# malaire/reed-solomon-16

Hardware: AMD Instinct MI355X
Metric: encode+decode GiB/s (device-resident, 1024B shards); % of HBM roofline (higher is better)
Workload: dtype u16; 1 GPU; 32768:32768 x 1024 B encode + 100%-loss decode per GPU (BASELINE configs[3]); original_count=32768, recovery_count=32768, parallelism=independent stripes x 1 (weak, no collective), column_slices=1, decode_issue=serial: rs16_decode_device after the encode

## Files before the change

include/rs16.h:

```cpp
#ifndef RS16_H
#define RS16_H

#include <stddef.h>
#include <stdint.h>

#ifdef __cplusplus
extern "C" {
#endif

typedef enum rs16_error_code {
    RS16_OK = 0,
    RS16_DIFFERENT_SHARD_SIZE = 1,
    RS16_DUPLICATE_ORIGINAL_SHARD_INDEX = 2,
    RS16_DUPLICATE_RECOVERY_SHARD_INDEX = 3,
    RS16_INVALID_ORIGINAL_SHARD_INDEX = 4,
    RS16_INVALID_RECOVERY_SHARD_INDEX = 5,
    RS16_INVALID_SHARD_SIZE = 6,
    RS16_NOT_ENOUGH_SHARDS = 7,
    RS16_TOO_FEW_ORIGINAL_SHARDS = 8,
    RS16_TOO_MANY_ORIGINAL_SHARDS = 9,
    RS16_UNSUPPORTED_SHARD_COUNT = 10,
    RS16_DEVICE_ERROR = 100,
    RS16_INVALID_ARGUMENT = 101
} rs16_error_code;
// ... 71 lines not shown
const void* rs16_decoder_restored_original_device(rs16_decoder* dec, size_t index);
int rs16_decoder_restored_original_copy(rs16_decoder* dec, size_t index, void* dst, size_t len, rs16_error* err);
void rs16_decoder_result_drop(rs16_decoder* dec);
int rs16_decoder_is_high_rate(const rs16_decoder* dec);

int rs16_encode_device(rs16_engine* eng, size_t original_count, size_t recovery_count, size_t shard_bytes,
                       const void* d_original, void* d_recovery, void* stream, rs16_error* err);
int rs16_encode_device_batch(rs16_engine* eng, size_t original_count, size_t recovery_count, size_t shard_bytes,
                             size_t nstripes, const void* d_original, size_t original_stride, void* d_recovery,
                             size_t recovery_stride, void* stream, rs16_error* err);
int rs16_decode_device(rs16_engine* eng, size_t original_count, size_t recovery_count, size_t shard_bytes,
                       void* d_original, const uint8_t* d_original_received, const void* d_recovery,
                       const uint8_t* d_recovery_received, size_t original_received_count,
                       size_t recovery_received_count, void* stream, rs16_error* err);
int rs16_decode_device_batch(rs16_engine* eng, size_t original_count, size_t recovery_count, size_t shard_bytes,
                             size_t nstripes, void* d_original, size_t original_stride,
                             const uint8_t* d_original_received, const void* d_recovery, size_t recovery_stride,
                             const uint8_t* d_recovery_received, size_t original_received_count,
                             size_t recovery_received_count, void* stream, rs16_error* err);
int rs16_decode_device_batch_varied(rs16_engine* eng, size_t original_count, size_t recovery_count,
                                    size_t shard_bytes, size_t nstripes, void* d_original, size_t original_stride,
                                    const uint8_t* d_original_received, size_t original_received_stride,
                                    const void* d_recovery, size_t recovery_stride,
                                    const uint8_t* d_recovery_received, size_t recovery_received_stride,
                                    const size_t* original_received_counts, const size_t* recovery_received_counts,
                                    void* stream, rs16_error* err);
int rs16_decode_check(rs16_engine* eng, void* stream, rs16_error* err);
int rs16_engine_set_slices(rs16_engine* eng, int slices, rs16_error* err);

int rs16_encode_host(rs16_engine* eng, size_t original_count, size_t recovery_count, size_t shard_bytes,
                     const void* h_original, void* h_recovery, size_t slice_bytes, rs16_error* err);
int rs16_decode_host(rs16_engine* eng, size_t original_count, size_t recovery_count, size_t shard_bytes,
                     void* h_original, const uint8_t* original_received, const void* h_recovery,
                     const uint8_t* recovery_received, size_t slice_bytes, rs16_error* err);

int rs16_decode_prepare(rs16_engine* eng, size_t original_count, size_t recovery_count, size_t shard_bytes,
                        const uint8_t* d_original_received, const uint8_t* d_recovery_received,
                        size_t original_received_count, size_t recovery_received_count, void* stream,
                        rs16_error* err);
int rs16_decode_device_prepared(rs16_engine* eng, size_t original_count, size_t recovery_count,
                                size_t shard_bytes, void* d_original, const void* d_recovery, void* stream,
                                rs16_error* err);

enum { RS16_UPDATE_MAX_SHARDS = 32 };
typedef struct rs16_update_plan rs16_update_plan;
rs16_update_plan* rs16_update_plan_new(rs16_engine* eng, int rate, size_t original_count, size_t recovery_count,
                                       const size_t* indices, size_t n, rs16_error* err);
void rs16_update_plan_free(rs16_update_plan* plan);
size_t rs16_update_plan_count(const rs16_update_plan* plan);
int rs16_update_plan_coefficients(rs16_update_plan* plan, uint16_t* out, rs16_error* err);
int rs16_update_device(rs16_update_plan* plan, size_t shard_bytes, const void* d_delta, void* d_recovery,
                       size_t recovery_pos, size_t recovery_n, void* stream, rs16_error* err);

int rs16_encode_host_batch(rs16_engine* eng, size_t original_count, size_t recovery_count, size_t shard_bytes,
                           size_t nstripes, const void* h_original, size_t original_stride, void* h_recovery,
                           size_t recovery_stride, rs16_error* err);
int rs16_decode_host_batch(rs16_engine* eng, size_t original_count, size_t recovery_count, size_t shard_bytes,
                           size_t nstripes, void* h_original, size_t original_stride,
                           const uint8_t* original_received, size_t original_received_stride,
                           const void* h_recovery, size_t recovery_stride, const uint8_t* recovery_received,
                           size_t recovery_received_stride, rs16_error* err);

int rs16_encode_host_multi(rs16_engine* const* engines, int n, size_t original_count, size_t recovery_count,
                           size_t shard_bytes, const void* h_original, void* h_recovery, rs16_error* err);
int rs16_decode_host_multi(rs16_engine* const* engines, int n, size_t original_count, size_t recovery_count,
                           size_t shard_bytes, void* h_original, const uint8_t* original_received,
                           const void* h_recovery, const uint8_t* recovery_received, rs16_error* err);

typedef struct rs16_comm rs16_comm;
int rs16_comm_unique_id(void* id128, rs16_error* err);
rs16_comm* rs16_comm_new(rs16_engine* eng, int nranks, int rank, const void* id128, rs16_error* err);
int rs16_comm_init_all(rs16_engine* const* engines, int n, rs16_comm** comms, rs16_error* err);
void rs16_comm_free(rs16_comm* comm);
int rs16_comm_rank(const rs16_comm* comm);
int rs16_comm_size(const rs16_comm* comm);
int rs16_column_slice(size_t shard_bytes, int nranks, int rank, size_t* offset, size_t* width);
int rs16_scatter_columns(rs16_comm* const* comms, int n, int root, size_t rows, size_t shard_bytes,
                         const void* const* d_full, void* const* d_slice, void* stream, rs16_error* err);
int rs16_gather_columns(rs16_comm* const* comms, int n, int root, size_t rows, size_t shard_bytes,
                        const void* const* d_slice, void* const* d_full, void* stream, rs16_error* err);
int rs16_scatter_columns_virtual(rs16_comm* comm, int vslices, size_t rows, size_t shard_bytes, const void* d_full,
                                 void* const* d_slices, void* stream, rs16_error* err);
int rs16_gather_columns_virtual(rs16_comm* comm, int vslices, size_t rows, size_t shard_bytes,
                                const void* const* d_slices, void* d_full, void* stream, rs16_error* err);

void* rs16_device_alloc(rs16_engine* eng, size_t bytes, rs16_error* err);
void rs16_device_free(rs16_engine* eng, void* d_ptr);
int rs16_memcpy_htod(rs16_engine* eng, void* d_dst, const void* src, size_t bytes, void* stream, rs16_error* err);
int rs16_memcpy_dtoh(rs16_engine* eng, void* dst, const void* d_src, size_t bytes, void* stream, rs16_error* err);
int rs16_memset_device(rs16_engine* eng, void* d_dst, int value, size_t bytes, void* stream, rs16_error* err);
int rs16_memcpy2d_htod(rs16_engine* eng, void* d_dst, size_t d_pitch, const void* src, size_t h_pitch, size_t width,
                       size_t rows, void* stream, rs16_error* err);
int rs16_memcpy2d_dtoh(rs16_engine* eng, void* dst, size_t h_pitch, const void* d_src, size_t d_pitch, size_t width,
                       size_t rows, void* stream, rs16_error* err);
void* rs16_stream_create(rs16_engine* eng, rs16_error* err);
void rs16_stream_destroy(rs16_engine* eng, void* stream);
void* rs16_host_alloc(rs16_engine* eng, size_t bytes, rs16_error* err);
void rs16_host_free(rs16_engine* eng, void* h_ptr);

int rs16_engine_set_profiling(rs16_engine* eng, int enable, rs16_error* err);
int rs16_engine_profile_read(rs16_engine* eng, int prog, double* total_ms, uint64_t* launches, rs16_error* err);
void rs16_engine_profile_reset(rs16_engine* eng);
int rs16_prog_count(void);
int rs16_engine_set_stamps(rs16_engine* eng, void* d_buf, int prog, rs16_error* err);
const char* rs16_prog_name(int prog);

enum {
    RS16_DIAG_FORCE_VOFF64 = 1,
    RS16_DIAG_EVAL_TWO_KERNEL = 2,
    RS16_DIAG_EVAL_FULL = 4,
    RS16_DIAG_NO_COLUMN = 8,
    RS16_DIAG_FORCE_COLUMN = 16,
    RS16_DIAG_TILE_LAST = 32,
    RS16_DIAG_NO_TILE_LAST = 64,
    RS16_DIAG_FD_LDS = 128,
    RS16_DIAG_COL_RADIX4 = 256,
    RS16_DIAG_NO_IDENTITY = 512,
    RS16_DIAG_NO_MID_DIRECT = 1024,
    RS16_DIAG_WIDE_TWIDDLES = 2048,
    RS16_DIAG_NO_LATE_ROWS = 4096,
    RS16_DIAG_NO_PAIRED_ROWS = 8192,
    RS16_DIAG_NO_TOWER_ROWS = 16384
};
int rs16_engine_set_diagnostics(rs16_engine* eng, int flags);
int rs16_set_diagnostics(int flags);

void rs16_host_mul(const void* in, void* out, size_t bytes, uint16_t log_m);
void rs16_host_mul_narrow(const void* in, void* out, size_t bytes, uint16_t log_m);
uint32_t rs16_host_twiddle(uint32_t index, uint32_t* log_m, uint32_t* table20);
int rs16_host_twiddle_narrow(uint32_t index);
uint64_t rs16_host_fast_div_check(uint32_t divisor, uint32_t n0, uint32_t count, uint32_t step);
typedef struct rs16_pass_consts {
    uint32_t voff32, full_lanes, nslab;
    uint32_t quads, threads, load_shb, store_shb, reg_bits, row_sets;
    uint64_t rs_in, rs_seg, rs_out;
    uint32_t late_rows;
} rs16_pass_consts;
int rs16_host_pass_consts(int prog, int T, uint32_t lo, uint64_t s_in, uint64_t s_out, uint64_t s_seg, uint64_t s_rest,
                          uint32_t qrow, uint32_t chunk, uint32_t row_base_in, uint32_t in_rows_mask, int diag,
                          rs16_pass_consts* out);
int rs16_host_pass_consts_many(int prog, int T, uint32_t lo, size_t n, const uint64_t* s_in, const uint64_t* s_out,
                               const uint64_t* s_seg, const uint64_t* s_rest, const uint32_t* qrow, uint32_t chunk,
                               uint32_t row_base_in, uint32_t in_rows_mask, int diag, rs16_pass_consts* out);
int rs16_host_pass_consts_rows(int prog, int T, uint32_t lo, uint64_t s_in, uint64_t s_out, uint64_t s_seg,
                               uint64_t s_rest, uint32_t qrow, uint32_t chunk, uint32_t row_base_in,
                               uint32_t in_rows_mask, uint32_t a_count, int diag, rs16_pass_consts* out);
int rs16_host_paired_rows(uint32_t chunk_rows, uint64_t S, uint64_t S_user, uint32_t a_count, uint32_t seg_chunk,
                          uint32_t row_base_in, int diag);
int rs16_host_tower_rows(uint32_t chunk_rows, uint64_t S, uint64_t S_user, uint32_t a_count, uint32_t seg_chunk,
                         uint32_t row_base_in, int diag);
uint32_t rs16_host_tower_basis(uint32_t i);
void rs16_host_tower_conv(const void* in, void* out, size_t bytes);
int rs16_host_tower_twiddle(uint32_t index, uint32_t* table20);
void rs16_host_mul_tower(const void* in, void* out, size_t bytes, uint32_t index, int narrow);
int rs16_host_update_consts(uint32_t rows, uint64_t shard_bytes, uint32_t n, uint32_t* quads_per_lane,
                            uint32_t* nslab, uint32_t* rows_per_wave, uint64_t* blocks);

const char* rs16_version(void);

#ifdef __cplusplus
}
#endif
#endif
```

reed-solomon-16_amd/csrc/rs16_api.cpp:

```cpp
#include <atomic>
#include <rccl/rccl.h>

#include <cstdio>

#include "rs16_api.hpp"
#include "rs16_pass_common.hpp"

using namespace rs16;

extern "C" size_t rs16_error_message(const rs16_error* e, char* buf, size_t len) {
    char tmp[256];
    unsigned long long a = e->v0, b = e->v1, c = e->v2;
    switch (e->code) {
    case RS16_OK: snprintf(tmp, sizeof tmp, "ok"); break;
    case RS16_DIFFERENT_SHARD_SIZE:
        snprintf(tmp, sizeof tmp, "different shard size: expected %llu bytes, got %llu bytes", a, b);
        break;
    case RS16_DUPLICATE_ORIGINAL_SHARD_INDEX: snprintf(tmp, sizeof tmp, "duplicate original shard index: %llu", a); break;
    case RS16_DUPLICATE_RECOVERY_SHARD_INDEX: snprintf(tmp, sizeof tmp, "duplicate recovery shard index: %llu", a); break;
    case RS16_INVALID_ORIGINAL_SHARD_INDEX:
        snprintf(tmp, sizeof tmp, "invalid original shard index: %llu >= original_count %llu", b, a);
        break;
    case RS16_INVALID_RECOVERY_SHARD_INDEX:
        snprintf(tmp, sizeof tmp, "invalid recovery shard index: %llu >= recovery_count %llu", b, a);
        break;
    case RS16_INVALID_SHARD_SIZE:
        snprintf(tmp, sizeof tmp, "invalid shard size: %llu bytes (must non-zero and multiple of 64)", a);
        break;
    case RS16_NOT_ENOUGH_SHARDS:
        snprintf(tmp, sizeof tmp, "not enough shards: %llu original + %llu recovery < %llu original_count", b, c, a);
        break;
    case RS16_TOO_FEW_ORIGINAL_SHARDS:
        snprintf(tmp, sizeof tmp, "too few original shards: got %llu shards while original_count is %llu", b, a);
        break;
    case RS16_TOO_MANY_ORIGINAL_SHARDS:
        snprintf(tmp, sizeof tmp, "too many original shards: got more than original_count (%llu) shards", a);
        break;
    case RS16_UNSUPPORTED_SHARD_COUNT:
        snprintf(tmp, sizeof tmp, "unsupported shard count: %llu original shards with %llu recovery shards", a, b);
        break;
    case RS16_DEVICE_ERROR:
        if (a >= 1000)
            snprintf(tmp, sizeof tmp, "device error: RCCL: %s", ncclGetErrorString((ncclResult_t)(a - 1000)));
        else
            snprintf(tmp, sizeof tmp, "device error: %s", hipGetErrorString((hipError_t)a));
        break;
    case RS16_INVALID_ARGUMENT: snprintf(tmp, sizeof tmp, "invalid argument"); break;
    default: snprintf(tmp, sizeof tmp, "unknown error %d", e->code); break;
    }
    size_t n = strlen(tmp);
    if (buf && len) {
        size_t c2 = std::min(n, len - 1);
        memcpy(buf, tmp, c2);
        buf[c2] = 0;
    }
    return n;
}

template <class F> static void host_mul_table(const void* in, void* out, size_t bytes, const uint32_t* t, F mul) {
    const uint8_t* src = (const uint8_t*)in;
    uint8_t* dst = (uint8_t*)out;
    for (size_t q = 0; q < bytes / 8; q++) {
        const size_t off = (q >> 3) * 64 + (q & 7) * 4;
        uint32_t yl, yh, ol = 0, oh = 0;
        memcpy(&yl, src + off, 4);
        memcpy(&yh, src + off + 32, 4);
        mul(ol, oh, yl, yh, t);
        memcpy(dst + off, &ol, 4);
        memcpy(dst + off + 32, &oh, 4);
    }
}
template <class Mul> static void host_mul(const void* in, void* out, size_t bytes, uint16_t log_m, Mul mul) {
    host_mul_table(in, out, bytes, &host_tables().mul_tab[(size_t)log_m * TAB_DWORDS], mul);
}
extern "C" void rs16_host_mul(const void* in, void* out, size_t bytes, uint16_t log_m) {
    host_mul(in, out, bytes, log_m, mul_xor);
}
extern "C" void rs16_host_mul_narrow(const void* in, void* out, size_t bytes, uint16_t log_m) {
    host_mul(in, out, bytes, log_m, mul_xor_narrow);
}
extern "C" uint32_t rs16_host_twiddle(uint32_t index, uint32_t* log_m, uint32_t* table20) {
    const HostTables& t = host_tables();
    if (index >= GF_MODULUS) return ~0u;
    if (log_m) *log_m = t.skew[index];
    if (table20) memcpy(table20, &t.skew_tab[(size_t)index * TAB_DWORDS], 20 * sizeof(uint32_t));
    return t.skew[index] == GF_MODULUS ? 0u : t.exp[t.skew[index]];
}
extern "C" int rs16_host_twiddle_narrow(uint32_t index) { return twiddle_narrow(index) ? 1 : 0; }
extern "C" uint64_t rs16_host_fast_div_check(uint32_t divisor, uint32_t n0, uint32_t count, uint32_t step) {
    const FastDiv f = fast_div_of(divisor);
    uint64_t bad = 0;
    for (uint64_t i = 0, n = n0; i < count && n < ((uint64_t)1 << 32); i++, n += step)
        bad += fast_div((uint32_t)n, f.mul, f.one) != (uint32_t)n / divisor;
    return bad;
}

static int host_pass_consts(int prog, int T, uint32_t lo, size_t n, const uint64_t* s_in, const uint64_t* s_out,
                            const uint64_t* s_seg, const uint64_t* s_rest, const uint32_t* qrow, uint32_t chunk,
                            uint32_t row_base_in, uint32_t in_rows_mask, uint32_t a_count, int diag,
                            rs16_pass_consts* out) {
    if (prog < 0 || prog >= NUM_PROGS || T < 0 || T > 8 || !out) return 0;
    const PassKernel& k = pass_kernel_of(prog, T);
    if (!k.fn) return 0;
    PassArgs a{};
    a.lo = lo, a.chunk = chunk, a.row_base_in = row_base_in, a.in_rows_mask = in_rows_mask;
    a.diag = (uint32_t)diag;
    a.a_count = a_count;
    for (size_t i = 0; i < n; i++) {
        a.S_in = s_in[i], a.S_out = s_out[i], a.S_seg = s_seg[i], a.S_rest = s_rest[i], a.qrow = qrow[i];
        const PassConsts c = pass_launch_consts(k, T, a);
        rs16_pass_consts& o = out[i];
        o.voff32 = c.voff32, o.full_lanes = c.full_lanes, o.nslab = c.nslab;
        o.quads = (uint32_t)k.quads, o.threads = (uint32_t)k.threads;
        o.load_shb = (uint32_t)k.load_shb, o.store_shb = (uint32_t)k.store_shb;
        o.reg_bits = (uint32_t)k.reg_bits, o.row_sets = k.quads >= 64 ? 1u : 64u / (uint32_t)k.quads;
        o.rs_in = c.rs_in, o.rs_seg = c.rs_seg, o.rs_out = c.rs_out;
        o.late_rows = c.late_rows;
    }
    return 1;
}
extern "C" int rs16_host_pass_consts_many(int prog, int T, uint32_t lo, size_t n, const uint64_t* s_in,
                                          const uint64_t* s_out, const uint64_t* s_seg, const uint64_t* s_rest,
                                          const uint32_t* qrow, uint32_t chunk, uint32_t row_base_in,
                                          uint32_t in_rows_mask, int diag, rs16_pass_consts* out) {
    return host_pass_consts(prog, T, lo, n, s_in, s_out, s_seg, s_rest, qrow, chunk, row_base_in, in_rows_mask, 0, diag,
                            out);
}
extern "C" int rs16_host_pass_consts_rows(int prog, int T, uint32_t lo, uint64_t s_in, uint64_t s_out, uint64_t s_seg,
                                          uint64_t s_rest, uint32_t qrow, uint32_t chunk, uint32_t row_base_in,
                                          uint32_t in_rows_mask, uint32_t a_count, int diag, rs16_pass_consts* out) {
    return host_pass_consts(prog, T, lo, 1, &s_in, &s_out, &s_seg, &s_rest, &qrow, chunk, row_base_in, in_rows_mask,
                            a_count, diag, out);
}
extern "C" int rs16_host_pass_consts(int prog, int T, uint32_t lo, uint64_t s_in, uint64_t s_out, uint64_t s_seg,
                                     uint64_t s_rest, uint32_t qrow, uint32_t chunk, uint32_t row_base_in,
                                     uint32_t in_rows_mask, int diag, rs16_pass_consts* out) {
    return rs16_host_pass_consts_many(prog, T, lo, 1, &s_in, &s_out, &s_seg, &s_rest, &qrow, chunk, row_base_in,
                                      in_rows_mask, diag, out);
}
extern "C" int rs16_host_paired_rows(uint32_t chunk_rows, uint64_t S, uint64_t S_user, uint32_t a_count,
                                     uint32_t seg_chunk, uint32_t row_base_in, int diag) {
    return z_form_sequence(chunk_rows, S, S_user, a_count, seg_chunk, row_base_in, diag) >= Z_PAIRED ? 1 : 0;
}
extern "C" int rs16_host_tower_rows(uint32_t chunk_rows, uint64_t S, uint64_t S_user, uint32_t a_count,
                                    uint32_t seg_chunk, uint32_t row_base_in, int diag) {
    return z_form_sequence(chunk_rows, S, S_user, a_count, seg_chunk, row_base_in, diag) == Z_TOWER ? 1 : 0;
}
extern "C" uint32_t rs16_host_tower_basis(uint32_t i) { return i < 8 ? host_tables().tower_a[i] : ~0u; }
extern "C" void rs16_host_tower_conv(const void* in, void* out, size_t bytes) {
    TowerB tb;
    memcpy(tb.p, host_tables().tower_b, sizeof tb.p);
    const uint8_t* src = (const uint8_t*)in;
    uint8_t* dst = (uint8_t*)out;
    for (size_t q = 0; q < bytes / 8; q++) {
        const size_t off = (q >> 3) * 64 + (q & 7) * 4;
        uint32_t l, h;
        memcpy(&l, src + off, 4);
        memcpy(&h, src + off + 32, 4);
        tower_conv(l, h, tb);
        memcpy(dst + off, &l, 4);
        memcpy(dst + off + 32, &h, 4);
    }
}
extern "C" int rs16_host_tower_twiddle(uint32_t index, uint32_t* table20) {
    if (index >= GF_MODULUS) return 0;
    if (table20) memcpy(table20, &host_tables().skew_tab_tower[(size_t)index * TAB_DWORDS], 20 * sizeof(uint32_t));
    return 1;
}
extern "C" void rs16_host_mul_tower(const void* in, void* out, size_t bytes, uint32_t index, int narrow) {
    const uint32_t* t = &host_tables().skew_tab_tower[(size_t)(index < GF_MODULUS ? index : GF_MODULUS) * TAB_DWORDS];
    host_mul_table(in, out, bytes, t, narrow ? mul_xor_tower_narrow : mul_xor);
}
extern "C" int rs16_host_update_consts(uint32_t rows, uint64_t shard_bytes, uint32_t n, uint32_t* quads_per_lane,
                                       uint32_t* nslab, uint32_t* rows_per_wave, uint64_t* blocks) {
    if (shard_bytes == 0 || (shard_bytes & 63) != 0 || shard_bytes / 8 > 0xFFFFFFFFu) return 0;
    UpdateArgs a{};
    a.S = shard_bytes, a.qrow = (uint32_t)(shard_bytes / 8), a.rows = rows;
    uint64_t nb;
    if (!update_launch_consts(a, n, &nb)) return 0;
    if (quads_per_lane) *quads_per_lane = a.quads_per_lane;
    if (nslab) *nslab = a.nslab;
    if (rows_per_wave) *rows_per_wave = a.rows_per_wave;
    if (blocks) *blocks = nb;
    return 1;
}

extern "C" int rs16_engine_set_profiling(rs16_engine* e, int enable, rs16_error* err) {
    if (int rc = e->activate(err)) return rc;
    if (int rc = e->prof_collect(err)) return rc;
    e->profiling = enable != 0;
    return set_error(err, RS16_OK);
}
extern "C" int rs16_engine_profile_read(rs16_engine* e, int prog, double* total_ms, uint64_t* launches,
                                        rs16_error* err) {
    if (prog < 0 || prog >= NUM_PROF) return set_error(err, RS16_INVALID_ARGUMENT);
    if (int rc = e->activate(err)) return rc;
    if (int rc = e->prof_collect(err)) return rc;
    if (total_ms) *total_ms = e->prof_ms[prog];
    if (launches) *launches = e->prof_n[prog];
    return set_error(err, RS16_OK);
}
extern "C" void rs16_engine_profile_reset(rs16_engine* e) {
    rs16_error err;
    (void)e->activate(&err);
    (void)e->prof_collect(&err);
    for (int i = 0; i < NUM_PROF; i++) e->prof_ms[i] = 0, e->prof_n[i] = 0;
}
extern "C" int rs16_engine_set_stamps(rs16_engine* e, void* d_buf, int prog, rs16_error* err) {
    if (prog < -1 || prog >= NUM_PROF) return set_error(err, RS16_INVALID_ARGUMENT);
    e->stamp_buf = d_buf;
    e->stamp_prof = prog;
    return set_error(err, RS16_OK);
}
extern "C" int rs16_engine_set_slices(rs16_engine* e, int n, rs16_error* err) {
    if (n < 1 || n > rs16_engine::MAX_SLICES) return set_error(err, RS16_INVALID_ARGUMENT);
    e->slices = n;
    return set_error(err, RS16_OK);
}
extern "C" int rs16_decode_check(rs16_engine* e, void* stream, rs16_error* err) {
    if (!e->last_dec_valid && !e->last_dec_flags_only) return set_error(err, RS16_OK);
    if (int rc = e->activate(err)) return rc;
    RS16_HIP(hipStreamSynchronize(e->pick(stream)));
    const DecodeGeom& g = e->last_dec;
    uint64_t a = 0, b = 0;
    if (e->last_dec_flags_only) {
        std::vector<uint8_t> f(2 * (size_t)GF_ORDER);
        RS16_HIP(hipMemcpy(f.data(), e->ws_flags.p, f.size(), hipMemcpyDeviceToHost));
        for (uint32_t i = 0; i < g.a_count; i++) a += f[i] != 0;
        for (uint32_t i = 0; i < g.b_count; i++) b += f[GF_ORDER + i] != 0;
    } else {
        const size_t chunks = ((size_t)g.n + 63) / 64;
        std::vector<uint32_t> c(2 * chunks);
        RS16_HIP(hipMemcpy(c.data(), e->ev_main.rcount.p, c.size() * 4, hipMemcpyDeviceToHost));
        for (size_t i = 0; i < chunks; i++) a += c[2 * i], b += c[2 * i + 1];
    }
    const auto want = DecodeSides::by_segment<uint64_t>(g.high, g.a_recv, g.b_recv);
    const auto got = DecodeSides::by_segment<uint64_t>(g.high, a, b);
    if (got != want) return set_error(err, RS16_INVALID_ARGUMENT, got.first, got.second);
    return set_error(err, RS16_OK);
}
static constexpr int DIAG_ALL = DIAG_FORCE_VOFF64 | DIAG_EVAL_TWO_KERNEL | DIAG_EVAL_FULL | DIAG_NO_COLUMN |
                                DIAG_FORCE_COLUMN | DIAG_TILE_LAST | DIAG_NO_TILE_LAST | DIAG_FD_LDS |
                                DIAG_COL_RADIX4 | DIAG_NO_IDENTITY | DIAG_NO_MID_DIRECT | DIAG_WIDE_TWIDDLES |
                                DIAG_NO_LATE_ROWS | DIAG_NO_PAIRED_ROWS | DIAG_NO_TOWER_ROWS;
extern "C" int rs16_engine_set_diagnostics(rs16_engine* e, int flags) {
    const int old = e->diag;
    e->diag = flags & DIAG_ALL;
    return old;
}
static std::atomic<int> g_default_diag{0};
extern "C" int rs16_set_diagnostics(int flags) { return g_default_diag.exchange(flags & DIAG_ALL); }
extern "C" int rs16_prog_count(void) { return NUM_PROF; }
extern "C" const char* rs16_prog_name(int prog) {
    static const char* names[] = {"GEN_FFT",   "GEN_IFFT",   "ENC_FIRST",     "ENC_MID",
                                  "ENC_LAST",  "ENC_SINGLE", "DEC_FIRST",     "DEC_MID",
                                  "DEC_LAST",  "DEC_SINGLE", "DEC_HALF_LAST", "DEC_HALF_SINGLE",
                                  "DEC_HALF_FIRST", "DEC_HALF_MID", "EVAL_POLY", "COL_ENC", "COL_DEC",
                                  "DEC_MID_DIRECT", "DEC_TILE_LAST"};
    static_assert(sizeof names / sizeof names[0] == NUM_PROF, "profiling names");
    return (prog >= 0 && prog < NUM_PROF) ? names[prog] : "?";
}

extern "C" const char* rs16_version(void) { return "rs16-mi355x 0.1 gfx950 (v_perm GF(2^16) engine)"; }

static bool high_supports(size_t k, size_t m) {
    return k > 0 && m > 0 && k < GF_ORDER && m < GF_ORDER && next_pow2(m) + k <= GF_ORDER;
}
static bool low_supports(size_t k, size_t m) {
    return k > 0 && m > 0 && k < GF_ORDER && m < GF_ORDER && next_pow2(k) + m <= GF_ORDER;
}

extern "C" int rs16_use_high_rate(size_t k, size_t m, rs16_error* err) {
    if (k > GF_ORDER || m > GF_ORDER) return set_error(err, RS16_UNSUPPORTED_SHARD_COUNT, k, m), -1;
    const size_t kp = next_pow2(k), mp = next_pow2(m);
    const size_t smaller = std::min(kp, mp), larger = std::max(k, m);
    if (k == 0 || m == 0 || smaller + larger > GF_ORDER) return set_error(err, RS16_UNSUPPORTED_SHARD_COUNT, k, m), -1;
    set_error(err, RS16_OK);
    if (kp < mp) return 0;
    if (kp > mp) return 1;
    return k <= m ? 1 : 0;
}

extern "C" int rs16_supports(int rate, size_t k, size_t m) {
    if (rate == RS16_RATE_HIGH) return high_supports(k, m);
    if (rate == RS16_RATE_LOW) return low_supports(k, m);
    return rs16_use_high_rate(k, m, nullptr) >= 0;
}

extern "C" int rs16_validate(int rate, size_t k, size_t m, size_t S, rs16_error* err) {
    if (!rs16_supports(rate, k, m)) return set_error(err, RS16_UNSUPPORTED_SHARD_COUNT, k, m);
    if (S == 0 || (S & 63) != 0 || (uint64_t)S >> 32) return set_error(err, RS16_INVALID_SHARD_SIZE, S);
    return set_error(err, RS16_OK);
}

extern "C" size_t rs16_encoder_work_count(int high, size_t k, size_t m) {
    const size_t chunk = high ? next_pow2(m) : next_pow2(k);
    const size_t n = high ? k : m;
    return (n + chunk - 1) / chunk * chunk;
}
extern "C" size_t rs16_decoder_work_count(int high, size_t k, size_t m) {
    return decode_geom(high != 0, k, m).n;
}

int rs16::resolve_rate(int rate, size_t k, size_t m, size_t S, bool* high, rs16_error* err) {
    if (rate == RS16_RATE_DEFAULT) {
        int h = rs16_use_high_rate(k, m, err);
        if (h < 0) return err ? err->code : RS16_UNSUPPORTED_SHARD_COUNT;
        *high = h == 1;
    } else if (rate == RS16_RATE_HIGH || rate == RS16_RATE_LOW) {
        *high = rate == RS16_RATE_HIGH;
    } else {
        return set_error(err, RS16_INVALID_ARGUMENT);
    }
    return rs16_validate(*high ? RS16_RATE_HIGH : RS16_RATE_LOW, k, m, S, err);
}
int rs16::check_received(size_t k, size_t orig_recv, size_t rec_recv, rs16_error* err) {
    if (orig_recv + rec_recv < k) return set_error(err, RS16_NOT_ENOUGH_SHARDS, k, orig_recv, rec_recv);
    return RS16_OK;
}

extern "C" rs16_engine* rs16_engine_new(int device, rs16_error* err) { return rs16_engine_new_ex(device, 0, err); }

extern "C" rs16_engine* rs16_engine_new_ex(int device, int flags, rs16_error* err) {
    if (flags & ~RS16_ENGINE_OWN_QUEUE) return set_error(err, RS16_INVALID_ARGUMENT), nullptr;
// ... 249 lines not shown
```

reed-solomon-16_amd/csrc/rs16_engine.cpp:

```cpp
#include <cstdlib>
#include "rs16_engine.hpp"

#include <algorithm>
#include <cstring>

namespace rs16 {

hipError_t DevBuf::reserve(size_t bytes) {
    if (bytes <= cap) return hipSuccess;
    if (p) (void)hipFree(p);
    p = nullptr;
    cap = 0;
    hipError_t e = hipMalloc(&p, bytes);
    if (e == hipSuccess) cap = bytes;
    return e;
}
void DevBuf::release() {
    if (p) (void)hipFree(p);
    p = nullptr;
    cap = 0;
}

hipError_t HostBuf::reserve(size_t bytes) {
    if (bytes <= cap) return hipSuccess;
// ... 114 lines not shown
        RS16_HIP(hipStreamWaitEvent(s, order_ev, 0));
    }
    return RS16_OK;
}

int rs16_engine::scratch_done(hipStream_t s, rs16_error* err) {
    if (s == stream) {
        last = LAST_ENGINE;
        return RS16_OK;
    }
    if (!order_ev) RS16_HIP(hipEventCreateWithFlags(&order_ev, hipEventDisableTiming));
    RS16_HIP(hipEventRecord(order_ev, s));
    last = LAST_CALLER;
    return RS16_OK;
}

int rs16_engine::prof_begin(hipStream_t s, hipEvent_t* ev, rs16_error* err) {
    *ev = nullptr;
    if (!profiling) return RS16_OK;
    if (ev_pool.empty()) {
        hipEvent_t e;
        RS16_HIP(hipEventCreate(&e));
        ev_pool.push_back(e);
    }
    *ev = ev_pool.back();
    ev_pool.pop_back();
    RS16_HIP(hipEventRecord(*ev, s));
    return RS16_OK;
}

int rs16_engine::prof_end(int id, hipStream_t s, hipEvent_t ev, rs16_error* err) {
    if (!ev) return RS16_OK;
    if (ev_pool.empty()) {
        hipEvent_t e;
        RS16_HIP(hipEventCreate(&e));
        ev_pool.push_back(e);
    }
    hipEvent_t b = ev_pool.back();
    ev_pool.pop_back();
    RS16_HIP(hipEventRecord(b, s));
    prof_pending.push_back({id, ev, b});
    if (prof_pending.size() > 4096) return prof_collect(err);
    return RS16_OK;
}

int rs16_engine::prof_collect(rs16_error* err) {
    for (const ProfRec& r : prof_pending) {
        RS16_HIP(hipEventSynchronize(r.b));
        float ms = 0.f;
        RS16_HIP(hipEventElapsedTime(&ms, r.a, r.b));
        prof_ms[r.id] += ms;
        prof_n[r.id] += 1;
        ev_pool.push_back(r.a);
        ev_pool.push_back(r.b);
    }
    prof_pending.clear();
    return RS16_OK;
}

template <class F> int rs16_engine::profiled(int prof, hipStream_t s, rs16_error* err, F launch) {
    hipEvent_t ev;
    if (int rc = prof_begin(s, &ev, err)) return rc;
    RS16_HIP(launch(stamp_buf && prof == stamp_prof ? (uint64_t*)stamp_buf : nullptr));
    return prof_end(prof, s, ev, err);
}

int rs16_engine::pass(int prog, int T, const PassArgs& a, uint32_t tiles, hipStream_t s, rs16_error* err, int prof) {
    return profiled(prof < 0 ? prog : prof, s, err, [&](uint64_t* stamps) {
        if (!stamps) return launch_pass(prog, T, a, tiles, s);
        PassArgs b = a;
        b.stamps = stamps;
        return launch_pass(prog, T, b, tiles, s);
    });
}

bool rs16_engine::col_ok(int L, size_t S, size_t nstripes, bool gen) const {
    const bool rows = col_rows_ok((uint32_t)L) || (gen && L == (int)COL_LGEN);
    if (!rows || (diag & DIAG_NO_COLUMN)) return false;
    return (S / 8) * nstripes <= col_max_quads || (diag & DIAG_FORCE_COLUMN);
}

bool rs16_engine::col_chunks_ok(int L, uint32_t nch, size_t S, bool high) const {
    const size_t rows_max = high && L <= 9 ? std::max<size_t>(col_max_chunk_rows, 8192) : col_max_chunk_rows;
    return L >= (int)COL_LCHUNK && L <= (int)COL_LMAX && nch > 1 && nch <= COL_MAX_CHUNKS &&
           (((size_t)nch << L) <= rows_max || (diag & DIAG_FORCE_COLUMN)) &&
           nch < col_img_count((uint32_t)L) && col_ok(L, S, 1);
}

ColArgs rs16_engine::col_args() const {
    ColArgs a;
    std::memset(&a, 0, sizeof a);
    a.skew_tab = d_skew_tab;
    a.mul_tab = d_mul_tab;
    a.zero = d_zero_sink;
    a.elog = (const uint32_t*)evset->elog.p;
    a.nstripes = 1;
    a.diag = (uint32_t)diag;
    return a;
}

int rs16_engine::col_tables(hipStream_t s, rs16_error* err) {
    if (d_col_img) return RS16_OK;
    const HostTables& t = host_tables();
    uint32_t *img = nullptr, *v = nullptr;
    RS16_HIP(hipMalloc(&img, COL_IMG_DWORDS * 4));
    if (hipError_t e = hipMalloc(&v, t.col_v.size() * 4)) {
        (void)hipFree(img);
        return hip_fail(err, e);
    }
    hipError_t e = hipMemcpyAsync(img, t.col_img.data(), COL_IMG_DWORDS * 4, hipMemcpyHostToDevice, s);
    if (e == hipSuccess) e = hipMemcpyAsync(v, t.col_v.data(), t.col_v.size() * 4, hipMemcpyHostToDevice, s);
    if (e == hipSuccess) e = hipStreamSynchronize(s);
    if (e != hipSuccess) {
        (void)hipFree(img);
        (void)hipFree(v);
        return hip_fail(err, e);
    }
    d_col_img = img;
    d_col_v = v;
    return RS16_OK;
}

int rs16_engine::col(const ColArgs& args, int L, int mode, hipStream_t s, rs16_error* err) {
    const bool dec = mode == COL_DEC_EWORK || mode == COL_DEC_EVAL || mode == COL_DEC_GEN;
    if (int rc = col_tables(s, err)) return rc;
    ColArgs a = args;
    const uint32_t N = 1u << L;
    if ((a.skew_ifft != 0 && a.skew_ifft != N) || (a.skew_fft != 0 && a.skew_fft != N) ||
        (a.nch > 1 && a.nch >= col_img_count((uint32_t)L)))
        return hip_fail(err, hipErrorInvalidValue);
    a.img_ifft = (const uint8_t*)(d_col_img + col_img_offset((uint32_t)L, a.skew_ifft ? 1 : 0));
    a.img_fft = (const uint8_t*)(d_col_img + col_img_offset((uint32_t)L, a.skew_fft ? 1 : 0));
    if (mode == COL_DEC_EVAL) a.vtab = d_col_v + col_v_offset(2u << L);
    if (mode == COL_DEC_GEN) a.vtab = d_col_v + col_v_offset(1u << L);
    return profiled(dec ? PROF_COL_DEC : PROF_COL_ENC, s, err, [&](uint64_t* stamps) {
        if (stamps) a.stamps = stamps;
        return launch_col(a, (uint32_t)L, mode, s);
    });
}

int rs16_engine::col_multi(size_t k, size_t m, size_t S, size_t S_user, const uint8_t* d_orig, uint8_t* d_rec,
                           uint32_t nch, bool high, hipStream_t s, rs16_error* err) {
    ColArgs c = col_args();
    c.in = d_orig;
    c.out = d_rec;
    c.S_in = c.S_out = S_user;
    c.qrow = (uint32_t)(S / 8);
    c.in_rows = (uint32_t)k;
    c.out_rows = (uint32_t)m;
    c.nch = nch;
    return profiled(PROF_COL_ENC, s, err, [&](uint64_t*) { return launch_col_multi(c, high, s); });
}

void rs16_engine::z_form_args(PassArgs& a, int prog, ZForm f) const {
    a.z_form = f;
    a.skew_tab = prog == ENC_MID && f == Z_TOWER ? d_skew_tab_tower : d_skew_tab;
}

int rs16_engine::fft(uint8_t* data, size_t S, size_t pos, size_t size, size_t skew_delta, hipStream_t s,
                     rs16_error* err) {
    const int L = ilog2(size);
    if (L == 0) return RS16_OK;
    PassArgs a = base_args(this, S);
    a.in = a.out = data + pos * S;
    a.skew_fft = (uint32_t)skew_delta;
    if (L <= 8) {
        RS16_PASS(GEN_FFT, L, a, 1, s);
        return RS16_OK;
    }
    const int lo = row_split(L).lo, hi = row_split(L).hi;
    a.lo = lo;
    RS16_PASS(GEN_FFT, hi, a, 1u << lo, s);
    a.lo = 0;
    RS16_PASS(GEN_FFT, lo, a, 1u << hi, s);
    return RS16_OK;
}

int rs16_engine::ifft(uint8_t* data, size_t S, size_t pos, size_t size, size_t skew_delta, hipStream_t s,
                      rs16_error* err) {
    const int L = ilog2(size);
    if (L == 0) return RS16_OK;
    PassArgs a = base_args(this, S);
    a.in = a.out = data + pos * S;
    a.skew_ifft = (uint32_t)skew_delta;
    if (L <= 8) {
        RS16_PASS(GEN_IFFT, L, a, 1, s);
        return RS16_OK;
    }
    const int lo = row_split(L).lo, hi = row_split(L).hi;
    a.lo = 0;
    RS16_PASS(GEN_IFFT, lo, a, 1u << hi, s);
    a.lo = lo;
    RS16_PASS(GEN_IFFT, hi, a, 1u << lo, s);
    return RS16_OK;
}

int rs16_engine::encode_high_fused(size_t k, size_t m, size_t S, size_t S_user, const uint8_t* d_orig, uint8_t* d_rec, uint8_t* Z,
                                   hipStream_t s, rs16_error* err, size_t nst, size_t bs_orig, size_t bs_rec) {
    const size_t chunk = next_pow2(m);
    const int L = ilog2(chunk);
    PassArgs a = base_args(this, S);
    a.seg_a = d_orig;
    a.S_seg = S_user;
    a.a_count = (uint32_t)k;
    a.skew_ifft = (uint32_t)chunk;
    a.skew_fft = 0;
    a.out_rows = (uint32_t)m;
    const uint32_t ns = (uint32_t)nst;
    auto batch = [&](uint32_t tiles, size_t bs_in, size_t bs_out, size_t bs_seg) {
        a.stripe_tiles = ns > 1 ? tiles : 0;
        a.bs_in = bs_in;
        a.bs_out = bs_out;
        a.bs_seg = bs_seg;
        return tiles * ns;
    };
    if (col_ok(L, S, nst)) {
        ColArgs c = col_args();
        c.in = d_orig;
        c.out = d_rec;
        c.S_in = c.S_out = S_user;
        c.qrow = (uint32_t)(S / 8);
        c.nstripes = ns;
        c.bs_in = bs_orig;
        c.bs_out = bs_rec;
        c.in_rows = (uint32_t)k;
        c.out_rows = (uint32_t)m;
        c.skew_ifft = (uint32_t)chunk;
        c.skew_fft = 0;
        return col(c, L, COL_ENC, s, err);
    }
    if (L <= 8) {
        a.out = d_rec;
        a.S_out = S_user;
        RS16_PASS(ENC_SINGLE, L, a, batch(1, 0, bs_rec, bs_orig), s);
        return RS16_OK;
    }
    const int lo = row_split(L).lo, hi = row_split(L).hi;
    const size_t zs = chunk * S;
    const ZForm zf = z_form_sequence((uint32_t)chunk, S, S_user, a.a_count, a.chunk, a.row_base_in, diag);
    a.out = Z;
    a.lo = 0;
    z_form_args(a, ENC_FIRST, zf);
    RS16_PASS(ENC_FIRST, lo, a, batch(1u << hi, 0, zs, bs_orig), s);
    a.in = Z;
    a.lo = lo;
    z_form_args(a, ENC_MID, zf);
    RS16_PASS(ENC_MID, hi, a, batch(1u << lo, zs, zs, 0), s);
    a.in = Z;
    a.out = d_rec;
    a.S_out = S_user;
    a.lo = 0;
    z_form_args(a, ENC_LAST, zf);
    const uint32_t tiles = (uint32_t)((m + ((size_t)1 << lo) - 1) >> lo);
    RS16_PASS(ENC_LAST, lo, a, batch(tiles, zs, bs_rec, 0), s);
    return RS16_OK;
}

int rs16_engine::decode_fused(const DecodeGeom& g, size_t S, size_t S_user, const uint8_t* seg_a, const uint8_t* flags_a,
                              const uint8_t* seg_b, const uint8_t* flags_b, uint8_t* rest, uint8_t* Z, uint8_t* U,
                              hipStream_t s, rs16_error* err) {
    if (int rc = decode_eval(g, flags_a, flags_b, s, err, S)) return rc;
    return decode_passes(g, S, S_user, seg_a, flags_a, seg_b, flags_b, rest, Z, U, (uint32_t*)evset->rcount.p, s, err);
}

int rs16_engine::guard_eval(hipStream_t s, bool consume, rs16_error* err) {
    if (!prep_pending) return RS16_OK;
    RS16_HIP(hipStreamWaitEvent(s, prep_ev, 0));
    prep_pending = false;
    if (!consume) prep.valid = false;
    return RS16_OK;
}

int rs16_engine::decode_eval(const DecodeGeom& g, const uint8_t* flags_a, const uint8_t* flags_b, hipStream_t s,
                             rs16_error* err, size_t S, size_t nstripes, uint32_t vary, size_t bs_fa, size_t bs_fb) {
    if (evset == &ev_main && !preparing)
        if (int rc = guard_eval(s, false, err)) return rc;
    if (!preparing) prep.valid = false;
    const size_t nv = vary > 1 ? vary : 1;
    RS16_HIP(evset->work32.reserve(nv * VARY_WORK * 4));
    RS16_HIP(evset->elog.reserve(nv * VARY_WORK * 4));
    RS16_HIP(evset->zflag.reserve(nv * VARY_ZFLAGS));
    RS16_HIP(evset->rbits.reserve(nv * VARY_RBITS * 4));
    RS16_HIP(evset->lost.reserve(nv * VARY_LOST * 4));
    RS16_HIP(evset->rcount.reserve(GF_ORDER / 64 * 8));
    var_ns = vary > 1 ? vary : 0;
    var_bs_fa = vary > 1 ? bs_fa : 0;
    var_bs_fb = vary > 1 ? bs_fb : 0;
    ErasureSpec es{};
    es.flags_a = flags_a;
    es.flags_b = flags_b;
    es.a_count = g.a_count;
    es.chunk = g.chunk;
    es.b_count = g.b_count;
    es.pad_fill = g.high ? 1 : 0;
    es.tail_fill = g.high ? 0 : 1;
    const int L = ilog2(g.n);
    es.rbits = (uint32_t*)evset->rbits.p;
    es.zflags = L > 8 ? (uint8_t*)evset->zflag.p : nullptr;
    es.n = g.n;
    es.zlo = (uint32_t)(L / 2);
    const bool prune = !half_decode(g) && L > 8;
    es.lostpart = prune ? (uint32_t*)evset->lost.p : nullptr;
    es.lostrange = prune ? (uint32_t*)evset->lost.p + 512 : nullptr;
    es.orig_b = g.high ? 1 : 0;
    es.rcount = (uint32_t*)evset->rcount.p;
    es.diag = (uint32_t)diag;
    last_dec = g;
    last_dec_valid = true;
    if (var_ns) {
        es.nstripes = var_ns;
        es.bs_fa = var_bs_fa;
        es.bs_fb = var_bs_fb;
        es.bs_work = es.bs_elog = VARY_WORK;
        es.bs_rbits = VARY_RBITS;
        es.bs_zflags = VARY_ZFLAGS;
        es.bs_lost = VARY_LOST;
        es.rcount = nullptr;
        last_dec_valid = false;
    }
    e_ident = identity_logs(g, vary);
    if (e_ident) {
        eval_in_col = elog_fused = false;
        return RS16_OK;
    }
    eval_in_col = S && (half_decode(g) ? g.high && col_ok(ilog2(g.n) - 1, S, nstripes)
                                       : col_ok(ilog2(g.n), S, nstripes, true));
    if (eval_in_col) return RS16_OK;
    es.stamps = stamp_prof == PROF_EVAL_POLY ? (uint64_t*)stamp_buf : nullptr;
    hipEvent_t pev;
    if (int rc = prof_begin(s, &pev, err)) return rc;
    const bool small = g.high && g.n <= 2048 && !(diag & DIAG_EVAL_FULL);
    elog_fused = !(half_decode(g) && ilog2(g.n) - 1 <= 8);
    if (small) {
        RS16_HIP(launch_eval_poly_small(es, (uint32_t)g.n, (uint32_t*)evset->work32.p, (uint32_t*)evset->elog.p, d_log_walsh,
                                        s, !elog_fused));
    } else {
        RS16_HIP(launch_eval_poly_from_flags(es, (uint32_t*)evset->work32.p, (uint32_t*)evset->elog.p, d_log_walsh, s,
                                             !elog_fused));
    }
    return prof_end(PROF_EVAL_POLY, s, pev, err);
}

bool rs16_engine::half_decode(const DecodeGeom& g) {
    const bool orig_lost = g.high ? g.b_recv == 0 : g.a_recv == 0;
    return orig_lost && g.n >= 2 && g.n == 2 * (size_t)g.chunk;
}

bool rs16_engine::identity_logs(const DecodeGeom& g, uint32_t vary) const {
    if ((diag & DIAG_NO_IDENTITY) || vary > 1 || !half_decode(g) || ilog2(g.n) - 1 < 11) return false;
    if (g.a_count != g.chunk || g.b_count != g.chunk) return false;
    return g.high ? g.a_recv == g.a_count : g.b_recv == g.b_count;
}

int rs16_engine::mid_tables(int L, const uint32_t** out, rs16_error* err) {
    DevBuf& b = mid_tab[L];
    if (!b.p) {
        const HostTables& t = host_tables();
        const std::vector<uint32_t> ent = mid_matrix_entries(t, L);
        std::vector<uint32_t> tabs(ent.size() * 20);
        for (size_t i = 0; i < ent.size(); i++)
            std::copy_n(&t.mul_tab[(size_t)ent[i] * TAB_DWORDS], 20, &tabs[i * 20]);
        hipError_t he = b.reserve(tabs.size() * 4);
        if (he == hipSuccess) he = hipMemcpy(b.p, tabs.data(), tabs.size() * 4, hipMemcpyHostToDevice);
        if (he != hipSuccess) {
            b.release();
            return hip_fail(err, he);
        }
    }
    *out = (const uint32_t*)b.p;
    return RS16_OK;
}

int rs16_engine::decode_passes(const DecodeGeom& g, size_t S, size_t S_user, const uint8_t* seg_a, const uint8_t* flags_a,
                               const uint8_t* seg_b, const uint8_t* flags_b, uint8_t* rest, uint8_t* Z, uint8_t* U,
                               uint32_t* rcount, hipStream_t s, rs16_error* err, size_t nst, size_t bs_a, size_t bs_b,
                               size_t bs_rest) {
    PassArgs a = base_args(this, S);
    a.S_seg = a.S_rest = S_user;
    a.seg_a = seg_a;
    a.seg_b = seg_b;
    a.flags_a = flags_a;
    a.flags_b = flags_b;
    a.a_count = g.a_count;
    a.chunk = g.chunk;
    a.b_count = g.b_count;
    a.elog = (const uint32_t*)evset->elog.p;
    a.ework = elog_fused ? (const uint32_t*)evset->work32.p : nullptr;
    a.rest = rest;
    a.rest_seg_b = g.high ? 1 : 0;
    a.rbits = (const uint32_t*)evset->rbits.p;
    a.skew_ifft = a.skew_fft = 0;
    if (var_ns) {
        a.bs_fa = var_bs_fa;
        a.bs_fb = var_bs_fb;
        a.bs_elog = VARY_WORK;
        a.bs_rbits = VARY_RBITS;
        a.bs_zflags = VARY_ZFLAGS;
        a.bs_lost = VARY_LOST;
        rcount = nullptr;
    }
    const uint32_t ns = (uint32_t)nst;
    const size_t zs = (size_t)g.n * S;
    a.bs_seg = bs_a;
    a.bs_seg_b = bs_b;
    a.bs_rest = bs_rest;
    auto batch = [&](uint32_t tiles, size_t bs_in, size_t bs_in2, size_t bs_out) {
        a.stripe_tiles = ns > 1 ? tiles : 0;
        a.bs_in = bs_in;
        a.bs_in2 = bs_in2;
        a.bs_out = bs_out;
        return tiles * ns;
    };
    const int L = ilog2(g.n);
    if (half_decode(g)) {
        const uint32_t half = g.n / 2, src = g.high ? 0 : half, dst = g.high ? half : 0;
        const uint32_t orig = g.high ? g.b_count : g.a_count;
        a.row_base_in = a.skew_ifft = src;
        a.row_base_out = a.skew_fft = dst;
        const int Lh = L - 1;
        if (e_ident) {
            const int lo = row_split(Lh).lo, hi = row_split(Lh).hi;
            a.seg_a = g.high ? seg_a : seg_b;
            a.bs_seg = g.high ? bs_a : bs_b;
            a.a_count = half;
            a.rcount = rcount;
            a.cnt_flags = g.high ? flags_a : flags_b;
            a.cnt_base = src;
            a.cnt_seg = g.high ? 0 : 1;
            const ZForm zf = z_form_sequence(half, S, S_user, a.a_count, a.chunk, a.row_base_in, diag);
            a.lo = 0;
            a.out = Z;
            z_form_args(a, ENC_FIRST, zf);
            RS16_PASS_AS(PROF_DEC_HALF_FIRST, ENC_FIRST, lo, a, batch(1u << hi, 0, 0, zs), s);
            a.rcount = nullptr;
            a.lo = lo;
            a.in = Z;
            z_form_args(a, ENC_MID, zf);
            RS16_PASS_AS(PROF_DEC_HALF_MID, ENC_MID, hi, a, batch(1u << lo, zs, 0, zs), s);
            a.lo = 0;
            a.out = rest;
            a.S_out = S_user;
            a.out_rows = orig;
            z_form_args(a, ENC_LAST, zf);
            a.rcount = rcount;
            a.cnt_flags = g.high ? flags_b : flags_a;
            a.cnt_base = dst;
            a.cnt_seg = g.high ? 1 : 0;
            RS16_PASS_AS(DEC_HALF_LAST, ENC_LAST, lo, a, batch((orig + (1u << lo) - 1) >> lo, zs, 0, bs_rest), s);
            return RS16_OK;
        }
        const bool col_eval = eval_in_col && g.high;
        if (!col_eval && Lh <= 8) {
            a.ework = nullptr;
            RS16_PASS(DEC_HALF_SINGLE, Lh, a, batch(1, 0, 0, 0), s);
            return RS16_OK;
        }
        if (col_eval || col_ok(Lh, S, ns)) {
            ColArgs c = col_args();
            c.in = g.high ? seg_a : seg_b;
            c.flags = g.high ? flags_a : flags_b;
            c.in_rows = g.high ? g.a_count : g.b_count;
            c.out = rest;
            c.S_in = c.S_out = S_user;
            c.qrow = (uint32_t)(S / 8);
            c.nstripes = ns;
            c.bs_in = g.high ? bs_a : bs_b;
            c.bs_out = bs_rest;
            c.out_rows = orig;
            c.base_in = c.skew_ifft = src;
            c.base_out = c.skew_fft = dst;
            c.chunk = g.chunk;
            c.e_pad = 1;
            c.bs_flags = g.high ? var_bs_fa : var_bs_fb;
            c.bs_flags_o = var_bs_fb;
            c.bs_elog = var_ns ? VARY_WORK : 0;
            if (col_eval) {
                c.flags_o = flags_b;
                c.o_rows = g.b_count;
                c.vtab = nullptr;
                c.rcount = rcount;
                return col(c, Lh, COL_DEC_EVAL, s, err);
            }
            c.elog = (const uint32_t*)evset->work32.p;
            return col(c, Lh, COL_DEC_EWORK, s, err);
        }
        const int lo = row_split(Lh).lo, hi = row_split(Lh).hi;
        a.lo = 0;
        a.out = Z;
        RS16_PASS_AS(PROF_DEC_HALF_FIRST, DEC_FIRST, lo, a, batch(1u << hi, 0, 0, zs), s);
        a.lo = lo;
        a.in = Z;
        RS16_PASS_AS(PROF_DEC_HALF_MID, ENC_MID, hi, a, batch(1u << lo, zs, 0, zs), s);
        a.lo = 0;
        a.out = nullptr;
        RS16_PASS(DEC_HALF_LAST, lo, a, batch((orig + (1u << lo) - 1) >> lo, zs, 0, 0), s);
        return RS16_OK;
    }
    if (eval_in_col) {
        ColArgs c = col_args();
        c.in = seg_a;
        c.flags = flags_a;
        c.in_rows = g.a_count;
        c.in_b = seg_b;
        c.bs_in_b = bs_b;
        c.flags_o = flags_b;
        c.o_rows = g.b_count;
        c.chunk = g.chunk;
        c.rev_a = g.high ? 0 : 1;
        c.e_pad = g.high ? 1 : 0;
        c.e_tail = g.high ? 0 : 1;
        c.e_k = g.high ? 0 : host_tables().col_k[L];
        c.out = rest;
        c.S_in = c.S_out = S_user;
        c.qrow = (uint32_t)(S / 8);
        c.nstripes = ns;
        c.bs_in = bs_a;
        c.bs_out = bs_rest;
        c.out_rows = g.high ? g.b_count : g.a_count;
        c.rcount = rcount;
        c.bs_flags = var_bs_fa;
        c.bs_flags_o = var_bs_fb;
        return col(c, L, COL_DEC_GEN, s, err);
    }
    if (L <= 8) {
        RS16_PASS(DEC_SINGLE, L, a, batch(1, 0, 0, 0), s);
        return RS16_OK;
    }
    const int lo = L / 2, hi = L - lo;
    a.zflags = (const uint8_t*)evset->zflag.p;
    a.lostrange = (const uint32_t*)evset->lost.p + 512;
    const uint32_t tile = 1u << lo, ntiles = 1u << hi;
    uint32_t t0z = ntiles, t1z = 0;
    if (g.a_recv) t0z = 0, t1z = (g.a_count + tile - 1) / tile;
    if (g.b_recv) {
        t0z = std::min(t0z, g.chunk / tile);
        t1z = std::max(t1z, std::min(ntiles, (uint32_t)(((size_t)g.chunk + g.b_count + tile - 1) / tile)));
    }
    if (t1z <= t0z) t0z = 0, t1z = 1;
    a.tile_base = t0z;
    a.lo = 0;
    a.out = Z;
    RS16_PASS(DEC_FIRST, lo, a, batch(t1z - t0z, 0, 0, zs), s);
    a.tile_base = 0;
    const uint32_t ob = g.high ? g.chunk : 0;
    const uint32_t oc = g.high ? g.b_count : g.a_count;
    const uint32_t t0 = ob >> lo, t1 = (uint32_t)(((size_t)ob + oc + ((size_t)1 << lo) - 1) >> lo);
    a.lo = lo;
    a.in = Z;
    a.out = U;
    a.need_lo = t0;
    a.need_hi = t1;
    const size_t lost = g.high ? (size_t)g.b_count - g.b_recv : (size_t)g.a_count - g.a_recv;
    if (!(diag & DIAG_NO_MID_DIRECT) && lost <= ((size_t)MID_DIRECT_MAX << lo) && ns <= 65535) {
        const uint32_t* mt = nullptr;
        if (int rc = mid_tables(L, &mt, err)) return rc;
        batch(1u << lo, zs, 0, zs);
        if (int rc = profiled(PROF_DEC_MID_DIRECT, s, err, [&](uint64_t* stamps) {
                a.stamps = stamps;
                const hipError_t e = launch_mid_direct(a, mt, (uint32_t)hi, ns, s);
                a.stamps = nullptr;
                return e;
            }))
            return rc;
        a.mid_direct = MID_DIRECT_MAX;
    }
    RS16_PASS(DEC_MID, hi, a, batch(1u << lo, zs, 0, zs), s);
    a.mid_direct = 0;
    a.need_lo = a.need_hi = 0;
    a.lo = 0;
    a.in = Z;
    a.in2 = U;
    a.out = nullptr;
    a.tile_base = t0;
    const bool tile_last = lo == 8 && !(diag & DIAG_NO_TILE_LAST) && (lost <= 2048 || (diag & DIAG_TILE_LAST));
    if (tile_last) {
        a.tl_max = (diag & DIAG_TILE_LAST) ? (1u << hi) : TILE_LAST_MAX;
        const uint32_t tiles = batch(std::min(t1 - t0, a.tl_max), zs, zs, 0);
        if (int rc = profiled(PROF_DEC_TILE_LAST, s, err, [&](uint64_t* stamps) {
                a.stamps = stamps;
                const hipError_t e = launch_tile_last(a, tiles, s);
                a.stamps = nullptr;
                return e;
            }))
            return rc;
        if (diag & DIAG_TILE_LAST) return RS16_OK;
    }
    RS16_PASS(DEC_LAST, lo, a, batch(t1 - t0, zs, zs, 0), s);
    return RS16_OK;
}

int rs16_engine::fft_to_recovery(size_t m, size_t S, size_t S_user, const uint8_t* src, uint8_t* Z, uint8_t* d_rec,
                                 size_t chunk, uint32_t nch, uint32_t skew, hipStream_t s, rs16_error* err) {
    const int L = ilog2(chunk), lo = L <= 8 ? L : L / 2, hi = L - lo;
    PassArgs a = base_args(this, S);
    a.skew_fft = skew;
    const uint32_t mask = src != Z ? (uint32_t)(chunk - 1) : 0u;
// ... 135 lines not shown
```

reed-solomon-16_amd/csrc/rs16_engine.hpp:

```cpp
#pragma once
#include <cstddef>
#include <cstdint>
#include <vector>

#include "../../include/rs16.h"
#include "rs16_internal.hpp"

namespace rs16 {

struct DevBuf {
    void* p = nullptr;
    size_t cap = 0;
    hipError_t reserve(size_t bytes);
    void release();
};
struct HostBuf {
    void* p = nullptr;
    size_t cap = 0;
    hipError_t reserve(size_t bytes);
    void release();
};
struct Pending {
    hipEvent_t ev = nullptr;
    bool busy = false;
    hipError_t record(hipStream_t s);
    hipError_t wait();
    void release();
};

int set_error(rs16_error* err, int code, uint64_t v0 = 0, uint64_t v1 = 0, uint64_t v2 = 0);
int hip_fail(rs16_error* err, hipError_t e);
#define RS16_HIP(call)                                 \
    do {                                               \
        hipError_t _e = (call);                        \
        if (_e != hipSuccess) return hip_fail(err, _e); \
    } while (0)
#define RS16_PASS(...)                                       \
    do {                                                     \
        if (int _rc = this->pass(__VA_ARGS__, err)) return _rc; \
    } while (0)
#define RS16_PASS_AS(PROF, ...)                                     \
    do {                                                            \
        if (int _rc = this->pass(__VA_ARGS__, err, PROF)) return _rc; \
    } while (0)

size_t next_pow2(size_t x);
inline int ilog2(size_t x) { int l = 0; while (((size_t)1 << l) < x) l++; return l; }

struct DecodeGeom {
    bool high;
    uint32_t a_count, chunk, b_count, n;
    size_t a_recv = 1, b_recv = 1;
};
DecodeGeom decode_geom(bool high, size_t k, size_t m);

}

struct rs16_encoder;
struct rs16_decoder;
struct rs16_update_plan;

struct rs16_engine {
    int device = 0;
    int flags = 0;
    hipStream_t stream = nullptr;
    int diag = 0;
    uint32_t* d_skew_tab = nullptr;
    uint32_t* d_skew_tab_tower = nullptr;
    uint32_t* d_mul_tab = nullptr;
    uint32_t* d_col_img = nullptr;
    uint32_t* d_col_v = nullptr;
    uint16_t* d_log_walsh = nullptr;
    uint8_t* d_zero_sink = nullptr;
    rs16::DevBuf ws_z, ws_u, ws_fd, ws_flags;
    rs16::DevBuf mid_tab[17];
    struct EvalBufs {
        rs16::DevBuf work32, elog;
        rs16::DevBuf zflag;
        rs16::DevBuf rbits;
        rs16::DevBuf lost;
        rs16::DevBuf rcount;
        void release() { work32.release(), elog.release(), zflag.release(), rbits.release(), lost.release(), rcount.release(); }
    };
    EvalBufs ev_main, ev_lane[2];
    EvalBufs* evset = &ev_main;
    struct Prepared {
        bool valid = false, nothing = false;
        size_t k = 0, m = 0, S = 0;
        rs16::DecodeGeom g{};
        const uint8_t* fl_a = nullptr;
        const uint8_t* fl_b = nullptr;
        int nslices = 1;
    } prep;
    hipEvent_t prep_ev = nullptr;
    bool prep_pending = false;
    bool preparing = false;
    int guard_eval(hipStream_t s, bool consume, rs16_error* err);
    rs16::DecodeGeom last_dec{};
    bool last_dec_valid = false;
    bool last_dec_flags_only = false;
    void forget_decode() { last_dec_valid = last_dec_flags_only = false; }
    struct HostSlot {
        hipStream_t s = nullptr;
        rs16::DevBuf orig, rec, z, u;
        rs16::DevBuf rcount;
    };
    HostSlot hslot[2];
    static constexpr int MAX_SLICES = 4;
    int slices = 1;
    hipStream_t sl_stream[MAX_SLICES] = {};
    hipStream_t sl_own[MAX_SLICES] = {};
    hipEvent_t sl_fork = nullptr, sl_join[MAX_SLICES] = {};
    int slice_count(size_t S) const;
    int fork(hipStream_t s, int n, rs16_error* err);
    int join(hipStream_t s, int n, rs16_error* err);
    rs16::DevBuf hflags;
    hipEvent_t hev = nullptr;
    hipEvent_t hp_ev[2] = {};
    hipEvent_t hp_off = nullptr;
    rs16::HostBuf hp_flags;
    int host_pipe_events(rs16_error* err);
    int host_slots(rs16_error* err);

    hipStream_t pick(void* s) const { return s ? (hipStream_t)s : stream; }
    int activate(rs16_error* err);

    enum { LAST_NONE, LAST_ENGINE, LAST_CALLER } last = LAST_NONE;
    hipEvent_t order_ev = nullptr;
    int order(hipStream_t s, rs16_error* err);
    int scratch_done(hipStream_t s, rs16_error* err);

    std::vector<rs16_encoder*> encoders;
    std::vector<rs16_decoder*> decoders;
    std::vector<rs16_update_plan*> update_plans;

    int pass(int prog, int T, const rs16::PassArgs& a, uint32_t tiles, hipStream_t s, rs16_error* err,
             int prof = -1);
    int prof_begin(hipStream_t s, hipEvent_t* ev, rs16_error* err);
    int prof_end(int id, hipStream_t s, hipEvent_t ev, rs16_error* err);
    template <class F> int profiled(int prof, hipStream_t s, rs16_error* err, F launch);
    bool profiling = false;
    void* stamp_buf = nullptr;
    int stamp_prof = -1;
    bool elog_fused = false;
    bool eval_in_col = false;
    bool e_ident = false;
    struct ProfRec {
        int id;
        hipEvent_t a, b;
    };
    std::vector<ProfRec> prof_pending;
    std::vector<hipEvent_t> ev_pool;
    double prof_ms[rs16::NUM_PROF] = {};
    uint64_t prof_n[rs16::NUM_PROF] = {};
    int prof_collect(rs16_error* err);

    void z_form_args(rs16::PassArgs& a, int prog, rs16::ZForm f) const;
    int fft(uint8_t* data, size_t S, size_t pos, size_t size, size_t skew_delta, hipStream_t s, rs16_error* err);
    int ifft(uint8_t* data, size_t S, size_t pos, size_t size, size_t skew_delta, hipStream_t s, rs16_error* err);

    int encode_high_fused(size_t k, size_t m, size_t S, size_t S_user, const uint8_t* d_orig, uint8_t* d_rec, uint8_t* Z,
                          hipStream_t s, rs16_error* err, size_t nstripes = 1, size_t bs_orig = 0, size_t bs_rec = 0);
    int decode_fused(const rs16::DecodeGeom& g, size_t S, size_t S_user, const uint8_t* seg_a, const uint8_t* flags_a,
                     const uint8_t* seg_b, const uint8_t* flags_b, uint8_t* rest, uint8_t* Z, uint8_t* U,
                     hipStream_t s, rs16_error* err);
    bool identity_logs(const rs16::DecodeGeom& g, uint32_t vary) const;
    int mid_tables(int L, const uint32_t** out, rs16_error* err);
    int decode_eval(const rs16::DecodeGeom& g, const uint8_t* flags_a, const uint8_t* flags_b, hipStream_t s,
                    rs16_error* err, size_t S = 0, size_t nstripes = 1, uint32_t vary = 0, size_t bs_fa = 0,
                    size_t bs_fb = 0);
    static constexpr uint32_t VARY_WORK = rs16::GF_ORDER, VARY_RBITS = rs16::GF_ORDER / 32, VARY_ZFLAGS = 256,
                              VARY_LOST = 520;
    uint32_t var_ns = 0;
    uint64_t var_bs_fa = 0, var_bs_fb = 0;
    int decode_passes(const rs16::DecodeGeom& g, size_t S, size_t S_user, const uint8_t* seg_a, const uint8_t* flags_a,
                      const uint8_t* seg_b, const uint8_t* flags_b, uint8_t* rest, uint8_t* Z, uint8_t* U,
                      uint32_t* rcount, hipStream_t s, rs16_error* err, size_t nstripes = 1, size_t bs_a = 0,
                      size_t bs_b = 0, size_t bs_rest = 0);
    static bool half_decode(const rs16::DecodeGeom& g);
    uint32_t col_max_quads = 256;
    bool col_ok(int L, size_t S, size_t nstripes, bool gen = false) const;
    uint32_t col_max_chunk_rows = 6144;
    bool col_chunks_ok(int L, uint32_t nch, size_t S, bool high) const;
    int col(const rs16::ColArgs& a, int L, int mode, hipStream_t s, rs16_error* err);
    int col_multi(size_t k, size_t m, size_t S, size_t S_user, const uint8_t* d_orig, uint8_t* d_rec, uint32_t nch,
                  bool high, hipStream_t s, rs16_error* err);
    int col_tables(hipStream_t s, rs16_error* err);
    rs16::ColArgs col_args() const;
    int encode_high_multi(size_t k, size_t m, size_t S, size_t S_user, const uint8_t* d_orig, uint8_t* d_rec,
                          uint8_t* Z, hipStream_t s, rs16_error* err);
    int encode_low_multi(size_t k, size_t m, size_t S, size_t S_user, const uint8_t* d_orig, uint8_t* d_rec,
                         uint8_t* Z, uint8_t* U, hipStream_t s, rs16_error* err);
    int fft_to_recovery(size_t m, size_t S, size_t S_user, const uint8_t* src, uint8_t* Z, uint8_t* d_rec,
                        size_t chunk, uint32_t nch, uint32_t skew, hipStream_t s, rs16_error* err);
};
```

reed-solomon-16_amd/csrc/rs16_gf.hpp:

```cpp
#pragma once
#include <stdint.h>

#if defined(__HIPCC__) || defined(__HIP__)
#include <hip/hip_runtime.h>
#define RS16_HD __host__ __device__ __forceinline__
#else
#define RS16_HD inline
#endif

namespace rs16 {

constexpr uint32_t GF_ORDER = 65536;
constexpr uint32_t GF_MODULUS = 65535;
constexpr uint32_t ZERO_ENTRY = 65536;
constexpr uint32_t TAB_ENTRIES = 65537;
constexpr uint32_t TAB_DWORDS = 32;

RS16_HD uint32_t perm_sw(uint32_t hi, uint32_t lo, uint32_t sel) {
    uint64_t pool = ((uint64_t)hi << 32) | lo;
    uint32_t r = 0;
    for (int i = 0; i < 4; i++) {
        uint32_t s = (sel >> (8 * i)) & 0xFF;
        r |= (uint32_t)((pool >> (8 * s)) & 0xFF) << (8 * i);
    }
    return r;
}

#if defined(__HIP_DEVICE_COMPILE__)
__device__ __forceinline__ uint32_t perm(uint32_t hi, uint32_t lo, uint32_t sel) {
    return __builtin_amdgcn_perm(hi, lo, sel);
}
__device__ __forceinline__ uint32_t xor3(uint32_t a, uint32_t b, uint32_t c) {
    return __builtin_amdgcn_bitop3_b32(a, b, c, 0x96);
}
#else
inline uint32_t perm(uint32_t hi, uint32_t lo, uint32_t sel) { return perm_sw(hi, lo, sel); }
inline uint32_t xor3(uint32_t a, uint32_t b, uint32_t c) { return a ^ b ^ c; }
#endif

struct MulSel {
    uint32_t s0, s1, s2, s3, s4, s5;
};
RS16_HD MulSel mul_selectors(uint32_t yL, uint32_t yH) {
#if defined(__HIP_DEVICE_COMPILE__)
    const uint64_t y = ((uint64_t)yH << 32) | yL;
    uint64_t a, b;
    asm("v_lshrrev_b64 %0, 3, %1" : "=v"(a) : "v"(y));
    asm("v_lshrrev_b64 %0, 6, %1" : "=v"(b) : "v"(y));
    const uint32_t s0 = yL & 0x07070707u;
    const uint32_t s1 = (uint32_t)a & 0x07070707u;
    const uint32_t s2 = (uint32_t)b & 0x03030303u;
    const uint32_t s3 = yH & 0x07070707u;
    const uint32_t s4 = (uint32_t)(a >> 32) & 0x07070707u;
    const uint32_t s5 = (uint32_t)(b >> 32) & 0x03030303u;
#else
    const uint32_t s0 = yL & 0x07070707u;
    const uint32_t a = yL >> 3;
    const uint32_t s1 = a & 0x07070707u;
    const uint32_t s2 = (a >> 3) & 0x03030303u;
    const uint32_t s3 = yH & 0x07070707u;
    const uint32_t b = yH >> 3;
    const uint32_t s4 = b & 0x07070707u;
    const uint32_t s5 = (b >> 3) & 0x03030303u;
#endif
    return MulSel{s0, s1, s2, s3, s4, s5};
}
template <bool NARROW>
RS16_HD void mul_xor_sel(uint32_t& xL, uint32_t& xH, const MulSel& y, const uint32_t* t) {
    const uint32_t s0 = y.s0, s1 = y.s1, s2 = y.s2, s3 = y.s3, s4 = y.s4, s5 = y.s5;
    if constexpr (NARROW) {
        const uint32_t l0 = perm(t[1], t[0], s0);
        const uint32_t l1 = perm(t[5], t[4], s1);
        const uint32_t l3 = perm(t[9], t[8], s3), h3 = perm(t[11], t[10], s3);
        const uint32_t l4 = perm(t[13], t[12], s4), h4 = perm(t[15], t[14], s4);
        const uint32_t l2 = perm(t[16], t[16], s2);
        const uint32_t l5 = perm(t[18], t[18], s5), h5 = perm(t[19], t[19], s5);
        xL = xor3(xor3(xL, l0, l1), xor3(l2, l3, l4), l5);
        xH = xor3(xH, h3, h4) ^ h5;
    } else {
        const uint32_t l0 = perm(t[1], t[0], s0), h0 = perm(t[3], t[2], s0);
        const uint32_t l1 = perm(t[5], t[4], s1), h1 = perm(t[7], t[6], s1);
        const uint32_t l3 = perm(t[9], t[8], s3), h3 = perm(t[11], t[10], s3);
        const uint32_t l4 = perm(t[13], t[12], s4), h4 = perm(t[15], t[14], s4);
        const uint32_t l2 = perm(t[16], t[16], s2), h2 = perm(t[17], t[17], s2);
        const uint32_t l5 = perm(t[18], t[18], s5), h5 = perm(t[19], t[19], s5);
        xL = xor3(xor3(xL, l0, l1), xor3(l2, l3, l4), l5);
        xH = xor3(xor3(xH, h0, h1), xor3(h2, h3, h4), h5);
    }
}
template <bool NARROW>
RS16_HD void mul_xor_t(uint32_t& xL, uint32_t& xH, uint32_t yL, uint32_t yH, const uint32_t* t) {
    mul_xor_sel<NARROW>(xL, xH, mul_selectors(yL, yH), t);
}
RS16_HD void mul_xor(uint32_t& xL, uint32_t& xH, uint32_t yL, uint32_t yH, const uint32_t* t) {
    mul_xor_t<false>(xL, xH, yL, yH, t);
}
RS16_HD void mul_xor_narrow(uint32_t& xL, uint32_t& xH, uint32_t yL, uint32_t yH, const uint32_t* t) {
    mul_xor_t<true>(xL, xH, yL, yH, t);
}

constexpr uint32_t TOWER_B_DWORD = 20;
struct TowerB {
    uint32_t p[5];
};
RS16_HD void tower_conv_sel(uint32_t& L, const MulSel& y, const TowerB& tb) {
    const uint32_t b0 = perm(tb.p[1], tb.p[0], y.s3);
    const uint32_t b1 = perm(tb.p[3], tb.p[2], y.s4);
    const uint32_t b2 = perm(tb.p[4], tb.p[4], y.s5);
    L = xor3(L, b0, b1) ^ b2;
}
RS16_HD MulSel high_selectors(uint32_t H) {
    const uint32_t a = H >> 3;
    return MulSel{0, 0, 0, H & 0x07070707u, a & 0x07070707u, (a >> 3) & 0x03030303u};
}
RS16_HD void tower_conv(uint32_t& L, uint32_t H, const TowerB& tb) { tower_conv_sel(L, high_selectors(H), tb); }
RS16_HD MulSel low_selectors(uint32_t L, const MulSel& y) {
    const uint32_t a = L >> 3;
    return MulSel{L & 0x07070707u, a & 0x07070707u, (a >> 3) & 0x03030303u, y.s3, y.s4, y.s5};
}
RS16_HD void mul_xor_tower_narrow_sel(uint32_t& xL, uint32_t& xH, const MulSel& y, const uint32_t* t) {
    const uint32_t l0 = perm(t[1], t[0], y.s0), h0 = perm(t[1], t[0], y.s3);
    const uint32_t l1 = perm(t[5], t[4], y.s1), h1 = perm(t[5], t[4], y.s4);
    const uint32_t l2 = perm(t[16], t[16], y.s2), h2 = perm(t[16], t[16], y.s5);
    xL = xor3(xL, l0, l1) ^ l2;
    xH = xor3(xH, h0, h1) ^ h2;
}
RS16_HD void mul_xor_tower_narrow(uint32_t& xL, uint32_t& xH, uint32_t yL, uint32_t yH, const uint32_t* t) {
    mul_xor_tower_narrow_sel(xL, xH, mul_selectors(yL, yH), t);
}

RS16_HD uint32_t add_mod(uint32_t x, uint32_t y) {
    uint32_t s = x + y;
    return (s + (s >> 16)) & 0xFFFFu;
}
RS16_HD uint32_t sub_mod(uint32_t x, uint32_t y) {
    uint32_t d = x - y;
    return (d + (d >> 16)) & 0xFFFFu;
}

}
```

reed-solomon-16_amd/csrc/rs16_internal.hpp:

```cpp
#pragma once
#include <hip/hip_runtime.h>
#include <stddef.h>
#include <stdint.h>

#include <vector>

#include "rs16_gf.hpp"

namespace rs16 {

struct HostTables {
    std::vector<uint16_t> exp, log, skew, log_walsh;
    std::vector<uint32_t> skew_entry;
    std::vector<uint32_t> mul_tab;
    std::vector<uint32_t> skew_tab;
    uint8_t tower_a[8] = {};
    uint32_t tower_b[5] = {};
    std::vector<uint32_t> skew_tab_tower;
    std::vector<uint32_t> col_img;
    std::vector<uint32_t> col_v;
    std::vector<uint32_t> col_k;
};
std::vector<uint32_t> mid_matrix_entries(const HostTables& t, int L);

constexpr uint32_t COL_LMIN = 6, COL_LMAX = 10;
constexpr uint32_t COL_LGEN = 11;
constexpr uint32_t COL_LCHUNK = 8;
constexpr uint32_t col_img_count(uint32_t L) {
    return L == COL_LGEN ? 1u : (L >= COL_LCHUNK ? (1u << (16 - L)) : 2u);
}
constexpr size_t col_img_offset(uint32_t L, uint32_t d) {
    size_t off = 0;
    for (uint32_t l = COL_LMIN; l < L; l++) off += (size_t)col_img_count(l) * ((1u << l) - 1) * 20;
    return off + (size_t)d * ((1u << L) - 1) * 20;
}
constexpr size_t COL_IMG_DWORDS = col_img_offset(COL_LGEN + 1, 0);
constexpr size_t col_v_offset(uint32_t n) { return n - (1u << COL_LMIN); }
constexpr size_t COL_V_DWORDS = col_v_offset(4u << COL_LMAX);
const HostTables& host_tables();

RS16_HD bool twiddle_narrow(uint32_t i) {
    const uint32_t x = i + 1;
    return x < ((x & (0u - x)) << 8);
}
inline int first_narrow_layer(uint32_t lo, int T, uint32_t skew, uint32_t bh_max) {
    int k = T;
    for (int kb = T - 1; kb >= 0; kb--) {
        const uint64_t d = (uint64_t)1 << (lo + kb);
        const uint64_t xmax = (((uint64_t)bh_max + 1) << (lo + T)) - d + skew;
        const uint64_t low = (d + skew) & (2 * d - 1);
        const uint64_t bit = low ? (low & (0 - low)) : 2 * d;
        if (xmax >= (bit << 8)) break;
        k = kb;
    }
    return k;
}

enum Prog : int {
    GEN_FFT = 0,
    GEN_IFFT,
    ENC_FIRST,
    ENC_MID,
    ENC_LAST,
    ENC_SINGLE,
    DEC_FIRST,
    DEC_MID,
    DEC_LAST,
    DEC_SINGLE,
    DEC_HALF_LAST,
    DEC_HALF_SINGLE,
    NUM_PROGS
};
enum ProfId : int {
    PROF_DEC_HALF_FIRST = NUM_PROGS,
    PROF_DEC_HALF_MID,
    PROF_EVAL_POLY,
    PROF_COL_ENC,
    PROF_COL_DEC,
    PROF_DEC_MID_DIRECT,
    PROF_DEC_TILE_LAST,
    NUM_PROF
};

struct PassArgs {
    uint8_t* out;
    const uint8_t* in;
    const uint8_t* in2;
    const uint8_t* seg_a;
    const uint8_t* seg_b;
    const uint8_t* flags_a;
    const uint8_t* flags_b;
    uint8_t* rest;
    const uint32_t* elog;
    const uint32_t* skew_tab;
    const uint32_t* mul_tab;
    uint64_t S_in, S_out, S_seg, S_rest;
    uint32_t qrow;
    uint32_t nslab;
    uint32_t ntiles;
    uint32_t lo;
    uint32_t a_count, chunk, b_count;
    uint32_t skew_ifft, skew_fft;
    uint32_t out_rows;
    uint32_t rest_seg_b;
    uint32_t row_base_in, row_base_out;
    uint32_t tile_base;
    uint32_t need_lo, need_hi;
    uint32_t voff32;
    uint32_t fd_lds;
    const uint8_t* zflags;
    const uint32_t* rbits;
    const uint8_t* zero;
    const uint32_t* ework;
    const uint32_t* lostrange;
    uint64_t* stamps;
    uint32_t stripe_tiles;
    uint64_t bs_in, bs_out, bs_seg, bs_in2, bs_seg_b, bs_rest;
    uint32_t in_rows_mask;
    uint64_t bs_fa, bs_fb;
    uint32_t bs_elog, bs_rbits, bs_zflags, bs_lost;
    uint32_t diag;
    uint32_t* rcount;
    const uint8_t* cnt_flags;
    uint32_t cnt_base, cnt_seg;
    uint32_t mid_direct;
    uint32_t tl_max;
    uint64_t rs_in, rs_seg, rs_out;
    uint32_t full_lanes;
    uint32_t nslab_one, stripe_one;
    uint32_t z_form;
    uint64_t nslab_mul, stripe_mul;
};

struct FastDiv {
    uint64_t mul;
    uint32_t one;
};
inline FastDiv fast_div_of(uint32_t d) {
    if (d <= 1) return {0, ~0u};
    return {~(uint64_t)0 / d + 1, 0};
}
RS16_HD uint32_t fast_div(uint32_t n, uint64_t mul, uint32_t one) {
    const uint64_t lo = ((uint64_t)n * (uint32_t)mul) >> 32;
    return (uint32_t)(((uint64_t)n * (uint32_t)(mul >> 32) + lo) >> 32) + (n & one);
}

struct ColArgs {
    const uint8_t* img_ifft;
    const uint8_t* img_fft;
    const uint8_t* flags_o;
    uint32_t o_rows;
    const uint32_t* vtab;
    uint32_t* rcount;
    uint32_t chunk;
    uint32_t e_pad, e_tail, e_k;
    uint32_t rev_a;
    const uint8_t* in_b;
    uint64_t bs_in_b;
    const uint8_t* in;
    const uint8_t* flags;
    uint8_t* out;
    const uint32_t* elog;
    const uint32_t* skew_tab;
    const uint32_t* mul_tab;
    const uint8_t* zero;
    uint64_t S_in, S_out;
    uint32_t qrow;
    uint32_t nstripes;
    uint32_t in_rows, out_rows;
    uint32_t skew_ifft, skew_fft;
    uint32_t base_in, base_out;
    uint64_t bs_in, bs_out;
    uint64_t bs_flags, bs_flags_o;
    uint32_t bs_elog;
    uint32_t nch;
    uint64_t* stamps;
    uint32_t diag;
};
int col_rows_ok(uint32_t L);
enum ColMode : int { COL_ENC = 0, COL_DEC_EWORK, COL_DEC_EVAL, COL_DEC_GEN, COL_ENC_IFFT, COL_ENC_FFTX };
constexpr uint32_t COL_MAX_CHUNKS = 64;
hipError_t launch_col(const ColArgs& a, uint32_t L, int mode, hipStream_t s);
constexpr uint32_t COLM_L = 7, COLM_MAX_CHUNKS = 16;
hipError_t launch_col_multi(const ColArgs& a, bool high, hipStream_t s);

enum DiagFlags : int {
    DIAG_FORCE_VOFF64 = 1,
    DIAG_EVAL_TWO_KERNEL = 2,
    DIAG_EVAL_FULL = 4,
    DIAG_NO_COLUMN = 8,
    DIAG_FORCE_COLUMN = 16,
    DIAG_TILE_LAST = 32,
    DIAG_NO_TILE_LAST = 64,
    DIAG_FD_LDS = 128,
    DIAG_COL_RADIX4 = 256,
    DIAG_NO_IDENTITY = 512,
    DIAG_NO_MID_DIRECT = 1024,
    DIAG_WIDE_TWIDDLES = 2048,
    DIAG_NO_LATE_ROWS = 4096,
    DIAG_NO_PAIRED_ROWS = 8192,
    DIAG_NO_TOWER_ROWS = 16384,
};

constexpr size_t RS16_ZERO_BYTES = 65536;

hipError_t launch_pass(int prog, int T, const PassArgs& a, uint32_t num_tiles, hipStream_t s);
struct RowSplit {
    int lo, hi;
// ... 58 lines not shown
```

reed-solomon-16_amd/csrc/rs16_pass.hpp:

```cpp
#pragma once
#include <type_traits>

#include "rs16_pass_common.hpp"
#include "rs16_fwht.hpp"
#include "rs16_diag.hpp"

namespace rs16 {

enum LoadMode { LD_PLAIN = 0, LD_GATHER_ENC, LD_GATHER_DEC, LD_DEC_LAST };
enum StoreMode { ST_PLAIN = 0, ST_RECOVERY, ST_RESTORE };

template <int P> struct ProgTraits;
#define RS16_PROG(P, LD, I, F, FF, ST)          \
    template <> struct ProgTraits<P> {         \
        static constexpr int LOAD = LD;        \
        static constexpr bool IFFT = I;        \
        static constexpr bool FD = F;          \
        static constexpr bool FFT = FF;        \
        static constexpr int STORE = ST;       \
        static constexpr bool ST_NT = !(I && FF);                                           \
    };
RS16_PROG(GEN_FFT, LD_PLAIN, false, false, true, ST_PLAIN)
RS16_PROG(GEN_IFFT, LD_PLAIN, true, false, false, ST_PLAIN)
RS16_PROG(ENC_FIRST, LD_GATHER_ENC, true, false, false, ST_PLAIN)
// ... 295 lines not shown
    u32x4 v[PER > 0 ? PER : 1];

    template <class F> __device__ __forceinline__ void issue(const uint32_t* tabs, F entry) {
        const u32x4* tab = (const u32x4*)tabs;
#pragma unroll
        for (int i = 0; i < PER; i++) {
            const int idx = (int)threadIdx.x + i * Geo<T>::THREADS;
            if (idx < N * 5) v[i] = tab[(size_t)entry(idx / 5) * (TAB_DWORDS / 4) + idx % 5];
        }
    }
    __device__ __forceinline__ void commit(uint4* dst) const {
        u32x4* d = (u32x4*)dst;
#pragma unroll
        for (int i = 0; i < PER; i++) {
            const int idx = (int)threadIdx.x + i * Geo<T>::THREADS;
            if (idx < N * 5) d[idx] = v[i];
        }
    }
};

template <int P, int T> struct WaveStaged {
    static constexpr bool value = (P == ENC_FIRST || P == ENC_MID || P == ENC_LAST) && T >= 7;
};
template <int N> struct WaveStager {
    static constexpr int PER = (N * 5 + 63) / 64;
    u32x4 v[PER > 0 ? PER : 1];
    template <class F> __device__ __forceinline__ void issue(const uint32_t* tabs, uint32_t lane, F entry) {
        const u32x4* tab = (const u32x4*)tabs;
#pragma unroll
        for (int i = 0; i < PER; i++) {
            const int idx = (int)lane + i * 64;
            if (idx < N * 5) v[i] = tab[(size_t)entry(idx / 5) * (TAB_DWORDS / 4) + idx % 5];
        }
    }
    template <class F> __device__ __forceinline__ void commit(uint4* dst, uint32_t lane, F slot) const {
        u32x4* d = (u32x4*)dst;
#pragma unroll
        for (int i = 0; i < PER; i++) {
            const int idx = (int)lane + i * 64;
            if (idx < N * 5) d[slot(idx / 5) * 5 + idx % 5] = v[i];
        }
    }
};
__device__ __forceinline__ void wave_lds_publish() {
    __builtin_amdgcn_fence(__ATOMIC_RELEASE, "wavefront");
    __builtin_amdgcn_s_waitcnt(0xC07F);
    __builtin_amdgcn_wave_barrier();
    __builtin_amdgcn_fence(__ATOMIC_ACQUIRE, "wavefront");
}

template <int T> struct TwiddleEntry {
    const PassArgs& a;
    const Thr& c;
    int t_begin;
    uint32_t skew;
    __device__ __forceinline__ uint32_t operator()(int i) const {
        const int t = t_begin + i;
        const int kb = T - 32 + __clz((uint32_t)((1 << T) - 1 - t));
        const uint32_t j = (uint32_t)(t - ((1 << T) - (1 << (T - kb))));
        const uint32_t d = 1u << (a.lo + kb);
        const uint32_t g = (c.b_high << (a.lo + T)) + (j << (kb + 1 + a.lo));
        return g + d + skew - 1;
    }
};

template <int T> struct RevealEntry {
    const PassArgs& a;
    const Thr& c;
    const uint32_t* el;
    __device__ __forceinline__ uint32_t operator()(int k) const {
        const uint32_t r = row_rel<T>(c, a, (uint32_t)k) + a.row_base_out;
        return row_lost_original(a, r) ? GF_MODULUS - (el ? el[k] : a.elog[r]) : ZERO_ENTRY;
    }
};

struct NoFin {
    template <class X> __device__ __forceinline__ void operator()(const X&, const X&, int) const {}
};
struct NoPre {
    template <class X> __device__ __forceinline__ void operator()(X&, X&, int) const {}
};

template <int T, bool LB, int KB0, int KB1, bool FFT> struct LayerSeq {
    static constexpr int SH = LB ? Geo<T>::SHB : 0;
    static constexpr int NR = Geo<T>::NR;
    static constexpr bool DF = FFT && !LB && KB0 == 0 && KB1 == Geo<T>::R && NR >= 8;
    static constexpr int df_at(int g) {
        int skb[16] = {}, sgi[16] = {};
        int sp = 0, n = 0;
        skb[sp] = KB1 - 1, sgi[sp] = 0, sp++;
        while (sp > 0) {
            sp--;
            const int kb = skb[sp], gi = sgi[sp];
            if (n++ == g) return kb * 16 + gi;
            if (kb > 0) {
                skb[sp] = kb - 1, sgi[sp] = 2 * gi + 1, sp++;
                skb[sp] = kb - 1, sgi[sp] = 2 * gi, sp++;
            }
        }
        return 0;
    }
    static constexpr int kb_of(int s) { return FFT ? KB1 - 1 - s : KB0 + s; }
    static constexpr int groups_of(int s) { return NR >> (kb_of(s) - SH + 1); }
    static constexpr int total() {
        int n = 0;
        for (int s = 0; s < KB1 - KB0; s++) n += groups_of(s);
        return n;
    }
    static constexpr int step_of(int g) {
        if (DF) return KB1 - 1 - df_at(g) / 16;
        int s = 0;
        while (g >= groups_of(s)) g -= groups_of(s), s++;
        return s;
    }
    static constexpr int index_of(int g) {
        if (DF) return df_at(g) % 16;
        int s = 0;
        while (g >= groups_of(s)) g -= groups_of(s), s++;
        return g;
    }
};

template <int T, bool LB, int KB0, int KB1, bool FFT, int G, bool IN_TAB2>
__device__ __forceinline__ const uint4* group_table(const Thr& c, const uint4* tab1, const uint4* tab2) {
    using S = LayerSeq<T, LB, KB0, KB1, FFT>;
    constexpr int s = S::step_of(G), gi = S::index_of(G);
    constexpr int kb = S::kb_of(s);
    constexpr int off = (1 << T) - (1 << (T - kb));
    const uint32_t j = LB ? (uint32_t)gi : (c.s << (Geo<T>::R - 1 - kb)) + gi;
    const uint32_t t = off + j;
    constexpr uint32_t base2 = T > 4 ? Geo<T>::TSPLIT : 0;
    return IN_TAB2 ? tab2 + (t - base2) * 5 : tab1 + t * 5;
}

template <int NR> __device__ __forceinline__ void pin_rows(uint32_t (&L)[NR], uint32_t (&H)[NR]) {
    if constexpr (NR >= 4) {
#pragma unroll
        for (int i = 0; i < NR; i += 4)
            asm volatile("" : "+v"(L[i]), "+v"(L[i + 1]), "+v"(L[i + 2]), "+v"(L[i + 3]), "+v"(H[i]), "+v"(H[i + 1]),
                         "+v"(H[i + 2]), "+v"(H[i + 3]));
    } else {
#pragma unroll
        for (int i = 0; i < NR; i++) asm volatile("" : "+v"(L[i]), "+v"(H[i]));
    }
}

enum { PR_NONE = 0, PR_OUT, PR_ZERO };
template <int NV> struct NarrowVar {
    static constexpr int NONE = 99;
    static constexpr int IFFT_FROM = NV == 0 ? NONE : (NV == 2 ? 1 : 0);
    static constexpr int FFT_FROM = NV == 0 ? NONE : (NV == 3 ? 1 : 0);
};

template <int P, int T, int NK, bool LB, int KB0, int KB1, bool FFT, bool IN_TAB2, int PRUNE, int G, class FIN = NoFin,
          class PRE = NoPre, bool TW = false>
struct GroupLoop {
    static __device__ __forceinline__ void run(uint32_t (&L)[Geo<T>::NR], uint32_t (&H)[Geo<T>::NR], const Thr& c,
                                               const PassArgs& a, const uint4* tab1, const uint4* tab2,
                                               const uint32_t (&cur)[20], uint32_t zmask, const FIN& fin = FIN(),
                                               const PRE& pre = PRE()) {
        using S = LayerSeq<T, LB, KB0, KB1, FFT>;
        constexpr int s = S::step_of(G), gi = S::index_of(G);
        constexpr int kb = S::kb_of(s);
        constexpr int rb = kb - S::SH;
        constexpr bool more = G + 1 < S::total();
        constexpr bool NARROW = kb >= NK;
        uint32_t nxt[20];
        if constexpr (more)
            load_table_lds(nxt, group_table<T, LB, KB0, KB1, FFT, G + 1, IN_TAB2>(c, tab1, tab2));
        __builtin_amdgcn_sched_barrier(0);
        bool need = true;
        if constexpr (PRUNE == PR_OUT)
            need = ((uint32_t)gi << (kb + 1)) < a.need_hi && ((uint32_t)(gi + 1) << (kb + 1)) > a.need_lo;
        if constexpr (PRUNE == PR_ZERO) {
            static_assert(LB && kb >= 4, "zero pruning works on 16-row blocks of layout B");
            constexpr int nb = 1 << (kb - 3);
            constexpr uint32_t all = (uint32_t)((1ull << nb) - 1);
            need = ((zmask >> (gi * nb)) & all) != all;
        }
        bool mul = true;
        if constexpr (LB && gi == 0 && ProgTraits<P>::IFFT && ProgTraits<P>::FFT) {
            const uint32_t idx = (c.b_high << (a.lo + T)) + (1u << (a.lo + kb)) + (FFT ? a.skew_fft : a.skew_ifft) - 1;
            mul = (idx & (idx + 1)) != 0;
        }
        if (need && mul) {
#pragma unroll
            for (int j = 0; j < (1 << rb); j++) {
                const int m = (gi << (rb + 1)) + j, m2 = m + (1 << rb);
                if constexpr (!std::is_same<PRE, NoPre>::value && s == 0) pre(L, H, (gi << rb) + j);
                if constexpr (TW && P == ENC_LAST && LB && FFT && s == 0) {
                    MulSel y = high_selectors(H[m2]);
                    tower_conv_sel(L[m2], y, pre.tb);
                    y = low_selectors(L[m2], y);
                    tower_conv(L[m], H[m], pre.tb);
                    mul_xor_sel<false>(L[m], H[m], y, cur);
                    L[m2] ^= L[m];
                    H[m2] ^= H[m];
                } else if constexpr (TW && P == ENC_MID && NARROW) {
                    if (FFT) {
                        mul_xor_tower_narrow(L[m], H[m], L[m2], H[m2], cur);
                        L[m2] ^= L[m];
                        H[m2] ^= H[m];
                    } else {
                        L[m2] ^= L[m];
                        H[m2] ^= H[m];
                        mul_xor_tower_narrow(L[m], H[m], L[m2], H[m2], cur);
                    }
                } else if (FFT) {
                    mul_xor_t<NARROW>(L[m], H[m], L[m2], H[m2], cur);
                    L[m2] ^= L[m];
                    H[m2] ^= H[m];
                } else {
                    L[m2] ^= L[m];
                    H[m2] ^= H[m];
                    mul_xor_t<NARROW>(L[m], H[m], L[m2], H[m2], cur);
                }
            }
        } else if (need) {
#pragma unroll
            for (int j = 0; j < (1 << rb); j++) {
                const int m = (gi << (rb + 1)) + j, m2 = m + (1 << rb);
                L[m2] ^= L[m];
                H[m2] ^= H[m];
            }
        }
#pragma unroll
        for (int j = 0; j < (1 << rb); j++) {
            const int m = (gi << (rb + 1)) + j, m2 = m + (1 << rb);
            asm volatile("" : "+v"(L[m]), "+v"(H[m]), "+v"(L[m2]), "+v"(H[m2]));
        }
        __builtin_amdgcn_sched_barrier(0);
        if constexpr (S::DF && kb == 0) fin(L, H, gi << 1);
        if constexpr (more)
            GroupLoop<P, T, NK, LB, KB0, KB1, FFT, IN_TAB2, PRUNE, G + 1, FIN, PRE, TW>::run(L, H, c, a, tab1, tab2,
                                                                                              nxt, zmask, fin, pre);
    }
};

__device__ __forceinline__ const uint4* lds_vgpr(const uint4* p) {
    uint32_t v = (uint32_t)(uintptr_t)(const __attribute__((address_space(3))) uint4*)p;
    asm volatile("" : "+v"(v));
    return (const uint4*)(const __attribute__((address_space(3))) uint4*)(uintptr_t)v;
}

template <int P, int T, int NK, bool LB, int KB0, int KB1, bool FFT, bool IN_TAB2, int PRUNE = PR_NONE,
          class FIN = NoFin, class PRE = NoPre, bool TW = false>
__device__ __forceinline__ void layers(uint32_t (&L)[Geo<T>::NR], uint32_t (&H)[Geo<T>::NR], const Thr& c,
                                       const PassArgs& a, const uint4* tab1, const uint4* tab2,
                                       uint32_t zmask = 0, const FIN& fin = FIN(), const PRE& pre = PRE()) {
    if constexpr (KB1 > KB0) {
        if constexpr (LB) {
            if constexpr (IN_TAB2) tab2 = lds_vgpr(tab2);
            else tab1 = lds_vgpr(tab1);
        }
        uint32_t t0[20];
        load_table_lds(t0, group_table<T, LB, KB0, KB1, FFT, 0, IN_TAB2>(c, tab1, tab2));
        GroupLoop<P, T, NK, LB, KB0, KB1, FFT, IN_TAB2, PRUNE, 0, FIN, PRE, TW>::run(L, H, c, a, tab1, tab2, t0, zmask,
                                                                                     fin, pre);
    }
}

template <int T, int QL> struct Img {
    static constexpr int PLANE = (1 << T) * QL;
    static __device__ __forceinline__ uint32_t* at(uint2* lds, const Thr& c, uint32_t k) {
        return (uint32_t*)lds + k * QL + c.ql;
    }
};

template <int NQR> __device__ __forceinline__ bool my_round(const Thr& c, int r) {
    return NQR == 1 || c.round == (uint32_t)r;
}

template <int T, int QL, bool LB>
__device__ __forceinline__ void put_rows(const uint32_t (&L)[Geo<T>::NR], const uint32_t (&H)[Geo<T>::NR],
                                         const Thr& c, uint2* lds) {
#pragma unroll
    for (int m = 0; m < Geo<T>::NR; m++) {
        uint32_t* p = Img<T, QL>::at(lds, c, kidx<T, LB>(c, m));
        p[0] = L[m];
        p[Img<T, QL>::PLANE] = H[m];
    }
}
template <int T, int QL, bool LB>
__device__ __forceinline__ void get_rows(uint32_t (&L)[Geo<T>::NR], uint32_t (&H)[Geo<T>::NR], const Thr& c,
                                         uint2* lds) {
#pragma unroll
    for (int m = 0; m < Geo<T>::NR; m++) {
        const uint32_t* p = Img<T, QL>::at(lds, c, kidx<T, LB>(c, m));
        L[m] = p[0];
        H[m] = p[Img<T, QL>::PLANE];
    }
}

template <int T, int QL, bool LB>
__device__ __forceinline__ void fd_rows(uint32_t (&L)[Geo<T>::NR], uint32_t (&H)[Geo<T>::NR],
                                        const uint32_t (&SL)[Geo<T>::NR], const uint32_t (&SH)[Geo<T>::NR],
                                        const Thr& c, uint2* lds) {
    constexpr int R = Geo<T>::R, SHB = Geo<T>::SHB;
#pragma unroll
    for (int m = 0; m < Geo<T>::NR; m++) {
        const uint32_t k = kidx<T, LB>(c, m);
        uint32_t xl = L[m], xh = H[m];
#pragma unroll
        for (int b = 0; b < T; b++) {
            const bool reg_bit = LB ? (b >= SHB) : (b < R);
            if (reg_bit) {
                const int mb = LB ? b - SHB : b;
                if (!((m >> mb) & 1)) {
                    xl ^= SL[m | (1 << mb)];
                    xh ^= SH[m | (1 << mb)];
                }
            } else {
                constexpr int LOG_HWS = Geo<T>::HWS == 4 ? 2 : (Geo<T>::HWS == 2 ? 1 : 0);
                const int sb = LB ? b : b - R;
                if (sb >= LOG_HWS) {
                    if (!((c.w >> (sb - LOG_HWS)) & 1)) {
                        const uint32_t* p = Img<T, QL>::at(lds, c, k | (1u << b));
                        xl ^= p[0];
                        xh ^= p[Img<T, QL>::PLANE];
                    }
                } else {
                    const uint32_t* p = Img<T, QL>::at(lds, c, k | (1u << b));
                    const uint32_t vl = p[0], vh = p[Img<T, QL>::PLANE];
                    const bool take = !((k >> b) & 1);
                    xl ^= take ? vl : 0u;
                    xh ^= take ? vh : 0u;
                }
            }
        }
        L[m] = xl;
        H[m] = xh;
    }
}

struct NoMid {
    __device__ __forceinline__ void operator()() const {}
};
template <int T, int NQR, bool FROM_B, class MID = NoMid, class POST = NoMid>
__device__ __forceinline__ void exchange(uint32_t (&L)[Geo<T>::NR], uint32_t (&H)[Geo<T>::NR], const Thr& c,
                                         uint2* lds, MID mid = MID(), POST post = POST()) {
    constexpr int QL = Geo<T>::Q / NQR;
#pragma unroll
    for (int r = 0; r < NQR; r++) {
        if (my_round<NQR>(c, r)) put_rows<T, QL, FROM_B>(L, H, c, lds);
        __syncthreads();
        if (r == 0) mid();
        if (my_round<NQR>(c, r)) {
            get_rows<T, QL, !FROM_B>(L, H, c, lds);
            post();
        }
        __syncthreads();
    }
}

template <int T, int ND>
__device__ __forceinline__ void few_switch(uint32_t (&L)[Geo<T>::NR], uint32_t (&H)[Geo<T>::NR], const Thr& c,
                                           uint2* lds, uint32_t m0) {
    constexpr int Q = Geo<T>::Q, SHB = Geo<T>::SHB, R = Geo<T>::R, NR = Geo<T>::NR;
    constexpr uint32_t ROWS = (uint32_t)ND << SHB, PLANE = ROWS * Q;
    uint32_t* img = (uint32_t*)lds;
    const uint32_t base = m0 << SHB;
#pragma unroll
    for (int m = 0; m < NR; m++) {
        const uint32_t i = (uint32_t)m - m0;
        if (i < (uint32_t)ND) {
            const uint32_t r = c.s + (i << SHB);
            img[r * Q + c.qt] = L[m];
            img[PLANE + r * Q + c.qt] = H[m];
        }
    }
    __syncthreads();
    const uint32_t k0 = c.s << R;
    if (k0 >= base && k0 < base + ROWS) {
#pragma unroll
        for (int m = 0; m < NR; m++) {
            const uint32_t r = k0 - base + (uint32_t)m;
            L[m] = img[r * Q + c.qt];
            H[m] = img[PLANE + r * Q + c.qt];
        }
    }
}

template <int T>
__device__ __forceinline__ void fd_regs(uint32_t (&L)[Geo<T>::NR], uint32_t (&H)[Geo<T>::NR]) {
    constexpr int R = Geo<T>::R, SHB = Geo<T>::SHB;
#pragma unroll
    for (int m = 0; m < Geo<T>::NR; m++) {
#pragma unroll
        for (int b = R; b < T; b++) {
            const int mb = b - SHB;
            if (!((m >> mb) & 1)) {
                L[m] ^= L[m | (1 << mb)];
                H[m] ^= H[m | (1 << mb)];
            }
        }
    }
}
template <int T, int QL>
__device__ __forceinline__ void fd_image(uint32_t& dl, uint32_t& dh, const Thr& c, const uint2* lds, uint32_t k) {
// ... 235 lines not shown
        if constexpr (WS) {
            const TwiddleEntry<T> tw{a, c, 0, PT::IFFT ? a.skew_ifft : a.skew_fft};
            sw.issue(a.skew_tab, c.lane, [&](int i) { return tw((int)wave_group(c, i)); });
        }
        s1.issue(a.skew_tab, TwiddleEntry<T>{a, c, 0, PT::IFFT ? a.skew_ifft : a.skew_fft});
        if constexpr (N1B > 0) s1b.issue(a.skew_tab, TwiddleEntry<T>{a, c, G::TSPLIT, a.skew_ifft});
        if constexpr (S2) s2.issue(a.skew_tab, TwiddleEntry<T>{a, c, G::NTAB - N2, a.skew_fft});
    }
    Stager<T, (PT::LOAD == LD_GATHER_DEC ? (1 << T) : 0)> se;
    const uint32_t* el = nullptr;
    __device__ __forceinline__ void gather(const PassArgs& a, const Thr& c, uint8_t* smem) {
        if constexpr (SM::ELOG_BYTES > 0) {
            if (a.ework) {
                uint32_t* elds = (uint32_t*)(smem + SM::ELOG_OFF);
                if (c.w == 0) {
                    fwht256_wave(ev);
#pragma unroll
                    for (int j = 0; j < 4; j++) elds[c.lane + 64 * j] = ev[j];
                }
                __syncthreads();
                el = elds + (elog_row0(a, c) & 255u);
            }
        }
        if constexpr (PT::LOAD == LD_GATHER_DEC) {
            static_assert(PER_E == Stager<T, (1 << T)>::PER, "one table chunk per (thread, i)");
            const u32x4* tab = (const u32x4*)a.mul_tab;
            auto gather_rows = [&](auto log_of) {
#pragma unroll
                for (int i = 0; i < PER_E; i++) {
                    const uint32_t idx = threadIdx.x + (uint32_t)i * G::THREADS;
                    const uint32_t k = min(idx / 5, (1u << T) - 1);
                    const uint32_t r = row_rel<T>(c, a, k) + a.row_base_in;
                    const bool rcv = (rw[i] >> (r & 31)) & 1u;
                    const uint32_t e = rcv ? log_of(k, r) : ZERO_ENTRY;
                    if (idx < (1u << T) * 5)
                        se.v[i] = tab[(size_t)e * (TAB_DWORDS / 4) + idx % 5];
                }
            };
            if (el) gather_rows([&](uint32_t k, uint32_t) { return el[k]; });
            else gather_rows([&](uint32_t, uint32_t r) { return a.elog[r]; });
        }
    }
    template <bool GATHERED = false>
    __device__ __forceinline__ void finish(const PassArgs& a, const Thr& c, uint8_t* smem) {
        if constexpr (!GATHERED) gather(a, c, smem);
        if constexpr (PT::LOAD == LD_GATHER_DEC) se.commit((uint4*)(smem + SM::ERT_OFF));
        if constexpr (PT::STORE == ST_RESTORE && !LateReveal<P, T>::value) {
            RevealStage<P, T> rs;
            rs.issue(a, c, el);
            rs.commit(smem);
        }
        if constexpr (WS) {
            sw.commit((uint4*)(smem + SM::TAB1_OFF), c.lane, [&](int i) { return wave_group(c, i); });
            if constexpr (S2) s2.commit((uint4*)(smem + SM::TAB2_OFF));
            s1.commit((uint4*)(smem + SM::TAB1_OFF));
            s1b.commit((uint4*)(smem + (SM::SHARED ? SM::TABB_OFF : SM::TAB1_OFF + G::TSPLIT * 80)));
            wave_lds_publish();
            return;
        }
        if constexpr (S2) s2.commit((uint4*)(smem + SM::TAB2_OFF));
        s1.commit((uint4*)(smem + SM::TAB1_OFF));
        if constexpr (N1B > 0) s1b.commit((uint4*)(smem + SM::TABB_OFF));
        __syncthreads();
    }
};

template <int P, int T> struct RcvCount {
    static constexpr bool ON = P == ENC_FIRST || P == ENC_LAST;
    static constexpr uint32_t NCH = (1u << T) >= 64 ? (1u << T) / 64 : 1;
    bool go;
    uint32_t r0, f, cnt;
    __device__ __forceinline__ void issue(const PassArgs& a, const Thr& c, bool first) {
        go = false;
        if constexpr (ON) {
            r0 = uni(row_rel<T>(c, a, 0) + 64u * c.w);
            go = first && a.rcount && c.w < NCH && (r0 & 63u) == 0;
            f = 1;
            asm("" : "+v"(f));
            if (go && a.cnt_flags) f = a.cnt_flags[r0 + c.lane];
        }
    }
    __device__ __forceinline__ void count() {
        if constexpr (ON)
            if (go) cnt = uni((uint32_t)__popcll(__ballot(f != 0)));
    }
    __device__ __forceinline__ void store(const PassArgs& a, const Thr& c) const {
        if constexpr (ON) {
            if (go && c.lane == 0) {
                const uint32_t ch = (r0 + a.cnt_base) >> 6;
                a.rcount[2 * ch + a.cnt_seg] = cnt;
                a.rcount[2 * ch + 1 - a.cnt_seg] = 0;
            }
        }
    }
};

template <int P, int T, bool V32>
__device__ __forceinline__ void store_row(const PassArgs& a, const Thr& cs, uint32_t L, uint32_t H, int m,
                                          const uint4* rvt, const uint32_t* lostf) {
    using PT = ProgTraits<P>;
    constexpr bool END_B = !PT::FFT && T > 4;
    constexpr bool NT = PT::ST_NT;
    const uint32_t lr = lane_rows<T, END_B>(cs, a);
    const WaveRows<T, END_B> wr(cs, a);
    const uint32_t ur = wr(m);
    if constexpr (PT::STORE == ST_PLAIN) {
        const LaneOff<V32> lo(lr, a.S_out, cs.offL);
        const uint32_t k = kidx<T, END_B>(cs, m);
        st_ptr<NT>(lo.at(sgpr_ptr(a.out + (uint64_t)ur * a.S_out)),
                   cs.active & (P != DEC_MID || (k >= a.need_lo && k < a.need_hi)), L, H);
    } else if constexpr (PT::STORE == ST_RECOVERY) {
        const LaneOff<V32> lo(lr, a.S_out, cs.offL);
        st_ptr<NT>(lo.at(sgpr_ptr(a.out + (uint64_t)ur * a.S_out)), cs.active & row_below(ur, lr, a.out_rows), L, H);
    } else {
        const LaneOff<V32> lo(lr, a.S_rest, cs.offL);
        const int64_t shift = (int64_t)a.row_base_out - (a.rest_seg_b ? (int64_t)a.chunk : 0);
        const uint32_t k = kidx<T, END_B>(cs, m);
        if (cs.active & (lostf[k] != 0)) {
            uint32_t tt[20];
            load_table_lds(tt, rvt + k * 5);
            uint32_t ol = 0, oh = 0;
            mul_xor(ol, oh, L, H, tt);
            st_ptr<NT>(lo.at(sgpr_ptr(a.rest + ((int64_t)ur + shift) * (int64_t)a.S_rest)), true, ol, oh);
        }
    }
}
template <int P, int T, bool V32>
__device__ __forceinline__ void store_rows(const PassArgs& a, const Thr& cs, const uint32_t (&L)[Geo<T>::NR],
                                           const uint32_t (&H)[Geo<T>::NR], const uint4* rvt, const uint32_t* lostf) {
#pragma unroll
    for (int m = 0; m < Geo<T>::NR; m++) store_row<P, T, V32>(a, cs, L[m], H[m], m, rvt, lostf);
}
template <int P, int T, bool PAIR = false> struct EarlyStore {
    const PassArgs& a;
    const Thr& cs;
    const uint4* rvt;
    const uint32_t* lostf;
    const FastStore<P, T, PAIR> fs;
    __device__ __forceinline__ void operator()(const uint32_t (&L)[Geo<T>::NR], const uint32_t (&H)[Geo<T>::NR],
                                               int m) const {
        if (PAIR || fs.on) {
            fs.row(m, L[m], H[m]);
            fs.row(m + 1, L[m + 1], H[m + 1]);
        } else if (a.voff32) {
            store_row<P, T, true>(a, cs, L[m], H[m], m, rvt, lostf);
            store_row<P, T, true>(a, cs, L[m + 1], H[m + 1], m + 1, rvt, lostf);
        } else {
            store_row<P, T, false>(a, cs, L[m], H[m], m, rvt, lostf);
            store_row<P, T, false>(a, cs, L[m + 1], H[m + 1], m + 1, rvt, lostf);
        }
    }
};

template <int T> struct HalfSeq {
    static constexpr int SH = Geo<T>::SHB, NR = Geo<T>::NR;
    static constexpr int at(int g) {
        int n = 0;
        for (int half = 0; half < 2; half++)
            for (int kb = Geo<T>::R; kb < T; kb++) {
                const int rb = kb - SH;
                if (rb == 0 && half == 1) continue;
                for (int gi = 0; gi < (NR >> (rb + 1)); gi++)
                    if (n++ == g) return half * 256 + kb * 16 + gi;
            }
        return -1;
    }
    static constexpr int total() {
        int g = 0;
        while (at(g) >= 0) g++;
        return g;
    }
};
struct NoTower {};
template <int T, int G, class FIN, class TB = NoTower> struct HalfLoop {
    static_assert(std::is_same<TB, NoTower>::value || HalfSeq<T>::SH < Geo<T>::R, "a row's last layer: kb = T - 1");
    static __device__ __forceinline__ void run(uint32_t (&L)[Geo<T>::NR], uint32_t (&H)[Geo<T>::NR],
                                               const uint4* tab1, const uint32_t (&cur)[20], const FIN& fin,
                                               const TB& tb = TB()) {
        using S = HalfSeq<T>;
        constexpr int e = S::at(G), half = e >> 8, kb = (e >> 4) & 15, gi = e & 15, rb = kb - S::SH;
        constexpr bool more = G + 1 < S::total();
        uint32_t nxt[20];
        if constexpr (more) {
            constexpr int kb2 = (S::at(G + 1) >> 4) & 15, gi2 = S::at(G + 1) & 15;
            load_table_lds(nxt, tab1 + ((1 << T) - (1 << (T - kb2)) + gi2) * 5);
        }
        __builtin_amdgcn_sched_barrier(0);
#pragma unroll
        for (int j = 0; j < (1 << rb); j++) {
            if (rb > 0 && (j & 1) != half) continue;
            const int m = (gi << (rb + 1)) + j, m2 = m + (1 << rb);
            L[m2] ^= L[m];
            H[m2] ^= H[m];
            if constexpr (!std::is_same<TB, NoTower>::value && kb == T - 1) {
                const MulSel y = mul_selectors(L[m2], H[m2]);
                mul_xor_sel<false>(L[m], H[m], y, cur);
                tower_conv_sel(L[m2], y, tb);
                tower_conv(L[m], H[m], tb);
            } else {
                mul_xor(L[m], H[m], L[m2], H[m2], cur);
            }
            asm volatile("" : "+v"(L[m]), "+v"(H[m]), "+v"(L[m2]), "+v"(H[m2]));
        }
        __builtin_amdgcn_sched_barrier(0);
        if constexpr (more) {
            if constexpr (half == 0 && (S::at(G + 1) >> 8) == 1) fin(L, H);
            HalfLoop<T, G + 1, FIN, TB>::run(L, H, tab1, nxt, fin, tb);
        }
    }
};
template <int T, class FIN, class TB = NoTower>
__device__ __forceinline__ void ifft_b_halves(uint32_t (&L)[Geo<T>::NR], uint32_t (&H)[Geo<T>::NR], const uint4* tab1,
                                              const FIN& fin, const TB& tb = TB()) {
    constexpr int e = HalfSeq<T>::at(0), kb = (e >> 4) & 15, gi = e & 15;
    tab1 = lds_vgpr(tab1);
    uint32_t t0[20];
    load_table_lds(t0, tab1 + ((1 << T) - (1 << (T - kb)) + gi) * 5);
    HalfLoop<T, 0, FIN, TB>::run(L, H, tab1, t0, fin, tb);
}
template <int P, int T, bool PAIR = false> struct EvenStore {
    const PassArgs& a;
    const Thr& cs;
    const FastStore<P, T, PAIR> fs;
    __device__ __forceinline__ void operator()(const uint32_t (&L)[Geo<T>::NR], const uint32_t (&H)[Geo<T>::NR]) const {
        if (PAIR || fs.on) {
#pragma unroll
            for (int m = 0; m < Geo<T>::NR; m += 2) fs.row(m, L[m], H[m]);
            return;
        }
#pragma unroll
        for (int m = 0; m < Geo<T>::NR; m += 2) {
            if (a.voff32) store_row<P, T, true>(a, cs, L[m], H[m], m, nullptr, nullptr);
            else store_row<P, T, false>(a, cs, L[m], H[m], m, nullptr, nullptr);
        }
    }
};

template <int P, int T, int NV, class PRE = NoPre, bool PAIR_OUT = false, bool TOWER = false>
__device__ __forceinline__ void process_item(const PassArgs& a, const Thr& c, uint32_t tile, ItemRegs<P, T>& d,
                                             uint8_t* smem, const PRE& pre = PRE()) {
    using PT = ProgTraits<P>;
    constexpr int NKI = NarrowVar<NV>::IFFT_FROM, NKF = NarrowVar<NV>::FFT_FROM;
    static_assert(NV == 0 || (PT::IFFT && PT::FFT && T > 4), "narrow variants: two-direction passes only");
    using SM = Smem<P, T>;
    using G = Geo<T>;
    constexpr int NR = G::NR;
    constexpr int R = G::R;
    constexpr int NQR = Rnd<P, T>::NQR;
    constexpr bool TWO = SM::TWO;
    constexpr bool ZERO_SKIP = P == DEC_MID && T > 4 && G::R == 4;
    constexpr bool EARLY = LayerSeq<T, false, 0, R, true>::DF && P != DEC_MID && PT::STORE != ST_RESTORE && PT::FFT &&
                           T > 4;
    constexpr bool EARLY_B = PT::IFFT && !PT::FFT && PT::STORE == ST_PLAIN && T > 4 && G::R == 4;
    uint2* lds = (uint2*)smem;
    const uint4* tab1 = (const uint4*)(smem + SM::TAB1_OFF);
    const uint4* tab2 = (const uint4*)(smem + SM::TAB2_OFF);
    const uint4* ert = (const uint4*)(smem + SM::ERT_OFF);
    const uint4* rvt = (const uint4*)(smem + SM::RVT_OFF);
    const uint32_t* lostf = (const uint32_t*)(smem + SM::LOST_OFF);
    uint32_t(&L)[NR] = d.L;
    uint32_t(&H)[NR] = d.H;
    constexpr bool START_B = !PT::IFFT;
    [[maybe_unused]] constexpr bool END_B = !PT::FFT && T > 4;
    constexpr bool SPLIT_FD = P == DEC_MID && T > 4;
    constexpr int FD_PB = 1 << (R - G::SHB);
    constexpr int FD_ND = FD_PB > 2 ? FD_PB : 2;
    [[maybe_unused]] bool fd_few = false;
    [[maybe_unused]] uint32_t fd_m0 = 0;
    [[maybe_unused]] uint32_t dl[FD_ND], dh[FD_ND];
    if constexpr (SPLIT_FD) {
        const uint32_t lo = uni(a.need_lo), hi = uni(min(a.need_hi, 1u << T));
        const uint32_t m0 = (lo >> R) * FD_PB, m1 = hi <= lo ? m0 : (((hi - 1) >> R) + 1) * FD_PB;
        fd_few = !a.fd_lds && m1 - m0 <= (uint32_t)FD_ND;
        fd_m0 = hi <= lo ? 0u : min(m0, (uint32_t)(NR - FD_ND));
    }

    if constexpr (P == DEC_FIRST) {
        if (a.zflags && tile_is_zero(a, tile)) {
            __builtin_amdgcn_s_waitcnt(vmcnt_wait(0));
            return;
        }
    }
    if constexpr (PT::LOAD == LD_GATHER_DEC) {
#pragma unroll
        for (int m = 0; m < NR; m++) {
            uint32_t tt[20];
            load_table_lds(tt, ert + kidx<T, START_B>(c, m) * 5);
            const uint32_t yl = L[m], yh = H[m];
            L[m] = H[m] = 0;
            mul_xor(L[m], H[m], yl, yh, tt);
        }
    }
    if constexpr (PT::LOAD == LD_DEC_LAST) {
        if (!d.ztile) tile_fd<T, NQR, START_B>(L, H, d.zl, d.zh, c, lds);
    }

    [[maybe_unused]] Stager<T, (SM::SHARED ? G::TSPLIT : 0)> s3s;
    bool in_b = START_B;
    if constexpr (PT::IFFT) {
        bool skip_a = false;
        if constexpr (ZERO_SKIP) skip_a = __all(d.zrow == (1u << NR) - 1);
        if constexpr (WaveStaged<P, T>::value) RS16_STAMP_ROWS(a, 6, L, H, 0, 1);
        if constexpr (!std::is_same<PRE, NoPre>::value)
            layers<P, T, NKI, false, 0, R, false, false, PR_NONE, NoFin, PRE, TOWER>(L, H, c, a, tab1, tab2, 0, NoFin(),
                                                                                     pre);
        else if (!skip_a) layers<P, T, NKI, false, 0, R, false, false>(L, H, c, a, tab1, tab2);
        RS16_STAMP(a, 3);
        prio<1>();
        if constexpr (T > 4) {
            constexpr bool LS2 = SM::RESTAGE && !SM::SHARED;
            Stager<T, (LS2 ? G::TSPLIT : 0)> s3;
            if constexpr (LS2) s3.issue(a.skew_tab, TwiddleEntry<T>{a, c, 0, a.skew_fft});
            if constexpr (SM::SHARED) __syncthreads();
            exchange<T, NQR, false>(
                L, H, c, lds,
                [&]() {
                    if constexpr (LS2) s3.commit((uint4*)(smem + SM::TAB1_OFF));
                },
                [&]() {
                    if constexpr (SPLIT_FD) {
                        if (fd_few) {
                            constexpr int QL = G::Q / NQR;
#pragma unroll
                            for (int i = 0; i < FD_ND; i++)
                                fd_image<T, QL>(dl[i], dh[i], c, lds, kidx<T, true>(c, fd_m0 + i));
                        }
                    }
                });
            RS16_STAMP(a, 4);
            if constexpr (SM::SHARED) s3s.issue(a.skew_tab, TwiddleEntry<T>{a, c, 0, a.skew_fft});
            if constexpr (EARLY_B) {
                Thr cs = c;
                asm volatile("" : "+v"(cs.offL));
                const EvenStore<P, T, PAIR_OUT> even{a, cs, FastStore<P, T, PAIR_OUT>(a, cs)};
                if constexpr (TOWER) ifft_b_halves<T>(L, H, tab1, even, pre.tb);
                else ifft_b_halves<T>(L, H, tab1, even);
            } else {
                const uint4* tab1b = SM::SHARED ? (const uint4*)(smem + SM::TABB_OFF) - G::TSPLIT * 5 : tab1;
                layers<P, T, NKI, true, R, T, false, false, (ZERO_SKIP ? PR_ZERO : PR_NONE), NoFin, NoPre, TOWER>(
                    L, H, c, a, tab1b, tab2, d.zmask);
            }
            in_b = true;
        }
        RS16_STAMP(a, 5);
        prio<2>();
    }
    if constexpr (PT::FD) {
        if constexpr (SPLIT_FD) {
            if (fd_few) fd_regs<T>(L, H);
            else tile_fd<T, NQR, true>(L, H, L, H, c, lds);
        } else {
            if (in_b) tile_fd<T, NQR, true>(L, H, L, H, c, lds);
            else tile_fd<T, NQR, false>(L, H, L, H, c, lds);
        }
        RS16_STAMP(a, 6);
    }
    if constexpr (PT::FFT) {
        if constexpr (T > 4) {
            if constexpr (WaveStaged<P, T>::value && !PT::IFFT) RS16_STAMP_ROWS(a, 6, L, H, 0, NR / 2);
            if constexpr (!std::is_same<PRE, NoPre>::value && !PT::IFFT)
                layers<P, T, NKF, true, R, T, true, TWO, PR_NONE, NoFin, PRE, TOWER>(L, H, c, a, tab1, tab2, 0, NoFin(),
                                                                                     pre);
            else
                layers<P, T, NKF, true, R, T, true, TWO, (P == DEC_MID ? PR_OUT : PR_NONE), NoFin, NoPre, TOWER>(
                    L, H, c, a, tab1, tab2);
            if constexpr (SPLIT_FD) {
                if (fd_few) {
#pragma unroll
                    for (int m = 0; m < NR; m++) {
#pragma unroll
                        for (int i = 0; i < FD_ND; i++)
                            if ((uint32_t)m == fd_m0 + i) L[m] ^= dl[i], H[m] ^= dh[i];
                    }
                }
            }
            RS16_STAMP(a, 7);
            prio<3>();
            RevealStage<P, (LateReveal<P, T>::value ? T : 0)> rs;
            if constexpr (LateReveal<P, T>::value) {
                const uint32_t* el = nullptr;
                if (a.ework) {
                    const uint32_t base = a.row_base_out;
                    el = (const uint32_t*)(smem + SM::ELOG_OFF) + ((row_rel<T>(c, a, 0) + base) & 255u);
                }
                rs.issue(a, c, el);
            }
            if constexpr (SPLIT_FD) {
                if (fd_few) few_switch<T, FD_ND>(L, H, c, lds, fd_m0);
                else exchange<T, NQR, true>(L, H, c, lds);
            } else {
                exchange<T, NQR, true>(L, H, c, lds, [&]() {
                    if constexpr (LateReveal<P, T>::value) rs.commit(smem);
                });
            }
            if constexpr (SM::SHARED) {
                if constexpr (SPLIT_FD) {
                    if (fd_few) __syncthreads();
                }
                s3s.commit((uint4*)(smem + SM::TAB1_OFF));
                __syncthreads();
            }
            RS16_STAMP(a, 8);
            prio<4>();
            in_b = false;
        }
        bool need = true;
        if constexpr (P == DEC_MID) need = (c.s << R) < a.need_hi && ((c.s + 1) << R) > a.need_lo;
        if constexpr (PT::STORE == ST_RESTORE && T > 4) {
            uint32_t any = 0;
#pragma unroll
            for (int m = 0; m < NR; m++) any |= lostf[kidx<T, false>(c, m)];
            need = any != 0;
        }
        if constexpr (EARLY) {
            Thr cs = c;
            asm volatile("" : "+v"(cs.offL));
            layers<P, T, NKF, false, 0, R, true, (TWO && !(SM::RESTAGE)), PR_NONE, EarlyStore<P, T, PAIR_OUT>, NoPre,
                   TOWER>(L, H, c, a, tab1, tab2, 0,
                          EarlyStore<P, T, PAIR_OUT>{a, cs, rvt, lostf, FastStore<P, T, PAIR_OUT>(a, cs)});
        } else if (need) {
            layers<P, T, NKF, false, 0, R, true, (TWO && !(SM::RESTAGE))>(L, H, c, a, tab1, tab2);
        }
        RS16_STAMP(a, 9);
    }
    if constexpr (EARLY) {
        RS16_STAMP(a, 10);
        RS16_STAMP_END(a);
        return;
    }

    prio<5>();
    __builtin_amdgcn_s_waitcnt(vmcnt_wait(0));
    Thr cs = c;
    cs.b_low = uni(cs.b_low);
    cs.b_high = uni(cs.b_high);
    asm volatile("" : "+s"(cs.b_low), "+s"(cs.b_high));
    asm volatile("" : "+v"(cs.offL));
    const FastStore<P, T, PAIR_OUT> fs(a, cs);
    if (PAIR_OUT || fs.on) {
#pragma unroll
        for (int m = EARLY_B ? 1 : 0; m < NR; m += EARLY_B ? 2 : 1) fs.row(m, L[m], H[m]);
    } else if constexpr (EARLY_B) {
#pragma unroll
        for (int m = 1; m < NR; m += 2) {
            if (a.voff32) store_row<P, T, true>(a, cs, L[m], H[m], m, rvt, lostf);
            else store_row<P, T, false>(a, cs, L[m], H[m], m, rvt, lostf);
        }
    } else {
        if (a.voff32) store_rows<P, T, true>(a, cs, L, H, rvt, lostf);
        else store_rows<P, T, false>(a, cs, L, H, rvt, lostf);
    }
    RS16_STAMP(a, 10);
    RS16_STAMP_END(a);
}

#define RS16_PASS_HEAD(P, T) \
    const uint32_t item = blockIdx.x; \
    Thr c; \
    c.lane = threadIdx.x & 63; \
    c.w = uni(threadIdx.x >> 6); \
    c.qt = c.lane % G::Q; \
    c.s = c.w * G::HWS + c.lane / G::Q; \
    c.ql = c.qt % Rnd<P, T>::QL; \
    c.round = c.qt / Rnd<P, T>::QL; \
    uint32_t tile, slab; \
    set_item(c, a, item, G::Q, tile, slab); \
    bool first_stripe = true; \
    if (a.stripe_tiles) { \
        const uint32_t st = uni(fast_div(tile, a.stripe_mul, a.stripe_one)); \
        first_stripe = st == 0; \
        tile -= st * a.stripe_tiles; \
        stripe_displace(a, st); \
    } \
    tile += a.tile_base; \
    c.b_low = tile & ((1u << a.lo) - 1); \
    c.b_high = tile >> a.lo; \
    RcvCount<P, T> rcn; \
    rcn.issue(a, c, slab == 0 && first_stripe);
#define RS16_LATE_BODY(P, T, NV, RQ, PAIR_OUT, TOWER) \
    RS16_STAMP(a, 0); \
    const uint32_t slot = (__builtin_amdgcn_s_getreg((31 << 11) | 4) >> 16) & 15u; \
    if (slot == 0) __builtin_amdgcn_s_setprio(3); \
    else if (slot == 1) __builtin_amdgcn_s_setprio(2); \
    else if (slot == 2) __builtin_amdgcn_s_setprio(1); \
    TileStage<P, T> st; \
    st.issue(a, c); \
    ItemRegs<P, T> cur; \
    cur.zrow = cur.zmask = 0; \
    cur.ztile = false; \
    const RQ rq(a, c); \
    rq.prologue(cur.L, cur.H); \
    RS16_STAMP(a, 1); \
    prio<0>(); \
    st.template finish<false>(a, c, smem); \
    rcn.count(); \
    RS16_STAMP(a, 2); \
    process_item<P, T, NV, RQ, PAIR_OUT, TOWER>(a, c, tile, cur, smem, rq); \
    rcn.store(a, c);

template <int P, int T, int NV = 0>
__global__ void __launch_bounds__(Geo<T>::THREADS, ((P == DEC_SINGLE || P == DEC_HALF_SINGLE) ? 1 : 4))
    pass_kernel(PassArgs a) {
    using G = Geo<T>;
    extern __shared__ __attribute__((aligned(16))) uint8_t smem[];
    RS16_PASS_HEAD(P, T)
    if constexpr (P == DEC_FIRST) {
        if (a.zflags && tile_is_zero(a, tile)) return;
    }
    if constexpr (P == DEC_MID) {
        uint32_t nlo, nhi;
        if (a.mid_direct && a.lostrange && mid_need(a, nlo, nhi)) return;
    }
    if constexpr (P == DEC_LAST) {
        if (a.lostrange) {
            const uint32_t r0 = ((cu32p)a.lostrange)[0], r1 = ((cu32p)a.lostrange)[1];
            if (!((tile << T) < r1 && ((tile + 1) << T) > r0)) return;
            if (a.tl_max && tl_covers<T>(a)) return;
        }
    }
    RS16_STAMP(a, 0);
    if constexpr (T >= 7) {
        const uint32_t slot = (__builtin_amdgcn_s_getreg((31 << 11) | 4) >> 16) & 15u;
        if (slot == 0) __builtin_amdgcn_s_setprio(3);
        else if (slot == 1) __builtin_amdgcn_s_setprio(2);
        else if (slot == 2) __builtin_amdgcn_s_setprio(1);
    }
    TileStage<P, T> st;
    st.issue(a, c);
    constexpr bool EARLY = ProgTraits<P>::LOAD == LD_GATHER_DEC;
    if constexpr (EARLY) st.gather(a, c, smem);
    ItemRegs<P, T> cur;
    if constexpr (WaveStaged<P, T>::value) {
        static_assert(FastRows<P, T>::LOAD, "the encoder-family passes have the full-item loads");
        cur.zrow = cur.zmask = 0;
        cur.ztile = false;
        const uint32_t mode = uni(wave_rows_mode<P, T>(a, c));
        request_rows<P, T, true>(a, c, mode == ROWS_DIRECT, cur.L, cur.H);
        if (mode == ROWS_GENERAL) {
            if (a.voff32) load_rows<P, T, true>(a, c, tile, cur);
            else load_rows<P, T, false>(a, c, tile, cur);
            asm volatile("; general rows requested");
        }
    } else {
        load_item<P, T>(a, c, tile, cur);
    }
    if constexpr (P == DEC_MID) {
        if (a.lostrange) {
            uint32_t r0, r1;
            lost_range(a, r0, r1);
            const bool any = r0 < r1;
            a.need_lo = max(a.need_lo, any ? r0 >> a.lo : 0u);
            a.need_hi = min(a.need_hi, any ? ((r1 - 1) >> a.lo) + 1 : 0u);
        }
    }
    RS16_STAMP(a, 1);
    prio<0>();
    st.template finish<EARLY>(a, c, smem);
    rcn.count();
    RS16_STAMP(a, 2);
    process_item<P, T, NV>(a, c, tile, cur, smem);
    rcn.store(a, c);
}

template <int P, int T, int NV = 0>
__global__ void __launch_bounds__(Geo<T>::THREADS, 4) pass_kernel_late(PassArgs a) {
    using G = Geo<T>;
    static_assert(WaveStaged<P, T>::value, "late rows: the wave-staged passes");
    extern __shared__ __attribute__((aligned(16))) uint8_t smem[];
    RS16_PASS_HEAD(P, T)
    using RQ = LateRows<P, T>;
    RS16_LATE_BODY(P, T, NV, RQ, false, false)
}
template <int P, int T, int NV, bool PAIR_IN, bool PAIR_OUT>
__global__ void __launch_bounds__(Geo<T>::THREADS, 4) pass_kernel_late_paired(PassArgs a) {
    static_assert(PAIR_IN || PAIR_OUT, "the unpaired kernel is pass_kernel_late");
    using G = Geo<T>;
    static_assert(WaveStaged<P, T>::value, "late rows: the wave-staged passes");
    extern __shared__ __attribute__((aligned(16))) uint8_t smem[];
    RS16_PASS_HEAD(P, T)
    using RQ = LateRows<P, T, PAIR_IN>;
    RS16_LATE_BODY(P, T, NV, RQ, PAIR_OUT, false)
}

template <int P, int T, bool PAIR> struct LateRowsTower : LateRows<P, T, PAIR> {
    TowerB tb;
    __device__ __forceinline__ LateRowsTower(const PassArgs& a, const Thr& c) : LateRows<P, T, PAIR>(a, c) {
        const cu32p q = (cu32p)a.skew_tab + TOWER_B_DWORD;
#pragma unroll
        for (int i = 0; i < 5; i++) tb.p[i] = q[i];
    }
};
template <int P, int T, int NV> __global__ void __launch_bounds__(Geo<T>::THREADS, 4) pass_kernel_late_tower(PassArgs a) {
    static_assert(P == ENC_FIRST || P == ENC_MID || P == ENC_LAST, "tower rows: the encoder's three passes");
    constexpr bool PAIR_IN = P != ENC_FIRST, PAIR_OUT = P != ENC_LAST;
    using G = Geo<T>;
    using RQ = typename std::conditional<P == ENC_MID, LateRows<P, T, PAIR_IN>, LateRowsTower<P, T, PAIR_IN>>::type;
    extern __shared__ __attribute__((aligned(16))) uint8_t smem[];
    RS16_PASS_HEAD(P, T)
    RS16_LATE_BODY(P, T, NV, RQ, PAIR_OUT, true)
}

template <int P, int T, int NV> PassFn late_entry() {
    if constexpr (WaveStaged<P, T>::value) return pass_kernel_late<P, T, NV>;
    else return nullptr;
}
template <int P, int T, int NV = 0> PassFn paired_entry() {
    static_assert(P == ENC_FIRST || P == ENC_MID || P == ENC_LAST, "paired rows: the encoder's three passes");
    return pass_kernel_late_paired<P, T, NV, P != ENC_FIRST, P != ENC_LAST>;
}
template <int P, int T, int NV = 0> PassKernel pass_entry() {
    using PT = ProgTraits<P>;
    return {pass_kernel<P, T, NV>, Smem<P, T>::BYTES, Geo<T>::THREADS, Geo<T>::Q,
            !PT::IFFT ? Geo<T>::SHB : 0, (!PT::FFT && T > 4) ? Geo<T>::SHB : 0, Geo<T>::R,
            PT::LOAD == LD_GATHER_ENC ? 1 : 0, {late_entry<P, T, NV>(), nullptr, nullptr}};
}
template <int P> PassKernel pass_row(int T) {
    static const PassKernel row[9] = {pass_entry<P, 0>(), pass_entry<P, 1>(), pass_entry<P, 2>(),
                                      pass_entry<P, 3>(), pass_entry<P, 4>(), pass_entry<P, 5>(),
                                      pass_entry<P, 6>(), pass_entry<P, 7>(), pass_entry<P, 8>()};
    return row[T];
}
template <int P, int NV> PassKernel narrow_row(int T) {
    static const PassKernel row[4] = {pass_entry<P, 5, NV>(), pass_entry<P, 6, NV>(), pass_entry<P, 7, NV>(),
                                      pass_entry<P, 8, NV>()};
    return T >= 5 ? row[T - 5] : PassKernel{};
}

}
```

reed-solomon-16_amd/csrc/rs16_pass_common.hpp:

```cpp
#pragma once
#include "rs16_internal.hpp"

namespace rs16 {

typedef void (*PassFn)(PassArgs);
struct PassKernel {
    PassFn fn;
    int lds;
    int threads;
    int quads;
    int load_shb, store_shb;
    int reg_bits;
    int gather;
    PassFn late[3];
};
struct PassConsts {
    uint32_t nslab, voff32, full_lanes;
    uint64_t rs_in, rs_seg, rs_out;
    uint32_t late_rows;
};
PassConsts pass_launch_consts(const PassKernel& k, int T, const PassArgs& a);
const PassKernel& pass_kernel_of(int prog, int T);
constexpr int NARROW_VARIANTS = 4;
PassKernel pass_kernels_enc(int prog, int T, int nv);
PassFn pass_kernels_paired(int prog, int T, int nv);
PassKernel pass_kernels_dec(int prog, int T, int nv);
PassFn pass_kernels_tower(int prog, int T, int nv);

#if defined(__HIPCC__) || defined(__HIP__)
typedef const __attribute__((address_space(4))) uint32_t* cu32p;

__device__ __forceinline__ uint32_t uni(uint32_t v) { return __builtin_amdgcn_readfirstlane(v); }

__host__ __device__ constexpr int vmcnt_wait(int n) { return (n & 15) | ((n >> 4) << 14) | (7 << 4) | (15 << 8); }

__device__ __forceinline__ void load_table_lds(uint32_t (&t)[20], const uint4* p) {
#pragma unroll
    for (int i = 0; i < 5; i++) {
        const uint4 v = p[i];
        t[4 * i] = v.x;
        t[4 * i + 1] = v.y;
        t[4 * i + 2] = v.z;
        t[4 * i + 3] = v.w;
    }
}

__device__ __forceinline__ void stripe_displace(PassArgs& a, uint32_t st) {
    a.in += st * a.bs_in;
    a.in2 += st * a.bs_in2;
    a.out += st * a.bs_out;
    a.seg_a += st * a.bs_seg;
    a.seg_b += st * a.bs_seg_b;
    a.rest += st * a.bs_rest;
    if (a.flags_a) a.flags_a += st * a.bs_fa;
    if (a.flags_b) a.flags_b += st * a.bs_fb;
    if (a.elog) a.elog += st * a.bs_elog;
    if (a.ework) a.ework += st * a.bs_elog;
    if (a.rbits) a.rbits += st * a.bs_rbits;
    if (a.zflags) a.zflags += st * a.bs_zflags;
    if (a.lostrange) a.lostrange += st * a.bs_lost;
}

__device__ __forceinline__ bool tile_is_zero(const PassArgs& a, uint32_t tile) {
    return (((cu32p)a.zflags)[tile >> 2] >> (8 * (tile & 3))) & 1u;
}
__device__ __forceinline__ void lost_range(const PassArgs& a, uint32_t& r0, uint32_t& r1) {
    r0 = ((cu32p)a.lostrange)[0];
    r1 = ((cu32p)a.lostrange)[1];
}

template <int T> __device__ __forceinline__ bool tl_covers(const PassArgs& a) {
    uint32_t r0, r1;
    lost_range(a, r0, r1);
    return r0 < r1 && ((r1 - 1) >> T) - (r0 >> T) < a.tl_max;
}

__device__ __forceinline__ bool mid_need(const PassArgs& a, uint32_t& nlo, uint32_t& nhi) {
    uint32_t r0, r1;
    lost_range(a, r0, r1);
    if (r0 >= r1) return false;
    nlo = max(a.need_lo, r0 >> a.lo);
    nhi = min(a.need_hi, ((r1 - 1) >> a.lo) + 1);
    return nhi > nlo && nhi - nlo <= MID_DIRECT_MAX;
}

__device__ __forceinline__ bool row_lost_original(const PassArgs& a, uint32_t r) {
    const uint32_t base = a.rest_seg_b ? a.chunk : 0;
    const uint32_t cnt = a.rest_seg_b ? a.b_count : a.a_count;
    const uint8_t* fl = a.rest_seg_b ? a.flags_b : a.flags_a;
    return r >= base && r - base < cnt && fl && !fl[r - base];
}
#endif

}
```

reed-solomon-16_amd/csrc/rs16_pass_launch.hip:

```cpp
#include <algorithm>

#include "rs16_pass_common.hpp"

namespace rs16 {

struct KernelTable {
    PassKernel k[NUM_PROGS][9][NARROW_VARIANTS];
    KernelTable() {
        for (int prog = 0; prog < NUM_PROGS; prog++)
            for (int T = 0; T <= 8; T++)
                for (int nv = 0; nv < NARROW_VARIANTS; nv++) {
                    PassKernel& e = k[prog][T][nv];
                    e = pass_kernels_enc(prog, T, nv);
                    if (!e.fn) e = pass_kernels_dec(prog, T, nv);
                    e.late[Z_PAIRED] = pass_kernels_paired(prog, T, nv);
                    e.late[Z_TOWER] = pass_kernels_tower(prog, T, nv);
                }
    }
};
static const PassKernel& find_kernel(int prog, int T, int nv) {
    static const KernelTable table;
    return table.k[prog][T][nv];
}

static const PassKernel& pick_kernel(int prog, int T, int ni, int nf) {
    for (int nv = 1; nv < NARROW_VARIANTS; nv++) {
        const int vi = nv == 2 ? 1 : 0, vf = nv == 3 ? 1 : 0;
        if (ni > vi || nf > vf) continue;
        const PassKernel& k = find_kernel(prog, T, nv);
        if (k.fn) return k;
    }
    return find_kernel(prog, T, 0);
}

const PassKernel& pass_kernel_of(int prog, int T) { return find_kernel(prog, T, 0); }

PassConsts pass_launch_consts(const PassKernel& k, int T, const PassArgs& a) {
    PassConsts c;
    c.nslab = (a.qrow + k.quads - 1) / k.quads;
    {
        const uint64_t hws = k.quads >= 64 ? 1 : 64 / k.quads;
        const uint64_t smax = std::max(std::max(a.S_in, a.S_out), std::max(a.S_seg, a.S_rest));
        const uint64_t span = (uint64_t)1 << (T + a.lo);
        const bool fits = (hws - 1) * ((uint64_t)16 << a.lo) * smax + 8 * (uint64_t)a.qrow <= ((uint64_t)1 << 32);
        const bool aligned = a.chunk % span == 0 && a.row_base_in % span == 0;
        c.voff32 = fits && aligned && !(a.diag & DIAG_FORCE_VOFF64) ? 1u : 0u;
    }
    c.rs_in = a.S_in << (a.lo + k.load_shb);
    c.rs_seg = a.S_seg << (a.lo + k.load_shb);
    c.rs_out = a.S_out << (a.lo + k.store_shb);
    const bool full = c.voff32 && a.qrow % k.quads == 0 && a.in_rows_mask == 0 && c.rs_out < ((uint64_t)1 << 28);
    c.full_lanes = full ? 1u : 0u;
    {
        const uint64_t hws = k.quads >= 64 ? 1 : 64 / k.quads;
        const uint64_t wave_span = (hws << k.reg_bits) << a.lo;
        const bool whole = !k.gather || a.a_count % wave_span == 0;
        const bool strides = c.rs_in < ((uint64_t)1 << 28) && c.rs_seg < ((uint64_t)1 << 28);
        const bool on = k.late[Z_SHARD] && !(a.diag & DIAG_NO_LATE_ROWS);
        c.late_rows = on && c.voff32 && a.in_rows_mask == 0 && whole && strides ? 1u : 0u;
    }
    return c;
}

ZForm z_form_sequence(uint32_t chunk_rows, uint64_t S, uint64_t S_user, uint32_t a_count, uint32_t seg_chunk,
                      uint32_t row_base_in, int diag) {
    if (diag & DIAG_NO_PAIRED_ROWS) return Z_SHARD;
    if (chunk_rows < 512 || (chunk_rows & (chunk_rows - 1)) || S == 0 || S % 8 || S / 8 > 0xFFFFFFFFu) return Z_SHARD;
    const RowSplit sp = row_split(__builtin_ctz(chunk_rows));
    PassArgs a{};
    a.S_in = a.S_out = a.S_rest = S;
    a.S_seg = S_user;
    a.qrow = (uint32_t)(S / 8);
    a.a_count = a_count, a.chunk = seg_chunk, a.row_base_in = row_base_in;
    a.diag = (uint32_t)diag;
    const struct { int prog, T; uint32_t lo; uint64_t S_out; } seq[3] = {
        {ENC_FIRST, sp.lo, 0, S}, {ENC_MID, sp.hi, (uint32_t)sp.lo, S}, {ENC_LAST, sp.lo, 0, S_user}};
    bool tower = !(diag & DIAG_NO_TOWER_ROWS);
    for (const auto& p : seq) {
        if (p.T > 8) return Z_SHARD;
        const PassKernel& k = find_kernel(p.prog, p.T, 0);
        a.lo = p.lo, a.S_out = p.S_out;
        const PassConsts c = pass_launch_consts(k, p.T, a);
        if (!k.fn || !k.late[Z_PAIRED] || !c.late_rows || !c.full_lanes) return Z_SHARD;
        tower = tower && k.late[Z_TOWER];
    }
    return tower ? Z_TOWER : Z_PAIRED;
}

hipError_t launch_pass(int prog, int T, const PassArgs& args, uint32_t num_tiles, hipStream_t s) {
    if (prog < 0 || prog >= NUM_PROGS || T < 0 || T > 8) return hipErrorInvalidValue;
    if (num_tiles == 0 || args.qrow == 0) return hipSuccess;
    PassArgs a = args;
    int ni = T, nf = T;
    if (!(a.diag & DIAG_WIDE_TWIDDLES)) {
        const uint32_t bh_max = (a.tile_base + (a.stripe_tiles ? a.stripe_tiles : num_tiles) - 1) >> a.lo;
        ni = first_narrow_layer(a.lo, T, a.skew_ifft, bh_max);
        nf = first_narrow_layer(a.lo, T, a.skew_fft, bh_max);
    }
    const PassKernel& k = pick_kernel(prog, T, ni, nf);
    const PassConsts pc = pass_launch_consts(k, T, a);
    a.nslab = pc.nslab;
    a.ntiles = num_tiles;
    const uint32_t nwg = num_tiles * a.nslab;
    if (a.need_hi == 0) a.need_hi = 1u << T;
    a.voff32 = pc.voff32;
    a.fd_lds = (a.diag & DIAG_FD_LDS) ? 1u : 0u;
    a.rs_in = pc.rs_in, a.rs_seg = pc.rs_seg, a.rs_out = pc.rs_out;
    a.full_lanes = pc.full_lanes;
    const FastDiv dn = fast_div_of(a.nslab), ds = fast_div_of(a.stripe_tiles);
    a.nslab_mul = dn.mul, a.nslab_one = dn.one;
    a.stripe_mul = ds.mul, a.stripe_one = ds.one;
    const size_t lds = (size_t)k.lds;
    PassFn fn = pc.late_rows ? k.late[Z_SHARD] : k.fn;
    if (a.z_form != Z_SHARD) {
        const bool in_sequence = prog == ENC_FIRST || prog == ENC_MID || prog == ENC_LAST;
        if (a.z_form > Z_TOWER || !in_sequence || !pc.late_rows || !pc.full_lanes || !k.late[a.z_form])
            return hipErrorInvalidValue;
        fn = k.late[a.z_form];
    }
    if (lds > 65536) {
        hipError_t e = hipFuncSetAttribute((const void*)fn, hipFuncAttributeMaxDynamicSharedMemorySize, (int)lds);
        if (e != hipSuccess) return e;
    }
    dim3 grid(nwg), block(k.threads);
    hipLaunchKernelGGL(fn, grid, block, lds, s, a);
    return hipGetLastError();
}

}
```

reed-solomon-16_amd/csrc/rs16_pass_tower.hip:

```cpp
#include "rs16_pass.hpp"

namespace rs16 {

PassFn pass_kernels_tower(int prog, int T, int nv) {
    if (prog == ENC_FIRST && T == 7 && nv == 0) return pass_kernel_late_tower<ENC_FIRST, 7, 0>;
    if (prog == ENC_LAST && T == 7 && nv == 0) return pass_kernel_late_tower<ENC_LAST, 7, 0>;
    if (prog == ENC_MID && T == 7) {
        if (nv == 0) return pass_kernel_late_tower<ENC_MID, 7, 0>;
        if (nv == 1) return pass_kernel_late_tower<ENC_MID, 7, 1>;
    }
    if (prog == ENC_MID && T == 8) {
        switch (nv) {
            case 0: return pass_kernel_late_tower<ENC_MID, 8, 0>;
            case 1: return pass_kernel_late_tower<ENC_MID, 8, 1>;
            case 2: return pass_kernel_late_tower<ENC_MID, 8, 2>;
            case 3: return pass_kernel_late_tower<ENC_MID, 8, 3>;
        }
    }
    return nullptr;
}

}
```

reed-solomon-16_amd/csrc/rs16_tables.cpp:

```cpp
#include <cstdio>
#include <cstdlib>
#include <algorithm>
#include <cstring>
#include <mutex>
#include <vector>

#include "rs16_internal.hpp"

namespace rs16 {

namespace {
const uint16_t kCantorBasis[16] = {0x0001, 0xACCA, 0x3C0E, 0x163E, 0xC582, 0xED2E, 0x914C, 0x4012,
                                   0x6C98, 0x10D8, 0x6A72, 0xB900, 0xFDB8, 0xFB34, 0xFF38, 0x991E};
HostTables g_tables;
std::once_flag g_once;

inline uint16_t gf_mul(const HostTables& t, uint16_t x, uint32_t log_m) {
    return x == 0 ? 0 : t.exp[add_mod(t.log[x], log_m)];
}

inline uint16_t tower_conv(const HostTables& t, uint16_t x) {
    uint16_t r = x;
    for (int i = 0; i < 8; i++)
        if ((x >> (8 + i)) & 1) r ^= t.tower_a[i];
    return r;
}

void fwht_full(std::vector<uint16_t>& v) {
    for (uint32_t d = 1; d < GF_ORDER; d <<= 1)
        for (uint32_t r = 0; r < GF_ORDER; r += 2 * d)
            for (uint32_t i = r; i < r + d; i++) {
                uint32_t a = v[i], b = v[i + d];
                v[i] = (uint16_t)add_mod(a, b);
                v[i + d] = (uint16_t)sub_mod(a, b);
            }
}

void build(HostTables& t) {
    t.exp.assign(GF_ORDER, 0);
    t.log.assign(GF_ORDER, 0);
    {
        uint32_t state = 1;
        for (uint32_t i = 0; i < GF_MODULUS; i++) {
            t.exp[state] = (uint16_t)i;
            state <<= 1;
            if (state >= GF_ORDER) state ^= 0x1002Du;
        }
        t.exp[0] = (uint16_t)GF_MODULUS;
    }
    {
        std::vector<uint16_t> cb(GF_ORDER, 0);
        for (int b = 0; b < 16; b++) {
            uint32_t w = 1u << b;
            for (uint32_t j = 0; j < w; j++) cb[j + w] = cb[j] ^ kCantorBasis[b];
        }
        for (uint32_t i = 0; i < GF_ORDER; i++) t.log[i] = t.exp[cb[i]];
        for (uint32_t i = 0; i < GF_ORDER; i++) t.exp[t.log[i]] = (uint16_t)i;
        t.exp[GF_MODULUS] = t.exp[0];
    }
    {
        std::vector<uint16_t> sk(GF_MODULUS, 0);
        uint16_t temp[15];
        for (int i = 1; i < 16; i++) temp[i - 1] = (uint16_t)(1u << i);
        for (int m = 0; m < 15; m++) {
            const uint32_t step = 1u << (m + 1);
            sk[(1u << m) - 1] = 0;
            for (int i = m; i < 15; i++) {
                const uint32_t s = 1u << (i + 1);
                for (uint32_t j = (1u << m) - 1; j < s; j += step) sk[j + s] = sk[j] ^ temp[i];
            }
            temp[m] = (uint16_t)(GF_MODULUS - t.log[gf_mul(t, temp[m], t.log[temp[m] ^ 1])]);
            for (int i = m + 1; i < 15; i++) temp[i] = gf_mul(t, temp[i], add_mod(t.log[temp[i] ^ 1], temp[m]));
        }
        t.skew.resize(GF_MODULUS);
        for (uint32_t i = 0; i < GF_MODULUS; i++) t.skew[i] = t.log[sk[i]];
    }
    t.log_walsh = t.log;
    t.log_walsh[0] = 0;
    fwht_full(t.log_walsh);

    for (uint32_t i = 0; i < GF_MODULUS; i++)
        if ((t.skew[i] == GF_MODULUS) != ((i & (i + 1)) == 0)) {
            fprintf(stderr, "rs16: skew table sentinel at unexpected index %u\n", i);
            abort();
        }
    t.skew_entry.assign(GF_ORDER, ZERO_ENTRY);
    for (uint32_t i = 0; i < GF_MODULUS; i++) t.skew_entry[i] = t.skew[i] == GF_MODULUS ? ZERO_ENTRY : t.skew[i];

    t.mul_tab.assign((size_t)TAB_ENTRIES * TAB_DWORDS, 0);
    static const int kOff3[4] = {0, 3, 8, 11};
    static const int kOff2[2] = {6, 14};
    for (uint32_t lm = 0; lm < GF_ORDER; lm++) {
        uint32_t* e = &t.mul_tab[(size_t)lm * TAB_DWORDS];
        for (int g = 0; g < 4; g++)
            for (uint32_t v = 0; v < 8; v++) {
                uint16_t p = gf_mul(t, (uint16_t)(v << kOff3[g]), lm);
                for (int ob = 0; ob < 2; ob++) {
                    uint32_t byte = (p >> (8 * ob)) & 0xFF;
                    e[(g * 2 + ob) * 2 + (v >> 2)] |= byte << (8 * (v & 3));
                }
            }
        for (int gg = 0; gg < 2; gg++)
            for (uint32_t v = 0; v < 4; v++) {
                uint16_t p = gf_mul(t, (uint16_t)(v << kOff2[gg]), lm);
                for (int ob = 0; ob < 2; ob++) e[16 + gg * 2 + ob] |= ((p >> (8 * ob)) & 0xFFu) << (8 * v);
            }
    }

    t.skew_tab.resize((size_t)GF_ORDER * TAB_DWORDS);
    for (uint32_t i = 0; i < GF_ORDER; i++)
        std::copy_n(&t.mul_tab[(size_t)t.skew_entry[i] * TAB_DWORDS], TAB_DWORDS, &t.skew_tab[(size_t)i * TAB_DWORDS]);
    for (uint32_t i = 0; i < GF_MODULUS; i++) {
        const uint32_t* e = &t.skew_tab[(size_t)i * TAB_DWORDS];
        const bool zero = (e[2] | e[3] | e[6] | e[7] | e[17]) == 0;
        if (zero != twiddle_narrow(i)) {
            fprintf(stderr, "rs16: skew table entry %u is %s a subfield twiddle, against the index rule\n", i,
                    zero ? "" : "not");
            abort();
        }
    }

    for (uint32_t i = 0; i < 8; i++) {
        const uint16_t a = (uint16_t)((1u << (8 + i)) ^ gf_mul(t, (uint16_t)(1u << i), t.log[1u << 8]));
        if (a >= 256) {
            fprintf(stderr, "rs16: basis vector v_%u is not a_i + v_i v_8 with a_i in the subfield\n", 8 + i);
            abort();
        }
        t.tower_a[i] = (uint8_t)a;
    }
    for (uint32_t v = 0; v < 8; v++) {
        t.tower_b[v >> 2] |= (tower_conv(t, (uint16_t)(v << 8)) & 0xFFu) << (8 * (v & 3));
        t.tower_b[2 + (v >> 2)] |= (tower_conv(t, (uint16_t)(v << 11)) & 0xFFu) << (8 * (v & 3));
        if (v < 4) t.tower_b[4] |= (tower_conv(t, (uint16_t)(v << 14)) & 0xFFu) << (8 * v);
    }
    t.skew_tab_tower.assign((size_t)GF_ORDER * TAB_DWORDS, 0);
    for (uint32_t i = 0; i < GF_MODULUS; i++) {
        const uint32_t lm = t.skew_entry[i];
        if (lm == ZERO_ENTRY) continue;
        uint32_t* e = &t.skew_tab_tower[(size_t)i * TAB_DWORDS];
        auto prod = [&](uint32_t x) { return tower_conv(t, gf_mul(t, tower_conv(t, (uint16_t)x), lm)); };
        for (int g = 0; g < 4; g++)
            for (uint32_t v = 0; v < 8; v++) {
                const uint16_t p = prod(v << kOff3[g]);
                for (int ob = 0; ob < 2; ob++) e[(g * 2 + ob) * 2 + (v >> 2)] |= ((p >> (8 * ob)) & 0xFFu) << (8 * (v & 3));
            }
        for (int gg = 0; gg < 2; gg++)
            for (uint32_t v = 0; v < 4; v++) {
                const uint16_t p = prod(v << kOff2[gg]);
                for (int ob = 0; ob < 2; ob++) e[16 + gg * 2 + ob] |= ((p >> (8 * ob)) & 0xFFu) << (8 * v);
            }
        if (!twiddle_narrow(i)) continue;
        const bool cross = (e[2] | e[3] | e[6] | e[7] | e[17] | e[8] | e[9] | e[12] | e[13] | e[18]) != 0;
        const bool same = e[10] == e[0] && e[11] == e[1] && e[14] == e[4] && e[15] == e[5] && e[19] == e[16];
        if (cross || !same) {
            fprintf(stderr, "rs16: tower table of subfield twiddle %u %s\n", i,
                    cross ? "crosses between the bytes" : "maps the two bytes differently");
            abort();
        }
    }
    std::copy_n(t.tower_b, 5, &t.skew_tab[TOWER_B_DWORD]);
    std::copy_n(t.tower_b, 5, &t.skew_tab_tower[TOWER_B_DWORD]);

    t.col_img.assign(COL_IMG_DWORDS, 0);
    for (uint32_t L = COL_LMIN; L <= COL_LGEN; L++)
        for (uint32_t d = 0; d < col_img_count(L); d++) {
            const uint32_t N = 1u << L, delta = d * N;
            uint32_t* img = &t.col_img[col_img_offset(L, d)];
            for (uint32_t g = 0; g + 1 < N; g++) {
                uint32_t kb = 0;
                while (g >= N - (N >> (kb + 1))) kb++;
                const uint32_t j = g - (N - (N >> kb));
                const uint32_t idx = (j << (kb + 1)) + (1u << kb) + delta - 1;
                std::copy_n(&t.skew_tab[(size_t)idx * TAB_DWORDS], 20, img + (size_t)g * 20);
            }
        }

    {
        std::vector<int64_t> w(GF_ORDER);
        for (uint32_t i = 0; i < GF_ORDER; i++) w[i] = t.log_walsh[i];
        auto fwht = [](int64_t* x, uint32_t n) {
            for (uint32_t d = 1; d < n; d <<= 1)
                for (uint32_t i = 0; i < n; i += 2 * d)
                    for (uint32_t j = i; j < i + d; j++) {
                        const int64_t a = x[j], b = x[j + d];
                        x[j] = a + b;
                        x[j + d] = a - b;
                    }
        };
        auto mod = [](int64_t v) { return (uint32_t)(((v % 65535) + 65535) % 65535); };
        fwht(w.data(), GF_ORDER);
        t.col_k.assign(COL_LGEN + 2, 0);
        {
            int64_t pre = 0;
            for (uint32_t n = 1, j = 0; n <= (2u << COL_LMAX); n <<= 1) {
                for (; j < n; j++) pre += mod(w[j]);
                uint32_t lg = 0;
                while ((1u << lg) < n) lg++;
                if (lg < t.col_k.size()) t.col_k[lg] = mod((int64_t)t.log_walsh[0] - pre);
            }
        }
        t.col_v.assign(COL_V_DWORDS, 0);
        for (uint32_t n = 1u << COL_LMIN; n <= (2u << COL_LMAX); n <<= 1) {
            std::vector<int64_t> v(n);
            for (uint32_t i = 0; i < n; i++) v[i] = mod(w[i]);
            fwht(v.data(), n);
            uint32_t lg = 0;
            while ((1u << lg) < n) lg++;
            const int64_t inv = (int64_t)1 << (16 - lg);
            for (uint32_t k = 0; k < n; k++) t.col_v[col_v_offset(n) + k] = mod(mod(v[k]) * inv);
        }
    }
}
}

std::vector<uint32_t> mid_matrix_entries(const HostTables& t, int L) {
    const int lo = L / 2, hi = L - lo;
    const uint32_t N = 1u << hi;
    const uint16_t one = t.exp[0];
    std::vector<uint32_t> ent((size_t)N * N, ZERO_ENTRY);
    std::vector<uint16_t> v(N), w(N);
    auto tw = [&](uint32_t r_tile, int kb) {
        const uint32_t m = (uint32_t)(lo + kb);
        return (uint32_t)t.skew[((size_t)r_tile << lo) + (1u << m) - 1];
    };
    for (uint32_t c = 0; c < N; c++) {
        std::fill(v.begin(), v.end(), 0);
        v[c] = one;
        for (int kb = 0; kb < hi; kb++) {
            const uint32_t d = 1u << kb;
            for (uint32_t r = 0; r < N; r += 2 * d) {
                const uint32_t lm = tw(r, kb);
                for (uint32_t i = r; i < r + d; i++) {
                    v[i + d] ^= v[i];
                    if (lm != GF_MODULUS) v[i] ^= gf_mul(t, v[i + d], lm);
                }
            }
        }
        for (uint32_t i = 0; i < N; i++) {
            uint16_t x = v[i];
            for (uint32_t b = 1; b < N; b <<= 1)
                if (!(i & b)) x ^= v[i | b];
            w[i] = x;
        }
        for (int kb = hi - 1; kb >= 0; kb--) {
            const uint32_t d = 1u << kb;
            for (uint32_t r = 0; r < N; r += 2 * d) {
                const uint32_t lm = tw(r, kb);
                for (uint32_t i = r; i < r + d; i++) {
                    if (lm != GF_MODULUS) w[i] ^= gf_mul(t, w[i + d], lm);
                    w[i + d] ^= w[i];
                }
            }
        }
        for (uint32_t o = 0; o < N; o++) ent[(size_t)o * N + c] = w[o] ? t.log[w[o]] : ZERO_ENTRY;
    }
    return ent;
}

const HostTables& host_tables() {
    std::call_once(g_once, [] { build(g_tables); });
    return g_tables;
}

}
```

reed-solomon-16_amd/rs16/_lib.py:

```python
from __future__ import annotations

import ctypes as C
import os
from pathlib import Path

PKG_ROOT = Path(__file__).resolve().parents[1]
LIB_PATH = Path(os.environ.get("RS16_LIB", PKG_ROOT / "build" / "librs16.so"))


class RS16Error(C.Structure):
    _fields_ = [("code", C.c_int32), ("v0", C.c_uint64), ("v1", C.c_uint64), ("v2", C.c_uint64)]


class PassConsts(C.Structure):
    _fields_ = [(n, C.c_uint32) for n in ("voff32", "full_lanes", "nslab", "quads", "threads", "load_shb",
                                          "store_shb", "reg_bits", "row_sets")] + \
               [(n, C.c_uint64) for n in ("rs_in", "rs_seg", "rs_out")] + [("late_rows", C.c_uint32)]


_sz, _p, _i, _e = C.c_size_t, C.c_void_p, C.c_int, C.POINTER(RS16Error)
_u32, _u64 = C.c_uint32, C.c_uint64

SIGNATURES = {
    "rs16_error_message": (_sz, [_e, C.c_char_p, _sz]),
    "rs16_version": (C.c_char_p, []),
    "rs16_host_mul": (None, [_p, _p, _sz, C.c_uint16]),
    "rs16_host_mul_narrow": (None, [_p, _p, _sz, C.c_uint16]),
    "rs16_host_twiddle": (C.c_uint32, [C.c_uint32, C.POINTER(C.c_uint32), C.POINTER(C.c_uint32)]),
    "rs16_host_twiddle_narrow": (C.c_int, [C.c_uint32]),
    "rs16_host_fast_div_check": (C.c_uint64, [C.c_uint32, C.c_uint32, C.c_uint32, C.c_uint32]),
    "rs16_host_pass_consts": (_i, [_i, _i, _u32, _u64, _u64, _u64, _u64, _u32, _u32, _u32, _u32, _i,
                                   C.POINTER(PassConsts)]),
    "rs16_host_pass_consts_rows": (_i, [_i, _i, _u32, _u64, _u64, _u64, _u64, _u32, _u32, _u32, _u32, _u32, _i,
                                        C.POINTER(PassConsts)]),
    "rs16_host_pass_consts_many": (_i, [_i, _i, _u32, _sz, _p, _p, _p, _p, _p, _u32, _u32, _u32, _i, _p]),
    "rs16_host_paired_rows": (_i, [_u32, _u64, _u64, _u32, _u32, _u32, _i]),
    "rs16_host_tower_rows": (_i, [_u32, _u64, _u64, _u32, _u32, _u32, _i]),
    "rs16_host_tower_basis": (_u32, [_u32]),
    "rs16_host_tower_conv": (None, [_p, _p, _sz]),
    "rs16_host_tower_twiddle": (_i, [_u32, C.POINTER(_u32)]),
    "rs16_host_mul_tower": (None, [_p, _p, _sz, _u32, _i]),
    "rs16_host_update_consts": (_i, [_u32, _u64, _u32, C.POINTER(_u32), C.POINTER(_u32), C.POINTER(_u32),
                                     C.POINTER(_u64)]),
    "rs16_engine_set_profiling": (_i, [_p, _i, _e]),
    "rs16_engine_profile_read": (_i, [_p, _i, C.POINTER(C.c_double), C.POINTER(C.c_uint64), _e]),
    "rs16_engine_profile_reset": (None, [_p]),
    "rs16_prog_count": (_i, []),
    "rs16_engine_set_diagnostics": (_i, [_p, _i]),
    "rs16_prog_name": (C.c_char_p, [_i]),
    "rs16_engine_set_stamps": (_i, [_p, _p, _i, _e]),
    "rs16_engine_set_slices": (_i, [_p, _i, _e]),
    "rs16_engine_new": (_p, [_i, _e]),
    "rs16_engine_new_ex": (_p, [_i, _i, _e]),
    "rs16_set_diagnostics": (_i, [_i]),
    "rs16_engine_free": (None, [_p]),
    "rs16_engine_device": (_i, [_p]),
    "rs16_engine_stream": (_p, [_p]),
    "rs16_engine_synchronize": (_i, [_p, _p, _e]),
    "rs16_engine_fft": (_i, [_p, _p, _sz, _sz, _sz, _sz, _sz, _sz, _p, _e]),
    "rs16_engine_fft_skew_end": (_i, [_p, _p, _sz, _sz, _sz, _sz, _sz, _p, _e]),
    "rs16_engine_ifft": (_i, [_p, _p, _sz, _sz, _sz, _sz, _sz, _sz, _p, _e]),
    "rs16_engine_ifft_skew_end": (_i, [_p, _p, _sz, _sz, _sz, _sz, _sz, _p, _e]),
    "rs16_engine_fwht": (_i, [_p, _p, _sz, _p, _e]),
    "rs16_engine_eval_poly": (_i, [_p, _p, _sz, _p, _e]),
    "rs16_engine_mul": (_i, [_p, _p, _sz, C.c_uint16, _p, _e]),
    "rs16_engine_xor": (_i, [_p, _p, _p, _sz, _p, _e]),
    "rs16_engine_xor_within": (_i, [_p, _p, _sz, _sz, _sz, _sz, _sz, _p, _e]),
    "rs16_engine_formal_derivative": (_i, [_p, _p, _sz, _sz, _p, _e]),
    "rs16_supports": (_i, [_i, _sz, _sz]),
    "rs16_validate": (_i, [_i, _sz, _sz, _sz, _e]),
    "rs16_use_high_rate": (_i, [_sz, _sz, _e]),
    "rs16_encoder_work_count": (_sz, [_i, _sz, _sz]),
    "rs16_decoder_work_count": (_sz, [_i, _sz, _sz]),
    "rs16_encoder_new": (_p, [_p, _i, _sz, _sz, _sz, _e]),
    "rs16_encoder_free": (None, [_p]),
    "rs16_encoder_reset": (_i, [_p, _sz, _sz, _sz, _e]),
    "rs16_encoder_add_original_shard": (_i, [_p, _p, _sz, _e]),
    "rs16_encoder_add_original_shard_device": (_i, [_p, _p, _sz, _e]),
    "rs16_encoder_encode": (_i, [_p, _e]),
    "rs16_encoder_recovery": (_p, [_p, _sz, _e]),
    "rs16_encoder_recovery_device": (_p, [_p, _sz]),
    "rs16_encoder_recovery_copy": (_i, [_p, _sz, _p, _sz, _e]),
    "rs16_encoder_result_drop": (None, [_p]),
    "rs16_encoder_is_high_rate": (_i, [_p]),
    "rs16_decoder_new": (_p, [_p, _i, _sz, _sz, _sz, _e]),
    "rs16_decoder_free": (None, [_p]),
    "rs16_decoder_reset": (_i, [_p, _sz, _sz, _sz, _e]),
    "rs16_decoder_add_original_shard": (_i, [_p, _sz, _p, _sz, _e]),
    "rs16_decoder_add_recovery_shard": (_i, [_p, _sz, _p, _sz, _e]),
    "rs16_decoder_add_original_shard_device": (_i, [_p, _sz, _p, _sz, _e]),
    "rs16_decoder_add_recovery_shard_device": (_i, [_p, _sz, _p, _sz, _e]),
    "rs16_decoder_decode": (_i, [_p, _e]),
    "rs16_decoder_restored_original": (_p, [_p, _sz, _e]),
    "rs16_decoder_restored_original_device": (_p, [_p, _sz]),
    "rs16_decoder_restored_original_copy": (_i, [_p, _sz, _p, _sz, _e]),
    "rs16_decoder_result_drop": (None, [_p]),
    "rs16_decoder_is_high_rate": (_i, [_p]),
    "rs16_encode_device": (_i, [_p, _sz, _sz, _sz, _p, _p, _p, _e]),
    "rs16_encode_device_batch": (_i, [_p, _sz, _sz, _sz, _sz, _p, _sz, _p, _sz, _p, _e]),
    "rs16_decode_device_batch": (_i, [_p, _sz, _sz, _sz, _sz, _p, _sz, _p, _p, _sz, _p, _sz, _sz, _p, _e]),
    "rs16_decode_device_batch_varied": (_i, [_p, _sz, _sz, _sz, _sz, _p, _sz, _p, _sz, _p, _sz, _p, _sz, _p, _p, _p,
                                             _e]),
    "rs16_decode_device": (_i, [_p, _sz, _sz, _sz, _p, _p, _p, _p, _sz, _sz, _p, _e]),
    "rs16_decode_check": (_i, [_p, _p, _e]),
    "rs16_device_alloc": (_p, [_p, _sz, _e]),
    "rs16_device_free": (None, [_p, _p]),
    "rs16_memcpy_htod": (_i, [_p, _p, _p, _sz, _p, _e]),
    "rs16_memcpy_dtoh": (_i, [_p, _p, _p, _sz, _p, _e]),
    "rs16_memset_device": (_i, [_p, _p, _i, _sz, _p, _e]),
    "rs16_memcpy2d_htod": (_i, [_p, _p, _sz, _p, _sz, _sz, _sz, _p, _e]),
    "rs16_memcpy2d_dtoh": (_i, [_p, _p, _sz, _p, _sz, _sz, _sz, _p, _e]),
    "rs16_encode_host": (_i, [_p, _sz, _sz, _sz, _p, _p, _sz, _e]),
    "rs16_decode_host": (_i, [_p, _sz, _sz, _sz, _p, _p, _p, _p, _sz, _e]),
    "rs16_host_alloc": (_p, [_p, _sz, _e]),
    "rs16_comm_unique_id": (_i, [_p, _e]),
    "rs16_comm_new": (_p, [_p, _i, _i, _p, _e]),
    "rs16_comm_init_all": (_i, [_p, _i, _p, _e]),
    "rs16_comm_free": (None, [_p]),
    "rs16_comm_rank": (_i, [_p]),
    "rs16_comm_size": (_i, [_p]),
    "rs16_column_slice": (_i, [_sz, _i, _i, C.POINTER(_sz), C.POINTER(_sz)]),
    "rs16_scatter_columns": (_i, [_p, _i, _i, _sz, _sz, _p, _p, _p, _e]),
    "rs16_gather_columns": (_i, [_p, _i, _i, _sz, _sz, _p, _p, _p, _e]),
    "rs16_scatter_columns_virtual": (_i, [_p, _i, _sz, _sz, _p, _p, _p, _e]),
    "rs16_gather_columns_virtual": (_i, [_p, _i, _sz, _sz, _p, _p, _p, _e]),
    "rs16_encode_host_multi": (_i, [_p, _i, _sz, _sz, _sz, _p, _p, _e]),
    "rs16_decode_prepare": (_i, [_p, _sz, _sz, _sz, _p, _p, _sz, _sz, _p, _e]),
    "rs16_decode_device_prepared": (_i, [_p, _sz, _sz, _sz, _p, _p, _p, _e]),
    "rs16_update_plan_new": (_p, [_p, _i, _sz, _sz, C.POINTER(_sz), _sz, _e]),
    "rs16_update_plan_free": (None, [_p]),
    "rs16_update_plan_count": (_sz, [_p]),
    "rs16_update_plan_coefficients": (_i, [_p, C.POINTER(C.c_uint16), _e]),
    "rs16_update_device": (_i, [_p, _sz, _p, _p, _sz, _sz, _p, _e]),
    "rs16_encode_host_batch":(_i, [_p, _sz, _sz, _sz, _sz, _p, _sz, _p, _sz, _e]),
    "rs16_decode_host_batch": (_i, [_p, _sz, _sz, _sz, _sz, _p, _sz, _p, _sz, _p, _sz, _p, _sz, _e]),
    "rs16_decode_host_multi": (_i, [_p, _i, _sz, _sz, _sz, _p, _p, _p, _p, _e]),
    "rs16_stream_create": (_p, [_p, _e]),
    "rs16_stream_destroy": (None, [_p, _p]),
    "rs16_host_free": (None, [_p, _p]),
}

_lib = None


def lib():
    global _lib
    if _lib is None:
        if not LIB_PATH.exists():
            raise OSError(f"rs16: native library not built: {LIB_PATH} (run make -C reed-solomon-16_amd/csrc)")
        L = C.CDLL(str(LIB_PATH))
        for name, (res, args) in SIGNATURES.items():
            f = getattr(L, name)
            f.restype, f.argtypes = res, args
        _lib = L
    return _lib


def hip_runtime():
    lib()
    with open("/proc/self/maps") as maps:
        for line in maps:
            path = line.split()[-1] if "/" in line else ""
            if "libamdhip64" in path and "/torch/" not in path:
                return C.CDLL(path)
    return C.CDLL("libamdhip64.so")
```

Before: 1003 GiB/s.

## Keep all encode passes in tower form with cheaper wide and beta twiddle multiplies

All three encode passes (first, mid, last) now use the tower-form skew table and run their butterflies in tower representation, not just the mid pass. Tower conversion moves to the first layer of the first pass and the last layer of the last pass. A wide multiply built from three byte maps and a beta multiply for twiddles of the form s + v_8 replace the generic six-selector multiply where index rules allow, cutting permute/XOR work per butterfly. It adds new kernel variants (wide3 for T=7), host-side table checks, and a host sweep validator, at the cost of more code paths and correctness risk in the variant selection logic.

```diff
diff --git a/include/rs16.h b/include/rs16.h
--- a/include/rs16.h
+++ b/include/rs16.h
@@ -247,7 +247,9 @@
 uint32_t rs16_host_tower_basis(uint32_t i);
 void rs16_host_tower_conv(const void* in, void* out, size_t bytes);
 int rs16_host_tower_twiddle(uint32_t index, uint32_t* table20);
-void rs16_host_mul_tower(const void* in, void* out, size_t bytes, uint32_t index, int narrow);
+void rs16_host_mul_tower(const void* in, void* out, size_t bytes, uint32_t index, int form);
+uint64_t rs16_host_tower_sweep(const uint32_t* index, size_t n, int form, const void* in, const void* want,
+                               size_t bytes);
 int rs16_host_update_consts(uint32_t rows, uint64_t shard_bytes, uint32_t n, uint32_t* quads_per_lane,
                             uint32_t* nslab, uint32_t* rows_per_wave, uint64_t* blocks);
 
diff --git a/reed-solomon-16_amd/csrc/rs16_api.cpp b/reed-solomon-16_amd/csrc/rs16_api.cpp
--- a/reed-solomon-16_amd/csrc/rs16_api.cpp
+++ b/reed-solomon-16_amd/csrc/rs16_api.cpp
@@ -1,4 +1,7 @@
+#include <algorithm>
 #include <atomic>
+#include <thread>
+#include <vector>
 #include <rccl/rccl.h>
 
 #include <cstdio>
@@ -167,9 +170,38 @@
     if (table20) memcpy(table20, &host_tables().skew_tab_tower[(size_t)index * TAB_DWORDS], 20 * sizeof(uint32_t));
     return 1;
 }
-extern "C" void rs16_host_mul_tower(const void* in, void* out, size_t bytes, uint32_t index, int narrow) {
+static void host_mul_tower(const void* in, void* out, size_t bytes, uint32_t index, int form) {
     const uint32_t* t = &host_tables().skew_tab_tower[(size_t)(index < GF_MODULUS ? index : GF_MODULUS) * TAB_DWORDS];
-    host_mul_table(in, out, bytes, t, narrow ? mul_xor_tower_narrow : mul_xor);
+    if (form == 2) host_mul_table(in, out, bytes, t, mul_xor_tower_wide);
+    else if (form == 3) host_mul_table(in, out, bytes, t, mul_xor_tower_beta);
+    else host_mul_table(in, out, bytes, t, form == 1 ? mul_xor_tower_narrow : mul_xor);
+}
+extern "C" void rs16_host_mul_tower(const void* in, void* out, size_t bytes, uint32_t index, int form) {
+    host_mul_tower(in, out, bytes, index, form);
+}
+extern "C" uint64_t rs16_host_tower_sweep(const uint32_t* index, size_t n, int form, const void* in, const void* want,
+                                          size_t bytes) {
+    std::atomic<uint64_t> bad{0};
+    std::atomic<size_t> next{0};
+    auto work = [&] {
+        std::vector<uint8_t> prod(bytes), shard(bytes);
+        for (size_t i; (i = next.fetch_add(1)) < n;) {
+            host_mul_tower(in, prod.data(), bytes, index[i], form);
+            rs16_host_tower_conv(prod.data(), shard.data(), bytes);
+            const uint8_t* w = (const uint8_t*)want + i * bytes;
+            uint64_t b = 0;
+            for (size_t blk = 0; blk < bytes / 64; blk++)
+                for (size_t e = 0; e < 32; e++)
+                    b += shard[blk * 64 + e] != w[blk * 64 + e] || shard[blk * 64 + 32 + e] != w[blk * 64 + 32 + e];
+            bad += b;
+        }
+    };
+    const size_t nthr = std::min<size_t>({n, 16, std::max(1u, std::thread::hardware_concurrency())});
+    std::vector<std::thread> thr;
+    for (size_t i = 1; i < nthr; i++) thr.emplace_back(work);
+    work();
+    for (auto& th : thr) th.join();
+    return bad.load();
 }
 extern "C" int rs16_host_update_consts(uint32_t rows, uint64_t shard_bytes, uint32_t n, uint32_t* quads_per_lane,
                                        uint32_t* nslab, uint32_t* rows_per_wave, uint64_t* blocks) {
diff --git a/reed-solomon-16_amd/csrc/rs16_engine.cpp b/reed-solomon-16_amd/csrc/rs16_engine.cpp
--- a/reed-solomon-16_amd/csrc/rs16_engine.cpp
+++ b/reed-solomon-16_amd/csrc/rs16_engine.cpp
@@ -290,9 +290,9 @@
     return profiled(PROF_COL_ENC, s, err, [&](uint64_t*) { return launch_col_multi(c, high, s); });
 }
 
-void rs16_engine::z_form_args(PassArgs& a, int prog, ZForm f) const {
+void rs16_engine::z_form_args(PassArgs& a, ZForm f) const {
     a.z_form = f;
-    a.skew_tab = prog == ENC_MID && f == Z_TOWER ? d_skew_tab_tower : d_skew_tab;
+    a.skew_tab = f == Z_TOWER ? d_skew_tab_tower : d_skew_tab;
 }
 
 int rs16_engine::fft(uint8_t* data, size_t S, size_t pos, size_t size, size_t skew_delta, hipStream_t s,
@@ -378,17 +378,15 @@
     const ZForm zf = z_form_sequence((uint32_t)chunk, S, S_user, a.a_count, a.chunk, a.row_base_in, diag);
     a.out = Z;
     a.lo = 0;
-    z_form_args(a, ENC_FIRST, zf);
+    z_form_args(a, zf);
     RS16_PASS(ENC_FIRST, lo, a, batch(1u << hi, 0, zs, bs_orig), s);
     a.in = Z;
     a.lo = lo;
-    z_form_args(a, ENC_MID, zf);
     RS16_PASS(ENC_MID, hi, a, batch(1u << lo, zs, zs, 0), s);
     a.in = Z;
     a.out = d_rec;
     a.S_out = S_user;
     a.lo = 0;
-    z_form_args(a, ENC_LAST, zf);
     const uint32_t tiles = (uint32_t)((m + ((size_t)1 << lo) - 1) >> lo);
     RS16_PASS(ENC_LAST, lo, a, batch(tiles, zs, bs_rec, 0), s);
     return RS16_OK;
@@ -568,18 +566,16 @@
             const ZForm zf = z_form_sequence(half, S, S_user, a.a_count, a.chunk, a.row_base_in, diag);
             a.lo = 0;
             a.out = Z;
-            z_form_args(a, ENC_FIRST, zf);
+            z_form_args(a, zf);
             RS16_PASS_AS(PROF_DEC_HALF_FIRST, ENC_FIRST, lo, a, batch(1u << hi, 0, 0, zs), s);
             a.rcount = nullptr;
             a.lo = lo;
             a.in = Z;
-            z_form_args(a, ENC_MID, zf);
             RS16_PASS_AS(PROF_DEC_HALF_MID, ENC_MID, hi, a, batch(1u << lo, zs, 0, zs), s);
             a.lo = 0;
             a.out = rest;
             a.S_out = S_user;
             a.out_rows = orig;
-            z_form_args(a, ENC_LAST, zf);
             a.rcount = rcount;
             a.cnt_flags = g.high ? flags_b : flags_a;
             a.cnt_base = dst;
diff --git a/reed-solomon-16_amd/csrc/rs16_engine.hpp b/reed-solomon-16_amd/csrc/rs16_engine.hpp
--- a/reed-solomon-16_amd/csrc/rs16_engine.hpp
+++ b/reed-solomon-16_amd/csrc/rs16_engine.hpp
@@ -155,7 +155,7 @@
     uint64_t prof_n[rs16::NUM_PROF] = {};
     int prof_collect(rs16_error* err);
 
-    void z_form_args(rs16::PassArgs& a, int prog, rs16::ZForm f) const;
+    void z_form_args(rs16::PassArgs& a, rs16::ZForm f) const;
     int fft(uint8_t* data, size_t S, size_t pos, size_t size, size_t skew_delta, hipStream_t s, rs16_error* err);
     int ifft(uint8_t* data, size_t S, size_t pos, size_t size, size_t skew_delta, hipStream_t s, rs16_error* err);
 
diff --git a/reed-solomon-16_amd/csrc/rs16_gf.hpp b/reed-solomon-16_amd/csrc/rs16_gf.hpp
--- a/reed-solomon-16_amd/csrc/rs16_gf.hpp
+++ b/reed-solomon-16_amd/csrc/rs16_gf.hpp
@@ -128,6 +128,30 @@
 RS16_HD void mul_xor_tower_narrow(uint32_t& xL, uint32_t& xH, uint32_t yL, uint32_t yH, const uint32_t* t) {
     mul_xor_tower_narrow_sel(xL, xH, mul_selectors(yL, yH), t);
 }
+RS16_HD void mul_xor_tower_wide_sel(uint32_t& xL, uint32_t& xH, const MulSel& y, const uint32_t* t) {
+    const uint32_t u0 = y.s0 ^ y.s3, u1 = y.s1 ^ y.s4, u2 = y.s2 ^ y.s5;
+    const uint32_t p0 = perm(t[1], t[0], y.s0), p1 = perm(t[5], t[4], y.s1), p2 = perm(t[16], t[16], y.s2);
+    const uint32_t q0 = perm(t[9], t[8], y.s3), q1 = perm(t[13], t[12], y.s4), q2 = perm(t[18], t[18], y.s5);
+    const uint32_t r0 = perm(t[11], t[10], u0), r1 = perm(t[15], t[14], u1), r2 = perm(t[19], t[19], u2);
+    const uint32_t p = xor3(p0, p1, p2);
+    xL = xor3(xor3(xL, p, q0), q1, q2);
+    xH = xor3(xor3(xH, p, r0), r1, r2);
+}
+RS16_HD void mul_xor_tower_wide(uint32_t& xL, uint32_t& xH, uint32_t yL, uint32_t yH, const uint32_t* t) {
+    mul_xor_tower_wide_sel(xL, xH, mul_selectors(yL, yH), t);
+}
+RS16_HD void mul_xor_tower_beta_sel(uint32_t& xL, uint32_t& xH, uint32_t yL, uint32_t yH, const MulSel& y,
+                                    const uint32_t* t) {
+    const uint32_t l0 = perm(t[1], t[0], y.s0), h0 = perm(t[1], t[0], y.s3);
+    const uint32_t l1 = perm(t[5], t[4], y.s1), h1 = perm(t[5], t[4], y.s4);
+    const uint32_t l2 = perm(t[16], t[16], y.s2), h2 = perm(t[16], t[16], y.s5);
+    const uint32_t q0 = perm(t[9], t[8], y.s3), q1 = perm(t[13], t[12], y.s4), q2 = perm(t[18], t[18], y.s5);
+    xL = xor3(xor3(xL, l0, l1), xor3(l2, q0, q1), q2);
+    xH = xor3(xor3(xH, h0, h1), h2, yL) ^ yH;
+}
+RS16_HD void mul_xor_tower_beta(uint32_t& xL, uint32_t& xH, uint32_t yL, uint32_t yH, const uint32_t* t) {
+    mul_xor_tower_beta_sel(xL, xH, yL, yH, mul_selectors(yL, yH), t);
+}
 
 RS16_HD uint32_t add_mod(uint32_t x, uint32_t y) {
     uint32_t s = x + y;
diff --git a/reed-solomon-16_amd/csrc/rs16_internal.hpp b/reed-solomon-16_amd/csrc/rs16_internal.hpp
--- a/reed-solomon-16_amd/csrc/rs16_internal.hpp
+++ b/reed-solomon-16_amd/csrc/rs16_internal.hpp
@@ -54,6 +54,17 @@
         k = kb;
     }
     return k;
+}
+
+RS16_HD bool twiddle_beta(uint32_t i) {
+    const uint32_t x = i + 1;
+    return (x >> 8) >= (x & (0u - x)) && (x >> 9) < (x & (0u - x));
+}
+inline bool layer_beta(uint32_t lo, int kb, int T, uint32_t skew, uint32_t bh_max) {
+    const uint64_t d = (uint64_t)1 << (lo + kb);
+    const uint64_t xmin = d + skew, xmax = (((uint64_t)bh_max + 1) << (lo + T)) - d + skew;
+    const uint64_t low = (d + skew) & (2 * d - 1);
+    return low != 0 && xmin >= ((low & (0 - low)) << 8) && xmax < ((low & (0 - low)) << 9);
 }
 
 enum Prog : int {
diff --git a/reed-solomon-16_amd/csrc/rs16_pass.hpp b/reed-solomon-16_amd/csrc/rs16_pass.hpp
--- a/reed-solomon-16_amd/csrc/rs16_pass.hpp
+++ b/reed-solomon-16_amd/csrc/rs16_pass.hpp
@@ -471,8 +471,15 @@
     static constexpr int FFT_FROM = NV == 0 ? NONE : (NV == 3 ? 1 : 0);
 };
 
+enum { TW_NONE = 0, TW_ROWS, TW_WIDE3 };
+template <bool WIDE3> __device__ __forceinline__ void mul_xor_tower_sel(uint32_t& xL, uint32_t& xH, const MulSel& y,
+                                                                      const uint32_t (&t)[20]) {
+    if constexpr (WIDE3) mul_xor_tower_wide_sel(xL, xH, y, t);
+    else mul_xor_sel<false>(xL, xH, y, t);
+}
+
 template <int P, int T, int NK, bool LB, int KB0, int KB1, bool FFT, bool IN_TAB2, int PRUNE, int G, class FIN = NoFin,
-          class PRE = NoPre, bool TW = false>
+          class PRE = NoPre, int TW = TW_NONE>
 struct GroupLoop {
     static __device__ __forceinline__ void run(uint32_t (&L)[Geo<T>::NR], uint32_t (&H)[Geo<T>::NR], const Thr& c,
                                                const PassArgs& a, const uint4* tab1, const uint4* tab2,
@@ -507,14 +514,41 @@
             for (int j = 0; j < (1 << rb); j++) {
                 const int m = (gi << (rb + 1)) + j, m2 = m + (1 << rb);
                 if constexpr (!std::is_same<PRE, NoPre>::value && s == 0) pre(L, H, (gi << rb) + j);
-                if constexpr (TW && P == ENC_LAST && LB && FFT && s == 0) {
+                if constexpr (TW && P == ENC_FIRST && !LB && kb == 0) {
+                    L[m2] ^= L[m];
+                    H[m2] ^= H[m];
                     MulSel y = high_selectors(H[m2]);
                     tower_conv_sel(L[m2], y, pre.tb);
                     y = low_selectors(L[m2], y);
                     tower_conv(L[m], H[m], pre.tb);
-                    mul_xor_sel<false>(L[m], H[m], y, cur);
+                    mul_xor_tower_sel<TW == TW_WIDE3>(L[m], H[m], y, cur);
+                } else if constexpr (TW && P == ENC_LAST && !LB && kb == 0) {
+                    const MulSel y = mul_selectors(L[m2], H[m2]);
+                    mul_xor_tower_sel<TW == TW_WIDE3>(L[m], H[m], y, cur);
+                    tower_conv_sel(L[m2], y, fin.tb);
+                    tower_conv(L[m], H[m], fin.tb);
                     L[m2] ^= L[m];
                     H[m2] ^= H[m];
+                } else if constexpr (TW && P != ENC_MID) {
+                    if (FFT) {
+                        mul_xor_tower_sel<TW == TW_WIDE3>(L[m], H[m], mul_selectors(L[m2], H[m2]), cur);
+                        L[m2] ^= L[m];
+                        H[m2] ^= H[m];
+                    } else {
+                        L[m2] ^= L[m];
+                        H[m2] ^= H[m];
+                        mul_xor_tower_sel<TW == TW_WIDE3>(L[m], H[m], mul_selectors(L[m2], H[m2]), cur);
+                    }
+                } else if constexpr (TW && P == ENC_MID && !NARROW && NK != NarrowVar<0>::NONE) {
+                    if (FFT) {
+                        mul_xor_tower_beta(L[m], H[m], L[m2], H[m2], cur);
+                        L[m2] ^= L[m];
+                        H[m2] ^= H[m];
+                    } else {
+                        L[m2] ^= L[m];
+                        H[m2] ^= H[m];
+                        mul_xor_tower_beta(L[m], H[m], L[m2], H[m2], cur);
+                    }
                 } else if constexpr (TW && P == ENC_MID && NARROW) {
                     if (FFT) {
                         mul_xor_tower_narrow(L[m], H[m], L[m2], H[m2], cur);
@@ -563,7 +597,7 @@
 }
 
 template <int P, int T, int NK, bool LB, int KB0, int KB1, bool FFT, bool IN_TAB2, int PRUNE = PR_NONE,
-          class FIN = NoFin, class PRE = NoPre, bool TW = false>
+          class FIN = NoFin, class PRE = NoPre, int TW = TW_NONE>
 __device__ __forceinline__ void layers(uint32_t (&L)[Geo<T>::NR], uint32_t (&H)[Geo<T>::NR], const Thr& c,
                                        const PassArgs& a, const uint4* tab1, const uint4* tab2,
                                        uint32_t zmask = 0, const FIN& fin = FIN(), const PRE& pre = PRE()) {
@@ -1105,6 +1139,10 @@
     }
 };
 
+template <int P, int T, bool PAIR> struct EarlyStoreTower : EarlyStore<P, T, PAIR> {
+    TowerB tb;
+};
+
 template <int T> struct HalfSeq {
     static constexpr int SH = Geo<T>::SHB, NR = Geo<T>::NR;
     static constexpr int at(int g) {
@@ -1125,8 +1163,8 @@
     }
 };
 struct NoTower {};
+template <bool WIDE3> struct TowerMul {};
 template <int T, int G, class FIN, class TB = NoTower> struct HalfLoop {
-    static_assert(std::is_same<TB, NoTower>::value || HalfSeq<T>::SH < Geo<T>::R, "a row's last layer: kb = T - 1");
     static __device__ __forceinline__ void run(uint32_t (&L)[Geo<T>::NR], uint32_t (&H)[Geo<T>::NR],
                                                const uint4* tab1, const uint32_t (&cur)[20], const FIN& fin,
                                                const TB& tb = TB()) {
@@ -1145,11 +1183,8 @@
             const int m = (gi << (rb + 1)) + j, m2 = m + (1 << rb);
             L[m2] ^= L[m];
             H[m2] ^= H[m];
-            if constexpr (!std::is_same<TB, NoTower>::value && kb == T - 1) {
-                const MulSel y = mul_selectors(L[m2], H[m2]);
-                mul_xor_sel<false>(L[m], H[m], y, cur);
-                tower_conv_sel(L[m2], y, tb);
-                tower_conv(L[m], H[m], tb);
+            if constexpr (std::is_same<TB, TowerMul<true>>::value) {
+                mul_xor_tower_wide(L[m], H[m], L[m2], H[m2], cur);
             } else {
                 mul_xor(L[m], H[m], L[m2], H[m2], cur);
             }
@@ -1193,8 +1228,10 @@
 __device__ __forceinline__ void process_item(const PassArgs& a, const Thr& c, uint32_t tile, ItemRegs<P, T>& d,
                                              uint8_t* smem, const PRE& pre = PRE()) {
     using PT = ProgTraits<P>;
-    constexpr int NKI = NarrowVar<NV>::IFFT_FROM, NKF = NarrowVar<NV>::FFT_FROM;
-    static_assert(NV == 0 || (PT::IFFT && PT::FFT && T > 4), "narrow variants: two-direction passes only");
+    constexpr bool WIDE3 = TOWER && !(PT::IFFT && PT::FFT) && NV == 1;
+    constexpr int TWF = !TOWER ? TW_NONE : (WIDE3 ? TW_WIDE3 : TW_ROWS);
+    constexpr int NKI = NarrowVar<(WIDE3 ? 0 : NV)>::IFFT_FROM, NKF = NarrowVar<(WIDE3 ? 0 : NV)>::FFT_FROM;
+    static_assert(NV == 0 || WIDE3 || (PT::IFFT && PT::FFT && T > 4), "narrow variants: two-direction passes only");
     using SM = Smem<P, T>;
     using G = Geo<T>;
     constexpr int NR = G::NR;
@@ -1255,7 +1292,7 @@
         if constexpr (ZERO_SKIP) skip_a = __all(d.zrow == (1u << NR) - 1);
         if constexpr (WaveStaged<P, T>::value) RS16_STAMP_ROWS(a, 6, L, H, 0, 1);
         if constexpr (!std::is_same<PRE, NoPre>::value)
-            layers<P, T, NKI, false, 0, R, false, false, PR_NONE, NoFin, PRE, TOWER>(L, H, c, a, tab1, tab2, 0, NoFin(),
+            layers<P, T, NKI, false, 0, R, false, false, PR_NONE, NoFin, PRE, TWF>(L, H, c, a, tab1, tab2, 0, NoFin(),
                                                                                      pre);
         else if (!skip_a) layers<P, T, NKI, false, 0, R, false, false>(L, H, c, a, tab1, tab2);
         RS16_STAMP(a, 3);
@@ -1286,11 +1323,11 @@
                 Thr cs = c;
                 asm volatile("" : "+v"(cs.offL));
                 const EvenStore<P, T, PAIR_OUT> even{a, cs, FastStore<P, T, PAIR_OUT>(a, cs)};
-                if constexpr (TOWER) ifft_b_halves<T>(L, H, tab1, even, pre.tb);
+                if constexpr (TOWER) ifft_b_halves<T>(L, H, tab1, even, TowerMul<WIDE3>());
                 else ifft_b_halves<T>(L, H, tab1, even);
             } else {
                 const uint4* tab1b = SM::SHARED ? (const uint4*)(smem + SM::TABB_OFF) - G::TSPLIT * 5 : tab1;
-                layers<P, T, NKI, true, R, T, false, false, (ZERO_SKIP ? PR_ZERO : PR_NONE), NoFin, NoPre, TOWER>(
+                layers<P, T, NKI, true, R, T, false, false, (ZERO_SKIP ? PR_ZERO : PR_NONE), NoFin, NoPre, TWF>(
                     L, H, c, a, tab1b, tab2, d.zmask);
             }
             in_b = true;
@@ -1312,10 +1349,10 @@
         if constexpr (T > 4) {
             if constexpr (WaveStaged<P, T>::value && !PT::IFFT) RS16_STAMP_ROWS(a, 6, L, H, 0, NR / 2);
             if constexpr (!std::is_same<PRE, NoPre>::value && !PT::IFFT)
-                layers<P, T, NKF, true, R, T, true, TWO, PR_NONE, NoFin, PRE, TOWER>(L, H, c, a, tab1, tab2, 0, NoFin(),
+                layers<P, T, NKF, true, R, T, true, TWO, PR_NONE, NoFin, PRE, TWF>(L, H, c, a, tab1, tab2, 0, NoFin(),
                                                                                      pre);
             else
-                layers<P, T, NKF, true, R, T, true, TWO, (P == DEC_MID ? PR_OUT : PR_NONE), NoFin, NoPre, TOWER>(
+                layers<P, T, NKF, true, R, T, true, TWO, (P == DEC_MID ? PR_OUT : PR_NONE), NoFin, NoPre, TWF>(
                     L, H, c, a, tab1, tab2);
             if constexpr (SPLIT_FD) {
                 if (fd_few) {
@@ -1365,11 +1402,17 @@
             for (int m = 0; m < NR; m++) any |= lostf[kidx<T, false>(c, m)];
             need = any != 0;
         }
-        if constexpr (EARLY) {
+        if constexpr (EARLY && TOWER && P == ENC_LAST) {
+            Thr cs = c;
+            asm volatile("" : "+v"(cs.offL));
+            layers<P, T, NKF, false, 0, R, true, false, PR_NONE, EarlyStoreTower<P, T, PAIR_OUT>, NoPre, TWF>(
+                L, H, c, a, tab1, tab2, 0,
+                EarlyStoreTower<P, T, PAIR_OUT>{{a, cs, rvt, lostf, FastStore<P, T, PAIR_OUT>(a, cs)}, pre.tb});
+        } else if constexpr (EARLY) {
             Thr cs = c;
             asm volatile("" : "+v"(cs.offL));
             layers<P, T, NKF, false, 0, R, true, (TWO && !(SM::RESTAGE)), PR_NONE, EarlyStore<P, T, PAIR_OUT>, NoPre,
-                   TOWER>(L, H, c, a, tab1, tab2, 0,
+                   TWF>(L, H, c, a, tab1, tab2, 0,
                           EarlyStore<P, T, PAIR_OUT>{a, cs, rvt, lostf, FastStore<P, T, PAIR_OUT>(a, cs)});
         } else if (need) {
             layers<P, T, NKF, false, 0, R, true, (TWO && !(SM::RESTAGE))>(L, H, c, a, tab1, tab2);
@@ -1565,7 +1608,7 @@
     using PT = ProgTraits<P>;
     return {pass_kernel<P, T, NV>, Smem<P, T>::BYTES, Geo<T>::THREADS, Geo<T>::Q,
             !PT::IFFT ? Geo<T>::SHB : 0, (!PT::FFT && T > 4) ? Geo<T>::SHB : 0, Geo<T>::R,
-            PT::LOAD == LD_GATHER_ENC ? 1 : 0, {late_entry<P, T, NV>(), nullptr, nullptr}};
+            PT::LOAD == LD_GATHER_ENC ? 1 : 0, {late_entry<P, T, NV>(), nullptr, nullptr}, nullptr};
 }
 template <int P> PassKernel pass_row(int T) {
     static const PassKernel row[9] = {pass_entry<P, 0>(), pass_entry<P, 1>(), pass_entry<P, 2>(),
diff --git a/reed-solomon-16_amd/csrc/rs16_pass_common.hpp b/reed-solomon-16_amd/csrc/rs16_pass_common.hpp
--- a/reed-solomon-16_amd/csrc/rs16_pass_common.hpp
+++ b/reed-solomon-16_amd/csrc/rs16_pass_common.hpp
@@ -13,6 +13,7 @@
     int reg_bits;
     int gather;
     PassFn late[3];
+    PassFn wide3;
 };
 struct PassConsts {
     uint32_t nslab, voff32, full_lanes;
@@ -26,6 +27,7 @@
 PassFn pass_kernels_paired(int prog, int T, int nv);
 PassKernel pass_kernels_dec(int prog, int T, int nv);
 PassFn pass_kernels_tower(int prog, int T, int nv);
+PassFn pass_kernel_tower_wide3(int prog, int T);
 
 #if defined(__HIPCC__) || defined(__HIP__)
 typedef const __attribute__((address_space(4))) uint32_t* cu32p;
diff --git a/reed-solomon-16_amd/csrc/rs16_pass_launch.hip b/reed-solomon-16_amd/csrc/rs16_pass_launch.hip
--- a/reed-solomon-16_amd/csrc/rs16_pass_launch.hip
+++ b/reed-solomon-16_amd/csrc/rs16_pass_launch.hip
@@ -15,6 +15,7 @@
                     if (!e.fn) e = pass_kernels_dec(prog, T, nv);
                     e.late[Z_PAIRED] = pass_kernels_paired(prog, T, nv);
                     e.late[Z_TOWER] = pass_kernels_tower(prog, T, nv);
+                    e.wide3 = nv == 0 ? pass_kernel_tower_wide3(prog, T) : nullptr;
                 }
     }
 };
@@ -23,14 +24,13 @@
     return table.k[prog][T][nv];
 }
 
-static const PassKernel& pick_kernel(int prog, int T, int ni, int nf) {
+static int pick_variant(int prog, int T, int ni, int nf) {
     for (int nv = 1; nv < NARROW_VARIANTS; nv++) {
         const int vi = nv == 2 ? 1 : 0, vf = nv == 3 ? 1 : 0;
         if (ni > vi || nf > vf) continue;
-        const PassKernel& k = find_kernel(prog, T, nv);
-        if (k.fn) return k;
+        if (find_kernel(prog, T, nv).fn) return nv;
     }
-    return find_kernel(prog, T, 0);
+    return 0;
 }
 
 const PassKernel& pass_kernel_of(int prog, int T) { return find_kernel(prog, T, 0); }
@@ -92,12 +92,16 @@
     if (num_tiles == 0 || args.qrow == 0) return hipSuccess;
     PassArgs a = args;
     int ni = T, nf = T;
+    const uint32_t bh_max = (a.tile_base + (a.stripe_tiles ? a.stripe_tiles : num_tiles) - 1) >> a.lo;
     if (!(a.diag & DIAG_WIDE_TWIDDLES)) {
-        const uint32_t bh_max = (a.tile_base + (a.stripe_tiles ? a.stripe_tiles : num_tiles) - 1) >> a.lo;
         ni = first_narrow_layer(a.lo, T, a.skew_ifft, bh_max);
         nf = first_narrow_layer(a.lo, T, a.skew_fft, bh_max);
     }
-    const PassKernel& k = pick_kernel(prog, T, ni, nf);
+    int nv = pick_variant(prog, T, ni, nf);
+    if (a.z_form == Z_TOWER && ((nv == 2 && !layer_beta(a.lo, 0, T, a.skew_ifft, bh_max)) ||
+                                (nv == 3 && !layer_beta(a.lo, 0, T, a.skew_fft, bh_max))))
+        nv = 0;
+    const PassKernel& k = find_kernel(prog, T, nv);
     const PassConsts pc = pass_launch_consts(k, T, a);
     a.nslab = pc.nslab;
     a.ntiles = num_tiles;
@@ -117,6 +121,7 @@
         if (a.z_form > Z_TOWER || !in_sequence || !pc.late_rows || !pc.full_lanes || !k.late[a.z_form])
             return hipErrorInvalidValue;
         fn = k.late[a.z_form];
+        if (a.z_form == Z_TOWER && k.wide3 && !(a.diag & DIAG_WIDE_TWIDDLES)) fn = k.wide3;
     }
     if (lds > 65536) {
         hipError_t e = hipFuncSetAttribute((const void*)fn, hipFuncAttributeMaxDynamicSharedMemorySize, (int)lds);
diff --git a/reed-solomon-16_amd/csrc/rs16_pass_tower.hip b/reed-solomon-16_amd/csrc/rs16_pass_tower.hip
--- a/reed-solomon-16_amd/csrc/rs16_pass_tower.hip
+++ b/reed-solomon-16_amd/csrc/rs16_pass_tower.hip
@@ -20,4 +20,10 @@
     return nullptr;
 }
 
+PassFn pass_kernel_tower_wide3(int prog, int T) {
+    if (prog == ENC_FIRST && T == 7) return pass_kernel_late_tower<ENC_FIRST, 7, 1>;
+    if (prog == ENC_LAST && T == 7) return pass_kernel_late_tower<ENC_LAST, 7, 1>;
+    return nullptr;
 }
+
+}
diff --git a/reed-solomon-16_amd/csrc/rs16_tables.cpp b/reed-solomon-16_amd/csrc/rs16_tables.cpp
--- a/reed-solomon-16_amd/csrc/rs16_tables.cpp
+++ b/reed-solomon-16_amd/csrc/rs16_tables.cpp
@@ -156,6 +156,40 @@
             fprintf(stderr, "rs16: tower table of subfield twiddle %u %s\n", i,
                     cross ? "crosses between the bytes" : "maps the two bytes differently");
             abort();
+        }
+    }
+    {
+        const uint16_t beta = 1u << 8, v7 = 1u << 7;
+        if (gf_mul(t, beta, t.log[beta]) != (beta ^ v7)) {
+            fprintf(stderr, "rs16: v_8^2 is not v_8 + v_7: no three-map wide multiply in tower form\n");
+            abort();
+        }
+        for (uint32_t i = 0; i < GF_MODULUS; i++) {
+            const uint32_t lm = t.skew_entry[i];
+            if (lm == ZERO_ENTRY) continue;
+            const uint32_t* e = &t.skew_tab_tower[(size_t)i * TAB_DWORDS];
+            bool ok = (e[0] ^ e[10]) == e[2] && (e[1] ^ e[11]) == e[3] && (e[4] ^ e[14]) == e[6] &&
+                      (e[5] ^ e[15]) == e[7] && (e[16] ^ e[19]) == e[17];
+            for (uint32_t j = 0; j < 16 && ok; j++) {
+                const uint32_t a = (j & 7) | (((j + 3) & 7) << 3) | ((j & 3) << 6);
+                const uint32_t b = j < 8 ? ((j + 5) & 7) | (((j * 3) & 7) << 3) | (((j + 1) & 3) << 6) : 0;
+                const uint16_t x = (uint16_t)(a | (b << 8));
+                const uint16_t want = tower_conv(t, gf_mul(t, tower_conv(t, x), lm));
+                uint32_t xl = 0, xh = 0;
+                mul_xor_tower_wide(xl, xh, a * 0x01010101u, b * 0x01010101u, e);
+                ok = xl == (want & 0xFFu) * 0x01010101u && xh == (uint32_t)(want >> 8) * 0x01010101u;
+            }
+            if (!ok) {
+                fprintf(stderr, "rs16: tower table of twiddle %u does not multiply by three byte maps\n", i);
+                abort();
+            }
+            const bool one = e[2] == 0x03020100u && e[3] == 0x07060504u && e[6] == 0x18100800u &&
+                             e[7] == 0x38302820u && e[17] == 0xC0804000u;
+            if (one != twiddle_beta(i)) {
+                fprintf(stderr, "rs16: twiddle %u is %s s + v_8 with s in the subfield, against the index rule\n", i,
+                        one ? "" : "not");
+                abort();
+            }
         }
     }
     std::copy_n(t.tower_b, 5, &t.skew_tab[TOWER_B_DWORD]);
diff --git a/reed-solomon-16_amd/rs16/_lib.py b/reed-solomon-16_amd/rs16/_lib.py
--- a/reed-solomon-16_amd/rs16/_lib.py
+++ b/reed-solomon-16_amd/rs16/_lib.py
@@ -40,6 +40,7 @@
     "rs16_host_tower_conv": (None, [_p, _p, _sz]),
     "rs16_host_tower_twiddle": (_i, [_u32, C.POINTER(_u32)]),
     "rs16_host_mul_tower": (None, [_p, _p, _sz, _u32, _i]),
+    "rs16_host_tower_sweep": (_u64, [C.POINTER(_u32), _sz, _i, _p, _p, _sz]),
     "rs16_host_update_consts": (_i, [_u32, _u64, _u32, C.POINTER(_u32), C.POINTER(_u32), C.POINTER(_u32),
                                      C.POINTER(_u64)]),
     "rs16_engine_set_profiling": (_i, [_p, _i, _e]),
```

Result: faster. 1037 GiB/s, median of 6 (+3.3%).
